# PACTHEMAN123/spMV-test

Hardware: AMD Instinct MI355X
Metric: fp32 CSR SpMV: achieved HBM GB/s (rocprofv3 FETCH_SIZE + WRITE_SIZE bytes of the K steps / wall time) (higher is better)
Workload: dtype f32; 1 GPU; c4: 16777216 x 16777216, nnz 268435456, row lengths 'mixed' mean 16, banded columns (band 8192), seed 20251031; variant=auto, rows_per_gpu=16777216, nnz_per_gpu=268435456, parallelism=single GPU, devices=1 ranks on 1 device(s), launch=one process, algorithmic_bytes_per_gpu=2348810244, hbm_bytes_per_gpu=1840380781

## Files before the change

include/spmv_hip.h:

```cpp
#ifndef SPMV_HIP_H
#define SPMV_HIP_H

#include <stdint.h>

#if defined(__GNUC__)
#define SPMV_API __attribute__((visibility("default")))
#else
#define SPMV_API
#endif

#ifdef __cplusplus
extern "C" {
#endif

typedef struct spmv_csr spmv_csr_t;

enum spmv_status {
    SPMV_OK = 0,
    SPMV_ERR_NO_DEVICE = -1,
    SPMV_ERR_INVALID = -2,
    SPMV_ERR_HIP = -3,
    SPMV_ERR_VARIANT = -4,
    SPMV_ERR_NOT_PLANNED = -5,
    SPMV_ERR_STALE_PLAN = -6
};

enum spmv_variant {
    SPMV_SCALAR = 0,
    SPMV_WAVE = 1,
    SPMV_WAVE_PIPE = 2,
    SPMV_VECTOR = 3,
    SPMV_ADAPTIVE = 4,
    SPMV_TILED = 5,
    SPMV_PANEL = 6,
    SPMV_AUTO = 7,
    SPMV_XSKIP = 8,
    SPMV_VARIANT_COUNT = 9
};

SPMV_API int spmv_device_count(void);
SPMV_API const char *spmv_last_error(void);
SPMV_API const char *spmv_variant_name(int variant);
SPMV_API float spmv_last_first_launch_ms(void);


SPMV_API int spmv_csr_create_host(int64_t rows, int64_t cols, int64_t nnz, const int32_t *row_ptr,
                         const int32_t *col_idx, const float *vals, spmv_csr_t **out);

SPMV_API int spmv_csr_create_device(int64_t rows, int64_t cols, int64_t nnz, const int32_t *d_row_ptr,
                           const int32_t *d_col_idx, const float *d_vals, spmv_csr_t **out);

SPMV_API int spmv_csr_from_dense_host(int M, int N, const float *A_host, void *stream, spmv_csr_t **out);

SPMV_API int spmv_csr_from_dense_device(int M, int N, const float *d_A, void *stream, spmv_csr_t **out);

SPMV_API int spmv_csr_download(const spmv_csr_t *h, int32_t *row_ptr, int32_t *col_idx, float *vals);

SPMV_API int spmv_csr_validate(const spmv_csr_t *h, void *stream);

SPMV_API int spmv_csr_dims(const spmv_csr_t *h, int64_t *rows, int64_t *cols, int64_t *nnz);

SPMV_API int spmv_csr_column_range(const spmv_csr_t *h, int64_t *col_min, int64_t *col_max, void *stream);
SPMV_API int spmv_csr_destroy(spmv_csr_t *h);

SPMV_API int spmv_csr_transpose(const spmv_csr_t *a, int keep_map, void *stream, spmv_csr_t **out);
SPMV_API int spmv_csr_transpose_values(spmv_csr_t *t, const spmv_csr_t *a, void *stream);
SPMV_API int64_t spmv_csr_transpose_map_bytes(const spmv_csr_t *t);

SPMV_API int spmv_csr_plan(spmv_csr_t *h, int variant, void *stream);
SPMV_API int spmv_csr_run(spmv_csr_t *h, int variant, const float *d_x, float *d_y, void *stream);

SPMV_API int spmv_csr_values_changed(spmv_csr_t *h);

SPMV_API int spmv_csr_plan_get(const spmv_csr_t *h, int variant, int32_t params[8]);
SPMV_API int spmv_csr_plan_set(spmv_csr_t *h, int variant, const int32_t params[8], void *stream);
SPMV_API int spmv_csr_plan_like(spmv_csr_t *dst, const spmv_csr_t *src, int variant, void *stream);

SPMV_API int64_t spmv_csr_plan_bytes(const spmv_csr_t *h, int variant);

SPMV_API int spmv_csr_plan_describe(const spmv_csr_t *h, int variant, char *buf, int n);

SPMV_API int spmv_csr_time(spmv_csr_t *h, int variant, const float *d_x, float *d_y, int iters,
                  void *stream, float *ms_per_launch);

SPMV_API int spmv_csr_run_host(spmv_csr_t *h, int variant, const float *x_host, float *y_host,
                               float *kernel_ms);

SPMV_API int spmv_csr_spmm_plan(spmv_csr_t *h, void *stream);
SPMV_API int spmv_csr_spmm(spmv_csr_t *h, int k, const float *d_X, int64_t ldx, float *d_Y, int64_t ldy, void *stream);
SPMV_API int64_t spmv_csr_spmm_plan_bytes(const spmv_csr_t *h);
SPMV_API int spmv_csr_spmm_describe(const spmv_csr_t *h, char *buf, int n);

SPMV_API int spmv_dense_gemv(int M, int N, const float *d_A, const float *d_x, float *d_y, int mode,
                    void *stream);

SPMV_API int64_t spmv_dense_gemv_workspace_bytes(int N, int mode);
SPMV_API int spmv_dense_gemv_ws(int M, int N, const float *d_A, const float *d_x, float *d_y, int mode,
                                void *d_workspace, int64_t workspace_bytes, void *stream);

SPMV_API int spmv_dense_gemv_host(int M, int N, const float *A_host, const float *x_host, float *y_host,
                                  int mode, float *kernel_ms);

SPMV_API int spmv_asp_retile(int M, int N, const float *d_A, float *d_asp, void *stream);
SPMV_API int spmv_asp_gemv_ws(int M, int N, const float *d_asp, const float *d_x, float *d_y, void *d_workspace,
                              int64_t workspace_bytes, void *stream);

typedef struct spmv_tcsr spmv_tcsr_t;
SPMV_API int spmv_tcsr_from_dense_host(int M, int N, const float *A_host, void *stream, spmv_tcsr_t **out);
SPMV_API int spmv_tcsr_from_dense_device(int M, int N, const float *d_A, void *stream, spmv_tcsr_t **out);
SPMV_API int spmv_tcsr_sizes(const spmv_tcsr_t *h, int64_t *n_blk_idx, int64_t *n_bitmaps, int64_t *n_vals);
SPMV_API int spmv_tcsr_download(const spmv_tcsr_t *h, int32_t *blk_idx, uint32_t *bitmaps, float *vals);
SPMV_API int spmv_tcsr_run(const spmv_tcsr_t *h, const float *d_x, float *d_y, void *stream);
SPMV_API int spmv_tcsr_run_host(const spmv_tcsr_t *h, const float *x_host, float *y_host, float *kernel_ms);
SPMV_API int spmv_tcsr_destroy(spmv_tcsr_t *h);

enum spmv_bitmap_format { SPMV_FMT_WSP = 0, SPMV_FMT_AWSP = 1, SPMV_FMT_AWSP_REF = 2, SPMV_FMT_COUNT = 3 };
typedef struct spmv_bitmap spmv_bitmap_t;
SPMV_API int spmv_bitmap_from_dense_host(int format, int M, int N, const float *A_host, void *stream, spmv_bitmap_t **out);
SPMV_API int spmv_bitmap_from_dense_device(int format, int M, int N, const float *d_A, void *stream, spmv_bitmap_t **out);
SPMV_API int spmv_bitmap_sizes(const spmv_bitmap_t *h, int64_t *n_bitmaps, int64_t *n_vals, int32_t stats[4]);
SPMV_API int spmv_bitmap_download(const spmv_bitmap_t *h, uint32_t *bitmaps, float *vals);
SPMV_API int spmv_bitmap_run(const spmv_bitmap_t *h, const float *d_x, float *d_y, void *stream);
SPMV_API int spmv_bitmap_run_host(const spmv_bitmap_t *h, const float *x_host, float *y_host, float *kernel_ms);
SPMV_API int spmv_bitmap_destroy(spmv_bitmap_t *h);

SPMV_API int spmv_synth_fill(uint64_t seed, int64_t row0, int64_t n_local, int64_t rows, int64_t cols,
                    int64_t band, const int32_t *d_row_ptr, int32_t *d_col_idx, float *d_vals,
                    void *stream);
SPMV_API int spmv_synth_x(uint64_t seed, int64_t j0, int64_t n, float *d_x, void *stream);

SPMV_API int spmv_calib_stream(const void *d_src, int64_t bytes, float *d_sink, void *stream);
SPMV_API int spmv_calib_gather(const float *d_table, int64_t table_lines, int64_t n_lines, int touch, float *d_sink,
                               void *stream);
SPMV_API int spmv_calib_store(float *d_dst, int64_t bytes, int width, void *stream);
SPMV_API int spmv_calib_marker(int id, void *stream);

SPMV_API int spmv_debug_bounds(int64_t *records, int n);

#ifdef __cplusplus
}
#endif
#endif
```

spmv-test_amd/capi.py:

```python
from __future__ import annotations

import ctypes as C
import os
from pathlib import Path

PKG_DIR = Path(__file__).resolve().parent
LIB_PATH = PKG_DIR / "lib" / "libspmv_hip.so"
LAUNCHERS_PATH = PKG_DIR / "lib" / "libspmv_launchers.so"
TESTER_PATH = PKG_DIR / "bin" / "sparse_sgemv"
DIST_LIB_PATH = PKG_DIR / "lib" / "libspmv_dist.so"
DIST_SELFTEST_PATH = PKG_DIR / "bin" / "spmv_dist_selftest"

SCALAR, WAVE, WAVE_PIPE, VECTOR, ADAPTIVE, TILED, PANEL, AUTO, XSKIP = range(9)
VARIANTS = {"scalar": SCALAR, "wave": WAVE, "wave_pipe": WAVE_PIPE, "vector": VECTOR,
            "adaptive": ADAPTIVE, "tiled": TILED, "panel": PANEL, "auto": AUTO}
ALL_VARIANTS = dict(VARIANTS, xskip=XSKIP)

OK, ERR_NO_DEVICE, ERR_INVALID, ERR_HIP, ERR_VARIANT, ERR_NOT_PLANNED, ERR_STALE_PLAN = 0, -1, -2, -3, -4, -5, -6

_i32p, _f32p, _vp = C.c_void_p, C.c_void_p, C.c_void_p
_H = C.c_void_p
_HP = C.POINTER(C.c_void_p)
SIGNATURES = {
    "spmv_device_count": (C.c_int, []),
    "spmv_last_error": (C.c_char_p, []),
    "spmv_variant_name": (C.c_char_p, [C.c_int]),
    "spmv_last_first_launch_ms": (C.c_float, []),
    "spmv_csr_create_host": (C.c_int, [C.c_int64, C.c_int64, C.c_int64, _i32p, _i32p, _f32p, _HP]),
    "spmv_csr_create_device": (C.c_int, [C.c_int64, C.c_int64, C.c_int64, _i32p, _i32p, _f32p, _HP]),
    "spmv_csr_from_dense_host": (C.c_int, [C.c_int, C.c_int, _f32p, _vp, _HP]),
    "spmv_csr_from_dense_device": (C.c_int, [C.c_int, C.c_int, _f32p, _vp, _HP]),
    "spmv_csr_download": (C.c_int, [_H, _i32p, _i32p, _f32p]),
    "spmv_csr_validate": (C.c_int, [_H, C.c_void_p]),
    "spmv_csr_dims": (C.c_int, [_H, C.POINTER(C.c_int64), C.POINTER(C.c_int64), C.POINTER(C.c_int64)]),
    "spmv_csr_column_range": (C.c_int, [_H, C.POINTER(C.c_int64), C.POINTER(C.c_int64), _vp]),
    "spmv_csr_destroy": (C.c_int, [_H]),
    "spmv_csr_transpose": (C.c_int, [_H, C.c_int, _vp, _HP]),
    "spmv_csr_transpose_values": (C.c_int, [_H, _H, _vp]),
    "spmv_csr_transpose_map_bytes": (C.c_int64, [_H]),
    "spmv_csr_plan": (C.c_int, [_H, C.c_int, _vp]),
    "spmv_csr_run": (C.c_int, [_H, C.c_int, _f32p, _f32p, _vp]),
    "spmv_csr_values_changed": (C.c_int, [_H]),
    "spmv_csr_spmm_plan": (C.c_int, [_H, _vp]),
    "spmv_csr_spmm": (C.c_int, [_H, C.c_int, _f32p, C.c_int64, _f32p, C.c_int64, _vp]),
    "spmv_csr_spmm_plan_bytes": (C.c_int64, [_H]),
    "spmv_csr_spmm_describe": (C.c_int, [_H, C.c_char_p, C.c_int]),
    "spmv_csr_plan_get": (C.c_int, [_H, C.c_int, C.POINTER(C.c_int32)]),
    "spmv_csr_plan_set": (C.c_int, [_H, C.c_int, C.POINTER(C.c_int32), _vp]),
    "spmv_csr_plan_like": (C.c_int, [_H, _H, C.c_int, _vp]),
    "spmv_csr_plan_bytes": (C.c_int64, [_H, C.c_int]),
    "spmv_csr_plan_describe": (C.c_int, [_H, C.c_int, C.c_char_p, C.c_int]),
    "spmv_csr_time": (C.c_int, [_H, C.c_int, _f32p, _f32p, C.c_int, _vp, C.POINTER(C.c_float)]),
    "spmv_csr_run_host": (C.c_int, [_H, C.c_int, _f32p, _f32p, C.POINTER(C.c_float)]),
    "spmv_dense_gemv": (C.c_int, [C.c_int, C.c_int, _f32p, _f32p, _f32p, C.c_int, _vp]),
    "spmv_dense_gemv_workspace_bytes": (C.c_int64, [C.c_int, C.c_int]),
    "spmv_dense_gemv_ws": (C.c_int, [C.c_int, C.c_int, _f32p, _f32p, _f32p, C.c_int, _vp, C.c_int64, _vp]),
    "spmv_asp_retile": (C.c_int, [C.c_int, C.c_int, _f32p, _f32p, _vp]),
    "spmv_asp_gemv_ws": (C.c_int, [C.c_int, C.c_int, _f32p, _f32p, _f32p, _vp, C.c_int64, _vp]),
    "spmv_dense_gemv_host": (C.c_int, [C.c_int, C.c_int, _f32p, _f32p, _f32p, C.c_int, C.POINTER(C.c_float)]),
    "spmv_tcsr_from_dense_host": (C.c_int, [C.c_int, C.c_int, _f32p, _vp, _HP]),
    "spmv_tcsr_from_dense_device": (C.c_int, [C.c_int, C.c_int, _f32p, _vp, _HP]),
    "spmv_tcsr_sizes": (C.c_int, [_H, C.POINTER(C.c_int64), C.POINTER(C.c_int64), C.POINTER(C.c_int64)]),
    "spmv_tcsr_download": (C.c_int, [_H, _i32p, _i32p, _f32p]),
    "spmv_tcsr_run": (C.c_int, [_H, _f32p, _f32p, _vp]),
    "spmv_tcsr_run_host": (C.c_int, [_H, _f32p, _f32p, C.POINTER(C.c_float)]),
    "spmv_tcsr_destroy": (C.c_int, [_H]),
    "spmv_bitmap_from_dense_host": (C.c_int, [C.c_int, C.c_int, C.c_int, _f32p, _vp, _HP]),
    "spmv_bitmap_from_dense_device": (C.c_int, [C.c_int, C.c_int, C.c_int, _f32p, _vp, _HP]),
    "spmv_bitmap_sizes": (C.c_int, [_H, C.POINTER(C.c_int64), C.POINTER(C.c_int64), C.POINTER(C.c_int32)]),
    "spmv_bitmap_download": (C.c_int, [_H, _i32p, _f32p]),
    "spmv_bitmap_run": (C.c_int, [_H, _f32p, _f32p, _vp]),
    "spmv_bitmap_run_host": (C.c_int, [_H, _f32p, _f32p, C.POINTER(C.c_float)]),
    "spmv_bitmap_destroy": (C.c_int, [_H]),
    "spmv_synth_fill": (C.c_int, [C.c_uint64, C.c_int64, C.c_int64, C.c_int64, C.c_int64, C.c_int64,
                                  _i32p, _i32p, _f32p, _vp]),
    "spmv_synth_x": (C.c_int, [C.c_uint64, C.c_int64, C.c_int64, _f32p, _vp]),
    "spmv_calib_stream": (C.c_int, [_vp, C.c_int64, _f32p, _vp]),
    "spmv_calib_gather": (C.c_int, [_f32p, C.c_int64, C.c_int64, C.c_int, _f32p, _vp]),
    "spmv_calib_store": (C.c_int, [_f32p, C.c_int64, C.c_int, _vp]),
    "spmv_calib_marker": (C.c_int, [C.c_int, _vp]),
    "spmv_debug_bounds": (C.c_int, [_vp, C.c_int]),
}
CHECKED_LIB_PATH = PKG_DIR / "lib" / "libspmv_hip_checked.so"
BOUNDS_SITES = ("k_bs_sums prod", "k_bs_sums acc", "k_bin_sums prod", "k_bin_sums r16", "k_bs_products c16",
                "k_bs_products pvals", "k_bs_products prod store", "k_bs_group store", "k_bs_place load",
                "k_bs_place acc store", "k_bs_place c16/pvals store", "k_bs_fill acc store", "k_bs_fill c16/pvals store",
                "k_panel packed", "k_panel pvals")


class SpmvError(RuntimeError):
    def __init__(self, status: int, message: str):
        super().__init__(f"libspmv_hip status {status}: {message}")
        self.status = status


_lib = None


def use_library(path) -> None:
    global _lib, LIB_PATH
    LIB_PATH = Path(path).resolve()
    _lib = None


def lib() -> C.CDLL:
    global _lib
    if _lib is None:
        if not LIB_PATH.exists():
            raise FileNotFoundError(
                f"{LIB_PATH} is missing: run `python -c 'import __graft_entry__ as g; g.build()'` "
                "(or `make -C spmv-test_amd`); there is no fallback implementation")
        import torch
        l = C.CDLL(os.fspath(LIB_PATH), mode=C.RTLD_LOCAL)
        for name, (res, args) in SIGNATURES.items():
            fn = getattr(l, name)
            fn.restype, fn.argtypes = res, args
        _lib = l
    return _lib


def check(status: int) -> None:
    if status != OK:
        raise SpmvError(status, lib().spmv_last_error().decode(errors="replace"))


def device_count() -> int:
    return lib().spmv_device_count()


def _ptr(t) -> int:
    if t is None:
        return 0
    if hasattr(t, "data_ptr"):
        return t.data_ptr()
    return t.ctypes.data


def _stream_handle(stream=None) -> int:
    import torch
    s = stream if stream is not None else torch.cuda.current_stream()
    return s.cuda_stream


class CsrMatrix:

    def __init__(self, handle: int, keepalive=()):
        self._h = C.c_void_p(handle)
        self._keep = tuple(keepalive)
        r, c, z = C.c_int64(), C.c_int64(), C.c_int64()
        check(lib().spmv_csr_dims(self._h, C.byref(r), C.byref(c), C.byref(z)))
        self.rows, self.cols, self.nnz = r.value, c.value, z.value

    @classmethod
    def from_host(cls, rows, cols, row_ptr, col_idx, vals):
        import numpy as np
        row_ptr = np.ascontiguousarray(row_ptr, dtype=np.int32)
        col_idx = np.ascontiguousarray(col_idx, dtype=np.int32)
        vals = np.ascontiguousarray(vals, dtype=np.float32)
        h = C.c_void_p()
        check(lib().spmv_csr_create_host(rows, cols, int(col_idx.size), _ptr(row_ptr), _ptr(col_idx),
                                         _ptr(vals), C.byref(h)))
        return cls(h.value)

    @classmethod
    def from_device(cls, rows, cols, row_ptr, col_idx, vals):
        h = C.c_void_p()
        check(lib().spmv_csr_create_device(rows, cols, int(col_idx.numel()), _ptr(row_ptr), _ptr(col_idx),
                                           _ptr(vals), C.byref(h)))
        return cls(h.value, keepalive=(row_ptr, col_idx, vals))

    @classmethod
    def from_dense_host(cls, A):
        import numpy as np
        A = np.ascontiguousarray(A, dtype=np.float32)
        M, N = A.shape
        h = C.c_void_p()
        check(lib().spmv_csr_from_dense_host(M, N, _ptr(A), 0, C.byref(h)))
        return cls(h.value)

    @classmethod
    def from_dense_device(cls, A):
        M, N = A.shape
        h = C.c_void_p()
        check(lib().spmv_csr_from_dense_device(M, N, _ptr(A), _stream_handle(), C.byref(h)))
        return cls(h.value)

    def plan(self, variant: int, stream=None) -> None:
        check(lib().spmv_csr_plan(self._h, variant, _stream_handle(stream)))

    def run(self, variant: int, x, y, stream=None) -> None:
        assert x.numel() >= self.cols and y.numel() >= self.rows
        check(lib().spmv_csr_run(self._h, variant, _ptr(x), _ptr(y), _stream_handle(stream)))

    def column_range(self, stream=None):
        lo, hi = C.c_int64(), C.c_int64()
        check(lib().spmv_csr_column_range(self._h, C.byref(lo), C.byref(hi), _stream_handle(stream)))
        return lo.value, hi.value

    def transpose(self, keep_map: bool = False, stream=None) -> "CsrMatrix":
        h = C.c_void_p()
        check(lib().spmv_csr_transpose(self._h, 1 if keep_map else 0, _stream_handle(stream), C.byref(h)))
        return CsrMatrix(h.value)

    def transpose_values(self, a: "CsrMatrix", stream=None) -> None:
        check(lib().spmv_csr_transpose_values(self._h, a._h, _stream_handle(stream)))

    def transpose_map_bytes(self) -> int:
        n = lib().spmv_csr_transpose_map_bytes(self._h)
        if n < 0:
            check(n)
        return n

    def spmm_plan(self, stream=None) -> None:
        check(lib().spmv_csr_spmm_plan(self._h, _stream_handle(stream)))

    def spmm(self, X, Y, stream=None) -> None:
        import torch
        for name, t in (("X", X), ("Y", Y)):
            if not isinstance(t, torch.Tensor) or t.dim() != 2 or t.dtype != torch.float32 or t.stride(1) != 1:
                raise ValueError(f"spmm: {name} must be a 2-D float32 tensor with stride(1) == 1")
        k = X.shape[1]
        if X.shape[0] != self.cols or Y.shape[0] != self.rows or Y.shape[1] < k:
            raise ValueError(f"spmm: X {tuple(X.shape)} and Y {tuple(Y.shape)} do not fit a {self.rows} x {self.cols} matrix")
        check(lib().spmv_csr_spmm(self._h, k, _ptr(X), X.stride(0), _ptr(Y), Y.stride(0), _stream_handle(stream)))

    def spmm_describe(self) -> str:
        buf = C.create_string_buffer(256)
        check(lib().spmv_csr_spmm_describe(self._h, buf, 256))
        return buf.value.decode()

    def spmm_plan_bytes(self) -> int:
        n = lib().spmv_csr_spmm_plan_bytes(self._h)
        if n < 0:
            check(n)
        return n

    def values_changed(self) -> None:
        check(lib().spmv_csr_values_changed(self._h))

    def time(self, variant: int, x, y, iters: int, stream=None) -> float:
        ms = C.c_float()
        check(lib().spmv_csr_time(self._h, variant, _ptr(x), _ptr(y), iters, _stream_handle(stream),
                                  C.byref(ms)))
        return ms.value

    def run_host(self, variant: int, x, y) -> float:
        import numpy as np
        assert x.dtype == np.float32 and y.dtype == np.float32
        ms = C.c_float()
        check(lib().spmv_csr_run_host(self._h, variant, _ptr(x), _ptr(y), C.byref(ms)))
        return ms.value

    def plan_params(self, variant: int):
        a = (C.c_int32 * 8)()
        check(lib().spmv_csr_plan_get(self._h, variant, a))
        return list(a)

    def plan_set(self, variant: int, params, stream=None) -> None:
        a = (C.c_int32 * 8)(*params)
        check(lib().spmv_csr_plan_set(self._h, variant, a, _stream_handle(stream)))

    def plan_like(self, other: "CsrMatrix", variant: int, stream=None) -> None:
        check(lib().spmv_csr_plan_like(self._h, other._h, variant, _stream_handle(stream)))

    def plan_describe(self, variant: int) -> str:
        buf = C.create_string_buffer(256)
        check(lib().spmv_csr_plan_describe(self._h, variant, buf, 256))
        return buf.value.decode()

    def plan_bytes(self, variant: int) -> int:
        return lib().spmv_csr_plan_bytes(self._h, variant)

    def download(self):
        import numpy as np
        rp = np.empty(self.rows + 1, np.int32)
        ci = np.empty(self.nnz, np.int32)
        va = np.empty(self.nnz, np.float32)
        check(lib().spmv_csr_download(self._h, _ptr(rp), _ptr(ci), _ptr(va)))
        return rp, ci, va

    def close(self) -> None:
        if self._h:
            check(lib().spmv_csr_destroy(self._h))
            self._h = C.c_void_p()
            self._keep = ()

    def __del__(self):
        try:
            self.close()
        except Exception:
            pass


class TcsrMatrix:

    def __init__(self, handle: int, M: int, N: int):
        self._h = C.c_void_p(handle)
        self.M, self.N = M, N
        a, b, c = C.c_int64(), C.c_int64(), C.c_int64()
        check(lib().spmv_tcsr_sizes(self._h, C.byref(a), C.byref(b), C.byref(c)))
        self.n_blk_idx, self.n_bitmaps, self.nnz = a.value, b.value, c.value

    @classmethod
    def from_dense_host(cls, A):
        import numpy as np
        A = np.ascontiguousarray(A, dtype=np.float32)
        M, N = A.shape
        h = C.c_void_p()
        check(lib().spmv_tcsr_from_dense_host(M, N, _ptr(A), 0, C.byref(h)))
        return cls(h.value, M, N)

    @classmethod
    def from_dense_device(cls, A):
        M, N = A.shape
        h = C.c_void_p()
        check(lib().spmv_tcsr_from_dense_device(M, N, _ptr(A), _stream_handle(), C.byref(h)))
        return cls(h.value, M, N)

    def download(self):
        import numpy as np
        bi = np.empty(self.n_blk_idx, np.int32)
        bm = np.empty(self.n_bitmaps, np.uint32)
        va = np.empty(self.nnz, np.float32)
        check(lib().spmv_tcsr_download(self._h, _ptr(bi), _ptr(bm), _ptr(va)))
        return bi, bm, va

    def run(self, x, y, stream=None) -> None:
        assert x.numel() >= self.M and y.numel() >= self.N
        check(lib().spmv_tcsr_run(self._h, _ptr(x), _ptr(y), _stream_handle(stream)))

    def run_host(self, x, y) -> float:
        ms = C.c_float()
        check(lib().spmv_tcsr_run_host(self._h, _ptr(x), _ptr(y), C.byref(ms)))
        return ms.value

    def close(self) -> None:
        if self._h:
            check(lib().spmv_tcsr_destroy(self._h))
            self._h = C.c_void_p()

    def __del__(self):
        try:
            self.close()
        except Exception:
            pass


BITMAP_FORMATS = {"wsp": 0, "awsp": 1, "awsp_ref": 2}


class BitmapMatrix:

    def __init__(self, handle: int, fmt: str, M: int, N: int):
        self._h = C.c_void_p(handle)
        self.fmt, self.M, self.N = fmt, M, N
        a, b = C.c_int64(), C.c_int64()
        st = (C.c_int32 * 4)()
        check(lib().spmv_bitmap_sizes(self._h, C.byref(a), C.byref(b), st))
        self.n_bitmaps, self.n_vals, self.stats = a.value, b.value, list(st)

    @classmethod
    def from_dense_host(cls, fmt: str, A):
        import numpy as np
        A = np.ascontiguousarray(A, dtype=np.float32)
        M, N = A.shape
        h = C.c_void_p()
        check(lib().spmv_bitmap_from_dense_host(BITMAP_FORMATS[fmt], M, N, _ptr(A), 0, C.byref(h)))
        return cls(h.value, fmt, M, N)

    @classmethod
    def from_dense_device(cls, fmt: str, A):
        M, N = A.shape
        h = C.c_void_p()
        check(lib().spmv_bitmap_from_dense_device(BITMAP_FORMATS[fmt], M, N, _ptr(A), _stream_handle(), C.byref(h)))
        return cls(h.value, fmt, M, N)

    def download(self):
        import numpy as np
        bm = np.empty(self.n_bitmaps, np.uint32)
        va = np.empty(self.n_vals, np.float32)
        check(lib().spmv_bitmap_download(self._h, _ptr(bm), _ptr(va)))
        return bm, va

    def run(self, x, y, stream=None) -> None:
        assert x.numel() >= self.M and y.numel() >= self.N
        check(lib().spmv_bitmap_run(self._h, _ptr(x), _ptr(y), _stream_handle(stream)))

    def run_host(self, x, y) -> float:
        ms = C.c_float()
        check(lib().spmv_bitmap_run_host(self._h, _ptr(x), _ptr(y), C.byref(ms)))
        return ms.value

    def close(self) -> None:
        if self._h:
            check(lib().spmv_bitmap_destroy(self._h))
            self._h = C.c_void_p()

    def __del__(self):
        try:
            self.close()
        except Exception:
            pass


def dense_gemv(A, x, y, mode: int, stream=None, workspace=None) -> None:
    M, N = A.shape
    if workspace is None:
        check(lib().spmv_dense_gemv(M, N, _ptr(A), _ptr(x), _ptr(y), mode, _stream_handle(stream)))
    else:
        check(lib().spmv_dense_gemv_ws(M, N, _ptr(A), _ptr(x), _ptr(y), mode, _ptr(workspace),
                                       workspace.numel() * workspace.element_size(), _stream_handle(stream)))


def dense_gemv_workspace_bytes(N: int, mode: int) -> int:
    return lib().spmv_dense_gemv_workspace_bytes(N, mode)


def asp_retile(A, out, stream=None) -> None:
    M, N = A.shape
    check(lib().spmv_asp_retile(M, N, _ptr(A), _ptr(out), _stream_handle(stream)))


def asp_gemv(M: int, N: int, asp, x, y, workspace, stream=None) -> None:
    check(lib().spmv_asp_gemv_ws(M, N, _ptr(asp), _ptr(x), _ptr(y), _ptr(workspace),
                                 workspace.numel() * workspace.element_size(), _stream_handle(stream)))


def synth_fill(seed, row0, n_local, rows, cols, band, row_ptr, col_idx, vals, stream=None) -> None:
    check(lib().spmv_synth_fill(seed, row0, n_local, rows, cols, band, _ptr(row_ptr), _ptr(col_idx),
                                _ptr(vals), _stream_handle(stream)))


def synth_x(seed, j0, n, x, stream=None) -> None:
    check(lib().spmv_synth_x(seed, j0, n, _ptr(x), _stream_handle(stream)))


def calib_stream(src, nbytes: int, sink, stream=None) -> None:
    check(lib().spmv_calib_stream(_ptr(src), nbytes, _ptr(sink), _stream_handle(stream)))


def calib_gather(table, table_lines: int, n_lines: int, touch: int, sink, stream=None) -> None:
    check(lib().spmv_calib_gather(_ptr(table), table_lines, n_lines, touch, _ptr(sink), _stream_handle(stream)))


def calib_store(dst, nbytes: int, width: int, stream=None) -> None:
    check(lib().spmv_calib_store(_ptr(dst), nbytes, width, _stream_handle(stream)))


def calib_marker(ident: int, stream=None) -> None:
    check(lib().spmv_calib_marker(ident, _stream_handle(stream)))


def debug_bounds(max_records: int = 64) -> list:
    import numpy as np
    rec = np.zeros(3 * max_records, np.int64)
    n = lib().spmv_debug_bounds(rec.ctypes.data, max_records)
    if n < 0:
        check(n)
    return [(BOUNDS_SITES[int(rec[3 * i])], int(rec[3 * i + 1]), int(rec[3 * i + 2])) for i in range(min(n, max_records))]
```

spmv-test_amd/csrc/capi.hip:

```cpp
#include <cstdarg>
#include <cstdint>
#include <cstdlib>
#include <cstring>
#include <new>
#include "spmv_internal.hpp"

namespace spmv {

static thread_local char g_err[512] = "";
static thread_local float g_first_launch_ms = 0.0f;

void set_error(const char *fmt, ...)
{
    va_list ap;
    va_start(ap, fmt);
    vsnprintf(g_err, sizeof g_err, fmt, ap);
    va_end(ap);
}

int hip_fail(hipError_t e, const char *what, const char *file, int line)
{
    set_error("HIP error %s:%d: %s (%s)", file, line, hipGetErrorString(e), what);
    return SPMV_ERR_HIP;
}

static int require_device()
{
    int n = 0;
    hipError_t e = hipGetDeviceCount(&n);
    if (e != hipSuccess || n <= 0) {
        (void)hipGetLastError();
        set_error("no HIP device visible (hipGetDeviceCount: %s); libspmv_hip has no CPU path",
                  e == hipSuccess ? "0 devices" : hipGetErrorString(e));
        return SPMV_ERR_NO_DEVICE;
    }
    return SPMV_OK;
}

int LdsOptIn::ensure(const void *fn, int device, int bytes)
{
    const uint64_t bit = (device >= 0 && device < 64) ? (1ull << device) : 0ull;
    if (bit && (done.load(std::memory_order_acquire) & bit)) return SPMV_OK;
    SPMV_HIP_TRY(hipFuncSetAttribute(fn, hipFuncAttributeMaxDynamicSharedMemorySize, bytes));
    if (bit) done.fetch_or(bit, std::memory_order_release);
    return SPMV_OK;
}

int device_cus(int device)
{
    static std::atomic<int> cache[64];
    const bool cached = device >= 0 && device < 64;
    if (cached) {
        const int c = cache[device].load(std::memory_order_relaxed);
        if (c > 0) return c;
    }
    int cus = 0;
    if (hipDeviceGetAttribute(&cus, hipDeviceAttributeMultiprocessorCount, device) != hipSuccess || cus <= 0) {
        (void)hipGetLastError();
        cus = 256;
    }
    if (cached) cache[device].store(cus, std::memory_order_relaxed);
    return cus;
}

int require_current(int device, const char *what)
{
    int cur = -1;
    if (hipGetDevice(&cur) != hipSuccess) {
        (void)hipGetLastError();
        set_error("%s: hipGetDevice failed", what);
        return SPMV_ERR_HIP;
    }
    if (cur != device) {
        set_error("%s: the handle lives on device %d but the current device is %d (hipSetDevice first)", what, device, cur);
        return SPMV_ERR_INVALID;
    }
    return SPMV_OK;
}

static bool aligned16(const void *p) { return (reinterpret_cast<uintptr_t>(p) & 15u) == 0; }

template <typename Launch>
static int time_cold_then_warm(const Launch &launch, float *kernel_ms)
{
    hipEvent_t ev[2] = {nullptr, nullptr};
    const int rc = [&]() -> int {
        SPMV_HIP_TRY(hipEventCreate(&ev[0]));
        SPMV_HIP_TRY(hipEventCreate(&ev[1]));
        float ms = 0.0f;
        for (int i = 0; i < 2; ++i) {
            SPMV_HIP_TRY(hipEventRecord(ev[0], nullptr));
            const int r = launch();
            SPMV_HIP_TRY(hipEventRecord(ev[1], nullptr));
            SPMV_HIP_TRY(hipEventSynchronize(ev[1]));
            if (r) return r;
            SPMV_HIP_TRY(hipEventElapsedTime(i == 0 ? &g_first_launch_ms : &ms, ev[0], ev[1]));
            SPMV_HIP_TRY(hipDeviceSynchronize());
        }
        if (kernel_ms) *kernel_ms = ms;
        return SPMV_OK;
    }();
    for (hipEvent_t e : ev)
        if (e) (void)hipEventDestroy(e);
    return rc;
}

}

using namespace spmv;

extern "C" {

int spmv_device_count(void)
{
    int n = 0;
    if (hipGetDeviceCount(&n) != hipSuccess) {
        (void)hipGetLastError();
        return 0;
    }
    return n;
}

const char *spmv_last_error(void) { return g_err; }

float spmv_last_first_launch_ms(void) { return g_first_launch_ms; }

int spmv_debug_bounds(int64_t *records, int n)
{
#if defined(SPMV_CHECK_BOUNDS)
    if (n < 0 || (n > 0 && !records)) {
        spmv::set_error("spmv_debug_bounds: n = %d records at %p", n, (void *)records);
        return SPMV_ERR_INVALID;
    }
    unsigned long long t[spmv::kBoundsSites][2] = {};
    if (int rc = spmv::bounds_collect_binned(t)) return rc;
    if (int rc = spmv::bounds_collect_panel(t)) return rc;
    int hit = 0;
    for (int i = 0; i < spmv::kBoundsSites; ++i) {
        if (t[i][0] == 0) continue;
        if (hit < n) {
            records[3 * hit] = i;
            records[3 * hit + 1] = (int64_t)t[i][0];
            records[3 * hit + 2] = (int64_t)t[i][1];
        }
        ++hit;
    }
    return hit;
#else
    (void)records;
    (void)n;
    spmv::set_error("spmv_debug_bounds: not instrumented (this is the normal build; lib/libspmv_hip_checked.so is the checked one)");
    return SPMV_ERR_INVALID;
#endif
}

const char *spmv_variant_name(int variant)
{
    switch (variant) {
        case SPMV_SCALAR: return "scalar";
        case SPMV_WAVE: return "wave";
        case SPMV_WAVE_PIPE: return "wave_pipe";
        case SPMV_VECTOR: return "vector";
        case SPMV_ADAPTIVE: return "adaptive";
        case SPMV_TILED: return "tiled";
        case SPMV_PANEL: return "panel";
        case SPMV_AUTO: return "auto";
        case SPMV_XSKIP: return "xskip";
        default: return "unknown";
    }
}

static int check_dims(int64_t rows, int64_t cols, int64_t nnz)
{
    if (rows < 0 || cols < 0 || nnz < 0 || rows >= (1LL << 31) || cols >= (1LL << 31) || nnz >= (1LL << 31)) {
        set_error("bad dimensions rows=%lld cols=%lld nnz=%lld (each must be in [0, 2^31))", (long long)rows,
                  (long long)cols, (long long)nnz);
        return SPMV_ERR_INVALID;
    }
    return SPMV_OK;
}

int spmv_csr_validate(const spmv_csr_t *h, void *stream)
{
    if (!h) { set_error("spmv_csr_validate: null handle"); return SPMV_ERR_INVALID; }
    hipStream_t st = (hipStream_t)stream;
    const int32_t init[4] = {INT32_MAX, INT32_MAX, 0, (int32_t)h->nnz};
    int32_t bad[4];
    DevPtr<int32_t> d_bad;
    SPMV_HIP_TRY(d_bad.alloc(4));
    SPMV_HIP_TRY(hipMemcpyAsync(d_bad.get(), init, sizeof init, hipMemcpyHostToDevice, st));
    int rc = launch_validate(h, d_bad.get(), st);
    if (rc) return rc;
    SPMV_HIP_TRY(hipMemcpyAsync(bad, d_bad.get(), sizeof bad, hipMemcpyDeviceToHost, st));
    SPMV_HIP_TRY(hipStreamSynchronize(st));
    if (bad[2] != 0 || (int64_t)bad[3] != h->nnz) {
        set_error("malformed CSR: row_ptr[0]=%d row_ptr[rows]=%d, expected 0 and nnz=%lld", bad[2], bad[3],
                  (long long)h->nnz);
        return SPMV_ERR_INVALID;
    }
    if (bad[0] != INT32_MAX) {
        set_error("malformed CSR: row_ptr decreases or leaves [0, nnz] at row %d", bad[0]);
        return SPMV_ERR_INVALID;
    }
    if (bad[1] != INT32_MAX) {
        set_error("malformed CSR: column index of element %d is outside [0, %lld)", bad[1], (long long)h->cols);
        return SPMV_ERR_INVALID;
    }
    return SPMV_OK;
}

int spmv_csr_create_host(int64_t rows, int64_t cols, int64_t nnz, const int32_t *row_ptr,
                         const int32_t *col_idx, const float *vals, spmv_csr_t **out)
{
    if (!out || !row_ptr || (nnz > 0 && (!col_idx || !vals))) {
        set_error("spmv_csr_create_host: null argument");
        return SPMV_ERR_INVALID;
    }
    int rc = check_dims(rows, cols, nnz);
    if (rc) return rc;
    if ((rc = require_device())) return rc;
    if (row_ptr[0] != 0 || row_ptr[rows] != nnz) {
        set_error("spmv_csr_create_host: row_ptr[0]=%d row_ptr[rows]=%d, expected 0 and nnz=%lld", row_ptr[0],
                  row_ptr[rows], (long long)nnz);
        return SPMV_ERR_INVALID;
    }
    DevPtr<int32_t> rp, ci;
    DevPtr<float> va;
    SPMV_HIP_TRY(rp.alloc((size_t)rows + 1));
    SPMV_HIP_TRY(ci.alloc((size_t)nnz));
    SPMV_HIP_TRY(va.alloc((size_t)nnz));
    SPMV_HIP_TRY(hipMemcpy(rp.get(), row_ptr, sizeof(int32_t) * ((size_t)rows + 1), hipMemcpyHostToDevice));
    if (nnz > 0) {
        SPMV_HIP_TRY(hipMemcpy(ci.get(), col_idx, sizeof(int32_t) * (size_t)nnz, hipMemcpyHostToDevice));
        SPMV_HIP_TRY(hipMemcpy(va.get(), vals, sizeof(float) * (size_t)nnz, hipMemcpyHostToDevice));
    }
    spmv_csr *h = new (std::nothrow) spmv_csr();
    if (!h) { set_error("out of host memory"); return SPMV_ERR_INVALID; }
    h->rows = rows; h->cols = cols; h->nnz = nnz;
    if (hipGetDevice(&h->device) != hipSuccess) h->device = 0;
    h->d_row_ptr = rp; h->d_col_idx = ci; h->d_vals = va;
    h->own_row_ptr = std::move(rp); h->own_col_idx = std::move(ci); h->own_vals = std::move(va);
    if ((rc = spmv_csr_validate(h, nullptr))) {
        spmv_csr_destroy(h);
        return rc;
    }
    *out = h;
    return SPMV_OK;
}

int spmv_csr_create_device(int64_t rows, int64_t cols, int64_t nnz, const int32_t *d_row_ptr,
                           const int32_t *d_col_idx, const float *d_vals, spmv_csr_t **out)
{
    if (!out || !d_row_ptr || (nnz > 0 && (!d_col_idx || !d_vals))) {
        set_error("spmv_csr_create_device: null argument");
        return SPMV_ERR_INVALID;
    }
    int rc = check_dims(rows, cols, nnz);
    if (rc) return rc;
    if ((rc = require_device())) return rc;
    if (!aligned16(d_col_idx) || !aligned16(d_vals)) {
        set_error("spmv_csr_create_device: col_idx and vals must be 16-byte aligned");
        return SPMV_ERR_INVALID;
    }
    spmv_csr *h = new (std::nothrow) spmv_csr();
    if (!h) { set_error("out of host memory"); return SPMV_ERR_INVALID; }
    h->rows = rows; h->cols = cols; h->nnz = nnz;
    h->d_row_ptr = d_row_ptr; h->d_col_idx = d_col_idx; h->d_vals = d_vals;
    if (hipGetDevice(&h->device) != hipSuccess) h->device = 0;
    if ((rc = spmv_csr_validate(h, nullptr))) {
        delete h;
        return rc;
    }
    *out = h;
    return SPMV_OK;
}

int spmv_csr_from_dense_device(int M, int N, const float *d_A, void *stream, spmv_csr_t **out)
{
    if (!out || M < 0 || N < 0 || (!d_A && (int64_t)M * N > 0)) {
        set_error("spmv_csr_from_dense_device: bad argument");
        return SPMV_ERR_INVALID;
    }
    int rc = require_device();
    if (rc) return rc;
    return dense_to_csr(M, N, d_A, (hipStream_t)stream, out);
}

int spmv_csr_from_dense_host(int M, int N, const float *A_host, void *stream, spmv_csr_t **out)
{
    if (!out || M < 0 || N < 0 || (!A_host && (int64_t)M * N > 0)) {
        set_error("spmv_csr_from_dense_host: bad argument");
        return SPMV_ERR_INVALID;
    }
    int rc = require_device();
    if (rc) return rc;
    const size_t bytes = sizeof(float) * (size_t)M * (size_t)N;
    DevPtr<float> dA;
    SPMV_HIP_TRY(dA.alloc((size_t)M * (size_t)N));
    SPMV_HIP_TRY(hipMemcpyAsync(dA.get(), A_host, bytes, hipMemcpyHostToDevice, (hipStream_t)stream));
    rc = dense_to_csr(M, N, dA.get(), (hipStream_t)stream, out);
    (void)hipStreamSynchronize((hipStream_t)stream);
    return rc;
}

int spmv_csr_download(const spmv_csr_t *h, int32_t *row_ptr, int32_t *col_idx, float *vals)
{
    if (!h) { set_error("spmv_csr_download: null handle"); return SPMV_ERR_INVALID; }
    if (row_ptr)
        SPMV_HIP_TRY(hipMemcpy(row_ptr, h->d_row_ptr, sizeof(int32_t) * ((size_t)h->rows + 1), hipMemcpyDeviceToHost));
    if (col_idx && h->nnz)
        SPMV_HIP_TRY(hipMemcpy(col_idx, h->d_col_idx, sizeof(int32_t) * (size_t)h->nnz, hipMemcpyDeviceToHost));
    if (vals && h->nnz)
        SPMV_HIP_TRY(hipMemcpy(vals, h->d_vals, sizeof(float) * (size_t)h->nnz, hipMemcpyDeviceToHost));
    return SPMV_OK;
}

int spmv_csr_dims(const spmv_csr_t *h, int64_t *rows, int64_t *cols, int64_t *nnz)
{
    if (!h) { set_error("spmv_csr_dims: null handle"); return SPMV_ERR_INVALID; }
    if (rows) *rows = h->rows;
    if (cols) *cols = h->cols;
    if (nnz) *nnz = h->nnz;
    return SPMV_OK;
}

int spmv_csr_column_range(const spmv_csr_t *h, int64_t *col_min, int64_t *col_max, void *stream)
{
    if (!h || !col_min || !col_max) { set_error("spmv_csr_column_range: null argument"); return SPMV_ERR_INVALID; }
    hipStream_t st = (hipStream_t)stream;
    DevPtr<int32_t> d;
    SPMV_HIP_TRY(d.alloc(2));
    int rc = launch_column_range(*h, d.get(), st);
    if (rc) return rc;
    int32_t out[2] = {0, 0};
    SPMV_HIP_TRY(hipMemcpyAsync(out, d.get(), sizeof out, hipMemcpyDeviceToHost, st));
    SPMV_HIP_TRY(hipStreamSynchronize(st));
    *col_min = out[1] < 0 ? h->cols : (int64_t)out[0];
    *col_max = (int64_t)out[1];
    return SPMV_OK;
}

int spmv_csr_destroy(spmv_csr_t *h)
{
    if (!h) return SPMV_OK;
    int rc = SPMV_OK;
    for (hipError_t e : {h->own_row_ptr.reset(), h->own_col_idx.reset(), h->own_vals.reset()})
        if (e != hipSuccess) rc = SPMV_ERR_HIP;
    delete h;
    if (rc) set_error("hipFree failed in spmv_csr_destroy");
    return rc;
}

int spmv_csr_transpose(const spmv_csr_t *a, int keep_map, void *stream, spmv_csr_t **out)
{
    if (!a || !out) { set_error("spmv_csr_transpose: null argument"); return SPMV_ERR_INVALID; }
    if (keep_map != 0 && keep_map != 1) {
        set_error("spmv_csr_transpose: keep_map = %d (0 or 1)", keep_map);
        return SPMV_ERR_INVALID;
    }
    if (int rc = require_device()) return rc;
    if (int rc = require_current(a->device, "spmv_csr_transpose")) return rc;
    return transpose(*a, keep_map == 1, (hipStream_t)stream, out);
}

int spmv_csr_transpose_values(spmv_csr_t *t, const spmv_csr_t *a, void *stream)
{
    if (!t || !a) { set_error("spmv_csr_transpose_values: null argument"); return SPMV_ERR_INVALID; }
    if (!t->transpose_map) {
        set_error("spmv_csr_transpose_values: the handle has no map (it was not made by spmv_csr_transpose with keep_map = 1)");
        return SPMV_ERR_INVALID;
    }
    if (a->rows != t->cols || a->cols != t->rows || a->nnz != t->nnz) {
        set_error("spmv_csr_transpose_values: a is %lld x %lld with %lld nonzeros, the transpose of t would be %lld x %lld with %lld",
                  (long long)a->rows, (long long)a->cols, (long long)a->nnz, (long long)t->cols, (long long)t->rows,
                  (long long)t->nnz);
        return SPMV_ERR_INVALID;
    }
    if (int rc = require_current(t->device, "spmv_csr_transpose_values")) return rc;
    if (a->device != t->device) {
        set_error("spmv_csr_transpose_values: a lives on device %d, t on device %d", a->device, t->device);
        return SPMV_ERR_INVALID;
    }
    if (int rc = transpose_values(*t, *a, (hipStream_t)stream)) return rc;
    ++t->values_gen;
    return SPMV_OK;
}

int64_t spmv_csr_transpose_map_bytes(const spmv_csr_t *t)
{
    if (!t) { set_error("spmv_csr_transpose_map_bytes: null handle"); return SPMV_ERR_INVALID; }
    return t->transpose_map ? 4 * t->nnz : 0;
}

static int plan_auto(spmv_csr &h, hipStream_t s)
{
    if (h.auto_variant == SPMV_PANEL) return refresh_panel(h, h.plan_auto_panel, s);
    if (h.auto_variant >= 0) return SPMV_OK;
    h.auto_made_tiled = h.plan_tiled.block == 0;
    int rc = plan_adaptive(h, true, s);
    if (rc) return rc;
    auto release_tiled = [&]() { if (h.auto_made_tiled) h.plan_tiled = ChunkPlan{}; h.auto_made_tiled = false; };
    const ChunkPlan &p = h.plan_tiled;
    const double cost_tiled = p.model_cost;
    const bool little_staged = p.nchunks > 0 && 2 * ((int64_t)p.staged_full + p.nsorted) < p.nchunks &&
                               2 * (int64_t)p.nblk_chunks < p.nchunks;
    const bool x_beyond_l2 = h.cols * (int64_t)sizeof(float) >= (4ll << 20);
    bool try_sorted = p.nchunks > 0 && cost_tiled > 1.20 && 2 * (int64_t)p.nblk_chunks < p.nchunks &&
                      h.rows >= 4096ll * (3 * device_cus(h.device) / 4);
    if (const char *e = getenv("SPMV_AUTO_SORTED_BLOCKS")) try_sorted = try_sorted && atoi(e) != 0;
    if (try_sorted) {
        double long_frac = 0.0, wide_frac = 0.0, lines_est = 0.0;
        if ((rc = colsort_probe(h, s, &long_frac, &wide_frac, &lines_est))) return rc;
        if (long_frac <= 0.10 && wide_frac <= 0.10 && 0.95 * colsort_cost(4096, lines_est, long_frac) < cost_tiled) {
            const bool big = lines_est > 0.30 && h.rows >= 4096ll * 16 * device_cus(h.device);
            rc = build_panel(h, h.plan_auto_panel, big ? 8192 : 0, big ? 4 : 0, 3, s);
            if (rc == SPMV_OK) {
                const PanelPlan &pp = h.plan_auto_panel;
                const bool fits = (double)pp.tail <= 0.10 * (double)h.nnz && 10 * pp.wide_blocks <= pp.nblocks;
                if (fits && colsort_model_cost(pp, h.nnz) < 0.98 * cost_tiled) {
                    h.auto_variant = SPMV_PANEL;
                    release_tiled();
                    return SPMV_OK;
                }
                h.plan_auto_panel = PanelPlan{};
            } else if (rc != SPMV_ERR_INVALID) {
                return rc;
            }
        }
    }
    if (little_staged && x_beyond_l2) {
        const bool big_x = h.cols * (int64_t)sizeof(float) >= (8ll << 20);
        const double tile = binned_tile_nonzeros(h, 4096);
        int try_binned = big_x && tile >= 4.0 ? 5 : 0;
        if (const char *e = getenv("SPMV_AUTO_BINNED")) try_binned = atoi(e) != 0 ? try_binned : 0;
        if (try_binned) {
            rc = build_panel(h, h.plan_auto_panel, 0, 0, try_binned, s);
            if (rc == SPMV_OK && try_binned == 5 && 32 * (int64_t)h.plan_auto_panel.flagged_tiles > h.plan_auto_panel.nblocks)
                rc = build_panel(h, h.plan_auto_panel, 0, 0, 4, s);
            if (rc == SPMV_OK) {
                h.auto_variant = SPMV_PANEL;
                release_tiled();
                return SPMV_OK;
            }
            if (rc != SPMV_ERR_INVALID) return rc;
        }
        rc = build_panel(h, h.plan_auto_panel, 0, 0, 1, s);
        if (rc == SPMV_OK) {
            h.auto_variant = SPMV_PANEL;
            release_tiled();
            return SPMV_OK;
        }
        if (rc != SPMV_ERR_INVALID) return rc;
    }
    h.auto_variant = SPMV_TILED;
    return SPMV_OK;
}

int spmv_csr_plan(spmv_csr_t *h, int variant, void *stream)
{
    if (!h) { set_error("spmv_csr_plan: null handle"); return SPMV_ERR_INVALID; }
    if (int rc = require_current(h->device, "spmv_csr_plan")) return rc;
    hipStream_t s = (hipStream_t)stream;
    switch (variant) {
        case SPMV_AUTO: return plan_auto(*h, s);
        case SPMV_WAVE: return h->nnz <= 32 * h->rows ? plan_wave(*h, s) : SPMV_OK;
        case SPMV_SCALAR:
        case SPMV_WAVE_PIPE: return plan_wave(*h, s);
        case SPMV_VECTOR: return plan_vector(*h, s);
        case SPMV_ADAPTIVE: return plan_adaptive(*h, false, s);
        case SPMV_TILED: return plan_adaptive(*h, true, s);
        case SPMV_PANEL: return plan_panel(*h, s);
        case SPMV_XSKIP: return plan_xskip(*h, s);
        default:
            set_error("spmv_csr_plan: unknown variant %d", variant);
            return SPMV_ERR_VARIANT;
    }
}

int spmv_csr_run(spmv_csr_t *h, int variant, const float *d_x, float *d_y, void *stream)
{
    if (!h || (!d_x && h->cols > 0) || (!d_y && h->rows > 0)) {
        set_error("spmv_csr_run: null argument");
        return SPMV_ERR_INVALID;
    }
    if (!aligned16(d_x)) {
        set_error("spmv_csr_run: x must be 16-byte aligned");
        return SPMV_ERR_INVALID;
    }
    if (int rc = require_current(h->device, "spmv_csr_run")) return rc;
    hipStream_t s = (hipStream_t)stream;
    if (variant == SPMV_AUTO) {
        if (h->auto_variant < 0) { set_error("SPMV_AUTO used before spmv_csr_plan"); return SPMV_ERR_NOT_PLANNED; }
        if (h->auto_variant == SPMV_PANEL) return launch_panel_plan(*h, h->plan_auto_panel, d_x, d_y, s);
        variant = h->auto_variant;
    }
    switch (variant) {
        case SPMV_SCALAR: return launch_scalar(*h, d_x, d_y, s);
        case SPMV_WAVE: return launch_wave(*h, d_x, d_y, false, s);
        case SPMV_WAVE_PIPE: return launch_wave(*h, d_x, d_y, true, s);
        case SPMV_VECTOR: return launch_vector(*h, d_x, d_y, s);
        case SPMV_ADAPTIVE: return launch_adaptive(*h, d_x, d_y, false, s);
        case SPMV_TILED: return launch_adaptive(*h, d_x, d_y, true, s);
        case SPMV_PANEL: return launch_panel(*h, d_x, d_y, s);
        case SPMV_XSKIP: return launch_xskip(*h, d_x, d_y, s);
        default:
            set_error("spmv_csr_run: unknown variant %d", variant);
            return SPMV_ERR_VARIANT;
    }
}

int spmv_csr_spmm_plan(spmv_csr_t *h, void *stream)
{
    if (!h) { set_error("spmv_csr_spmm_plan: null handle"); return SPMV_ERR_INVALID; }
    if (int rc = require_current(h->device, "spmv_csr_spmm_plan")) return rc;
    return plan_spmm(*h, (hipStream_t)stream);
}

int spmv_csr_spmm(spmv_csr_t *h, int k, const float *d_X, int64_t ldx, float *d_Y, int64_t ldy, void *stream)
{
    if (!h) { set_error("spmv_csr_spmm: null handle"); return SPMV_ERR_INVALID; }
    if (k < 1 || k > 64 || ldx < k || ldy < k) {
        set_error("spmv_csr_spmm: k = %d, ldx = %lld, ldy = %lld (need 1 <= k <= 64, ldx >= k, ldy >= k)", k, (long long)ldx,
                  (long long)ldy);
        return SPMV_ERR_INVALID;
    }
    if ((!d_X && h->cols > 0) || (!d_Y && h->rows > 0)) { set_error("spmv_csr_spmm: null X or Y"); return SPMV_ERR_INVALID; }
    if (!aligned16(d_X) || !aligned16(d_Y)) { set_error("spmv_csr_spmm: X and Y must be 16-byte aligned"); return SPMV_ERR_INVALID; }
    if (ldx > INT64_MAX / 4 / (h->cols > 0 ? h->cols : 1) || ldy > INT64_MAX / 4 / (h->rows > 0 ? h->rows : 1)) {
        set_error("spmv_csr_spmm: ldx = %lld or ldy = %lld overflows 64-bit byte offsets", (long long)ldx, (long long)ldy);
        return SPMV_ERR_INVALID;
    }
    if (int rc = require_current(h->device, "spmv_csr_spmm")) return rc;
    if (!h->plan_spmm.ready) { set_error("spmv_csr_spmm used before spmv_csr_spmm_plan"); return SPMV_ERR_NOT_PLANNED; }
    return launch_spmm(*h, k, d_X, ldx, d_Y, ldy, (hipStream_t)stream);
}

int64_t spmv_csr_spmm_plan_bytes(const spmv_csr_t *h)
{
    if (!h) { set_error("spmv_csr_spmm_plan_bytes: null handle"); return SPMV_ERR_INVALID; }
    return spmm_plan_bytes(*h);
}

int spmv_csr_spmm_describe(const spmv_csr_t *h, char *buf, int n)
{
    if (!h || !buf || n <= 0) { set_error("spmv_csr_spmm_describe: bad argument"); return SPMV_ERR_INVALID; }
    const SpmmPlan &p = h->plan_spmm;
    if (!p.ready) snprintf(buf, (size_t)n, "not planned");
    else snprintf(buf, (size_t)n, "row_cap=%d piece_len=%d long_rows=%d pieces=%d", p.row_cap, p.piece_len, p.n_long, p.pieces);
    return SPMV_OK;
}

int spmv_csr_values_changed(spmv_csr_t *h)
{
    if (!h) { set_error("spmv_csr_values_changed: null handle"); return SPMV_ERR_INVALID; }
    ++h->values_gen;
    return SPMV_OK;
}

int spmv_csr_plan_get(const spmv_csr_t *h, int variant, int32_t params[8])
{
    if (!h || !params) { set_error("spmv_csr_plan_get: null argument"); return SPMV_ERR_INVALID; }
    for (int i = 0; i < 8; ++i) params[i] = 0;
    const bool is_auto = variant == SPMV_AUTO;
    if (variant == SPMV_AUTO) {
        if (h->auto_variant < 0) { set_error("spmv_csr_plan_get: SPMV_AUTO is not planned"); return SPMV_ERR_NOT_PLANNED; }
        variant = h->auto_variant;
    }
    const PanelPlan &panel = is_auto ? h->plan_auto_panel : h->plan_panel;
    params[0] = variant;
    switch (variant) {
        case SPMV_SCALAR: case SPMV_WAVE: case SPMV_WAVE_PIPE: return SPMV_OK;
        case SPMV_VECTOR: params[1] = h->vector_width; return SPMV_OK;
        case SPMV_ADAPTIVE:
        case SPMV_TILED: {
            const ChunkPlan &p = variant == SPMV_TILED ? h->plan_tiled : h->plan_adaptive;
            if (!p.block) { set_error("spmv_csr_plan_get: variant %d is not planned", variant); return SPMV_ERR_NOT_PLANNED; }
            params[1] = p.block; params[2] = p.maxpass; params[3] = p.col16_wanted ? 1 : 0;
            return SPMV_OK;
        }
        case SPMV_XSKIP:
            if (!h->plan_xskip.ready) { set_error("spmv_csr_plan_get: xskip is not planned"); return SPMV_ERR_NOT_PLANNED; }
            params[1] = h->plan_xskip.slabs;
            return SPMV_OK;
        case SPMV_PANEL:
            if (!panel.ready) { set_error("spmv_csr_plan_get: panel is not planned"); return SPMV_ERR_NOT_PLANNED; }
            params[4] = panel.pw_bits; params[5] = panel.waves_per_launch;
            params[6] = panel.binned_mode ? (panel.scatter_mode ? 5 : 4) : panel.sorted_mode ? 3 : (panel.lds_mode ? 2 : 1);
            if (panel.sorted_mode) { params[4] = panel.sb_rows; params[5] = panel.sb_waves; }
            if (panel.binned_mode) { params[4] = panel.bin_rows; params[5] = 0; }
            return SPMV_OK;
        default: set_error("spmv_csr_plan_get: unknown variant %d", variant); return SPMV_ERR_VARIANT;
    }
}

int spmv_csr_plan_set(spmv_csr_t *h, int variant, const int32_t params[8], void *stream)
{
    if (!h || !params) { set_error("spmv_csr_plan_set: null argument"); return SPMV_ERR_INVALID; }
    if (int rc = require_current(h->device, "spmv_csr_plan_set")) return rc;
    hipStream_t s = (hipStream_t)stream;
    int target = variant;
    if (variant == SPMV_AUTO) {
        target = params[0];
        if (target != SPMV_TILED && target != SPMV_PANEL) {
            set_error("spmv_csr_plan_set: SPMV_AUTO resolves to tiled or panel, not %d", target);
            return SPMV_ERR_INVALID;
        }
    } else if (params[0] != variant) {
        set_error("spmv_csr_plan_set: params describe variant %d, not %d", params[0], variant);
        return SPMV_ERR_INVALID;
    }
    int rc;
    switch (target) {
        case SPMV_SCALAR: case SPMV_WAVE: case SPMV_WAVE_PIPE: rc = SPMV_OK; break;
        case SPMV_VECTOR: {
            const int w = params[1];
            if (w != 2 && w != 4 && w != 8 && w != 16 && w != 32) { set_error("spmv_csr_plan_set: lanes per row %d", w); return SPMV_ERR_INVALID; }
            h->vector_width = w;
            rc = SPMV_OK;
            break;
        }
        case SPMV_ADAPTIVE: rc = plan_adaptive_with(*h, params[1], s); break;
        case SPMV_TILED: rc = plan_tiled_with(*h, params[1], params[2], params[3] != 0, s); break;
        case SPMV_PANEL: rc = build_panel(*h, variant == SPMV_AUTO ? h->plan_auto_panel : h->plan_panel, params[4], params[5], params[6], s); break;
        case SPMV_XSKIP: h->plan_xskip = XskipPlan{}; rc = plan_xskip(*h, s); break;
        default: set_error("spmv_csr_plan_set: unknown variant %d", target); return SPMV_ERR_VARIANT;
    }
    if (rc == SPMV_OK && variant == SPMV_AUTO) h->auto_variant = target;
    return rc;
}

int spmv_csr_plan_like(spmv_csr_t *dst, const spmv_csr_t *src, int variant, void *stream)
{
    int32_t params[8];
    int rc = spmv_csr_plan_get(src, variant, params);
    return rc ? rc : spmv_csr_plan_set(dst, variant, params, stream);
}

int64_t spmv_csr_plan_bytes(const spmv_csr_t *h, int variant)
{
    if (!h) return 0;
    const PanelPlan &panel = variant == SPMV_AUTO ? h->plan_auto_panel : h->plan_panel;
    if (variant == SPMV_AUTO) variant = h->auto_variant;
    switch (variant) {
        case SPMV_ADAPTIVE:
            return (int64_t)(h->plan_adaptive.nchunks + 1) * 4 + (int64_t)h->plan_adaptive.nchunks * 8;
        case SPMV_TILED:
            return (int64_t)(h->plan_tiled.nchunks + 1) * 4 + (int64_t)h->plan_tiled.nchunks * 16 +
                   ((h->plan_tiled.n16 || h->plan_tiled.nsorted) ? (int64_t)h->plan_tiled.nchunks * 4 : 0) +
                   (int64_t)h->plan_tiled.n16 * 2 * h->plan_tiled.block * kNnzPerThread +
                   (int64_t)h->plan_tiled.nsorted * 4 * h->plan_tiled.block * kNnzPerThread +
                   (int64_t)h->plan_tiled.nblk_chunks * 256 * 4;
        case SPMV_XSKIP:
            return (int64_t)h->plan_xskip.nseg * 8 + ((int64_t)h->plan_xskip.nblocks + 1) * 4 +
                   (h->plan_xskip.slabs > 1 ? (int64_t)h->plan_xskip.nblocks * h->plan_xskip.slabs * 1024 * 8 : 0);
        case SPMV_PANEL:
            if (panel.binned_mode && panel.scatter_mode)
                return panel.padded * (2 + 4) + panel.padded / 512 * 4 + panel.runs * 4 + panel.bm_entries * (4 + 2) +
                       (int64_t)panel.nblocks * (1024 * 4 + 16) + ((int64_t)panel.npanels + 1) * 4;
            if (panel.binned_mode)
                return (int64_t)panel.nblocks * (2 * (int64_t)panel.npanels + 2) * 4 + panel.padded * (2 + 4 + 4) + h->nnz * 2;
            if (panel.sorted_mode)
                return panel.units * 4 + (int64_t)panel.nblocks * 20 + panel.tail_units * 512;
            return (int64_t)panel.nblocks * (panel.npanels + 1) * 4 + ((int64_t)panel.nblocks + 1) * 4;
        case SPMV_WAVE:
            if (h->nnz > 32 * h->rows) return 0;
            return (int64_t)h->plan_wave.n_long * 8 + (int64_t)h->plan_wave.pieces * 16;
        case SPMV_SCALAR:
        case SPMV_WAVE_PIPE:
            return (int64_t)h->plan_wave.n_long * 8 + (int64_t)h->plan_wave.pieces * 16 + h->plan_wave.blocks * 8;
        default: return 0;
    }
}

int spmv_csr_plan_describe(const spmv_csr_t *h, int variant, char *buf, int n)
{
    if (!h || !buf || n <= 0) { set_error("spmv_csr_plan_describe: bad argument"); return SPMV_ERR_INVALID; }
    const PanelPlan *panel = &h->plan_panel;
    if (variant == SPMV_AUTO) {
        if (h->auto_variant < 0) { snprintf(buf, (size_t)n, "not planned"); return SPMV_OK; }
        const int w = snprintf(buf, (size_t)n, "auto -> %s: ", spmv_variant_name(h->auto_variant));
        if (w < 0 || w >= n) return SPMV_OK;
        if (h->auto_variant != SPMV_PANEL) return spmv_csr_plan_describe(h, h->auto_variant, buf + w, n - w);
        panel = &h->plan_auto_panel;
        variant = SPMV_PANEL;
        buf += w;
        n -= w;
    }
    const ChunkPlan *p = variant == SPMV_ADAPTIVE ? &h->plan_adaptive : (variant == SPMV_TILED ? &h->plan_tiled : nullptr);
    if (variant == SPMV_VECTOR) snprintf(buf, (size_t)n, "lanes_per_row=%d", h->vector_width);
    else if (variant == SPMV_WAVE && h->nnz > 32 * h->rows) snprintf(buf, (size_t)n, "no plan (a wavefront per row)");
    else if (variant == SPMV_WAVE_PIPE || variant == SPMV_SCALAR || variant == SPMV_WAVE) {
        if (!h->plan_wave.ready) snprintf(buf, (size_t)n, "not planned (the first run plans)");
        else snprintf(buf, (size_t)n, "long_rows=%d pieces=%d block_rows=%d blocks=%lld blocks_with_x_window=%lld col16=%d", h->plan_wave.n_long,
                      h->plan_wave.pieces, h->plan_wave.block_rows, (long long)h->plan_wave.blocks, (long long)h->plan_wave.win_blocks,
                      h->plan_wave.d_col16 ? 1 : 0);
    }
    else if (variant == SPMV_PANEL && panel->ready && panel->binned_mode && panel->scatter_mode)
        snprintf(buf, (size_t)n, "binned scattered_products bins=%d rows_per_bin=%d panels=%d panel_columns=%d nonzeros_per_tile=%.1f rows_with_spare_sums=%d flagged_bins=%d product_workgroups_per_panel=%d padded=%lld bin_entries=%lld",
                 panel->nblocks, panel->bin_rows, panel->npanels, 1 << panel->pw_bits,
                 panel->nblocks ? (double)h->nnz / ((double)panel->nblocks * panel->npanels) : 0.0, panel->long_rows, panel->flagged_tiles,
                 panel->splits, (long long)panel->padded, (long long)panel->bm_entries);
    else if (variant == SPMV_PANEL && panel->ready && panel->binned_mode)
        snprintf(buf, (size_t)n, "binned bins=%d rows_per_bin=%d panels=%d panel_columns=%d nonzeros_per_tile=%.1f products_per_lane=%d long_rows=%d flagged_tiles=%d product_workgroups_per_panel=%d padded=%lld",
                 panel->nblocks, panel->bin_rows, panel->npanels, 1 << panel->pw_bits,
                 panel->nblocks ? (double)h->nnz / ((double)panel->nblocks * panel->npanels) : 0.0, panel->wide_pieces ? 4 : 2, panel->long_rows, panel->flagged_tiles, panel->splits,
                 (long long)panel->padded);
    else if (variant == SPMV_PANEL && panel->ready && panel->sorted_mode)
        snprintf(buf, (size_t)n, "sorted_blocks=%d rows_per_block=%d wavefronts=%d lines_per_nonzero=%.3f tail_nonzeros=%lld wide_blocks=%lld model_cost=%.3f",
                 panel->nblocks, panel->sb_rows, panel->sb_waves,
                 h->nnz ? (double)panel->lines / (double)h->nnz : 0.0, (long long)panel->tail,
                 (long long)panel->wide_blocks, colsort_model_cost(*panel, h->nnz));
    else if (variant == SPMV_PANEL && panel->ready)
        snprintf(buf, (size_t)n, "panel_columns=%d panels=%d row_blocks=%d waves_per_launch=%d launches=%d x_panels_in=%s nonzeros_per_step=%d",
                 1 << panel->pw_bits, panel->npanels, panel->nblocks,
                 panel->waves_per_launch, panel_launches(*panel), panel->lds_mode ? "LDS" : "L2", panel->lds_mode ? 64 : 256 * panel->step_vecs);
    else if (variant == SPMV_XSKIP && h->plan_xskip.ready)
        snprintf(buf, (size_t)n, "output_blocks=%d segments=%d slabs_per_block=%d", h->plan_xskip.nblocks, h->plan_xskip.nseg,
                 h->plan_xskip.slabs);
    else if (!p) snprintf(buf, (size_t)n, "no plan");
    else if (!p->block) snprintf(buf, (size_t)n, "not planned");
    else
        snprintf(buf, (size_t)n, "block=%d region=%d maxpass=%d chunks=%d staged_single=%d staged_full=%d col16_chunks=%d sorted_chunks=%d block_list_chunks=%d spanning_rows=%d persist=%d model_cost=%.3f",
                 p->block, p->region, p->maxpass, p->nchunks, p->staged_single, p->staged_full, p->n16, p->nsorted,
                 p->nblk_chunks, p->spanning_rows, p->persist ? 1 : 0, p->model_cost);
    return SPMV_OK;
}

int spmv_csr_time(spmv_csr_t *h, int variant, const float *d_x, float *d_y, int iters, void *stream,
                  float *ms_per_launch)
{
    if (iters <= 0 || !ms_per_launch) { set_error("spmv_csr_time: bad argument"); return SPMV_ERR_INVALID; }
    hipStream_t s = (hipStream_t)stream;
    hipEvent_t t0, t1;
    SPMV_HIP_TRY(hipEventCreate(&t0));
    SPMV_HIP_TRY(hipEventCreate(&t1));
    int rc = SPMV_OK;
    SPMV_HIP_TRY(hipEventRecord(t0, s));
    for (int i = 0; i < iters && rc == SPMV_OK; ++i) rc = spmv_csr_run(h, variant, d_x, d_y, s);
    SPMV_HIP_TRY(hipEventRecord(t1, s));
    SPMV_HIP_TRY(hipEventSynchronize(t1));
    float ms = 0.0f;
    SPMV_HIP_TRY(hipEventElapsedTime(&ms, t0, t1));
    (void)hipEventDestroy(t0);
    (void)hipEventDestroy(t1);
    *ms_per_launch = ms / (float)iters;
    return rc;
}

int spmv_csr_run_host(spmv_csr_t *h, int variant, const float *x_host, float *y_host, float *kernel_ms)
{
    if (!h || (!x_host && h->cols > 0) || (!y_host && h->rows > 0)) {
        set_error("spmv_csr_run_host: null argument");
        return SPMV_ERR_INVALID;
    }
    int rc = spmv_csr_plan(h, variant, nullptr);
    if (rc) return rc;
    DevPtr<float> dx, dy;
    SPMV_HIP_TRY(dx.alloc((size_t)h->cols));
    SPMV_HIP_TRY(dy.alloc((size_t)h->rows));
    SPMV_HIP_TRY(hipMemcpy(dx.get(), x_host, sizeof(float) * (size_t)h->cols, hipMemcpyHostToDevice));
    if ((rc = time_cold_then_warm([&] { return spmv_csr_run(h, variant, dx.get(), dy.get(), nullptr); }, kernel_ms)))
        return rc;
    SPMV_HIP_TRY(hipMemcpy(y_host, dy.get(), sizeof(float) * (size_t)h->rows, hipMemcpyDeviceToHost));
    return SPMV_OK;
}

int spmv_dense_gemv_host(int M, int N, const float *A_host, const float *x_host, float *y_host, int mode,
                         float *kernel_ms)
{
    if (M < 0 || N < 0 || ((int64_t)M * N > 0 && (!A_host || !x_host)) || (N > 0 && !y_host)) {
        set_error("spmv_dense_gemv_host: bad argument");
        return SPMV_ERR_INVALID;
    }
    int rc = require_device();
    if (rc) return rc;
    DevPtr<float> dA, dx, dy;
    SPMV_HIP_TRY(dA.alloc((size_t)M * (size_t)N));
    SPMV_HIP_TRY(dx.alloc((size_t)M));
    SPMV_HIP_TRY(dy.alloc((size_t)N));
    SPMV_HIP_TRY(hipMemcpy(dA.get(), A_host, sizeof(float) * (size_t)M * (size_t)N, hipMemcpyHostToDevice));
    SPMV_HIP_TRY(hipMemcpy(dx.get(), x_host, sizeof(float) * (size_t)M, hipMemcpyHostToDevice));
    if ((rc = time_cold_then_warm([&] { return dense_gemv(M, N, dA.get(), dx.get(), dy.get(), mode, nullptr); }, kernel_ms)))
        return rc;
    SPMV_HIP_TRY(hipMemcpy(y_host, dy.get(), sizeof(float) * (size_t)N, hipMemcpyDeviceToHost));
    return SPMV_OK;
}

static int tcsr_check_dims(int M, int N, const void *A, const void *out)
{
    if (!out || M < 0 || N < 0 || (M % 32) || (N % 32) || (!A && (int64_t)M * N > 0) || (int64_t)M * N >= (1LL << 36)) {
        set_error("spmv_tcsr_from_dense: M and N must be non-negative multiples of 32 (got %d x %d)", M, N);
        return SPMV_ERR_INVALID;
    }
    return require_device();
}

int spmv_tcsr_from_dense_device(int M, int N, const float *d_A, void *stream, spmv_tcsr_t **out)
{
    int rc = tcsr_check_dims(M, N, d_A, out);
    if (rc) return rc;
    return tcsr_from_dense(M, N, d_A, (hipStream_t)stream, out);
}

int spmv_tcsr_from_dense_host(int M, int N, const float *A_host, void *stream, spmv_tcsr_t **out)
{
    int rc = tcsr_check_dims(M, N, A_host, out);
    if (rc) return rc;
    DevPtr<float> dA;
    const size_t bytes = sizeof(float) * (size_t)M * (size_t)N;
    SPMV_HIP_TRY(dA.alloc((size_t)M * (size_t)N));
    SPMV_HIP_TRY(hipMemcpyAsync(dA.get(), A_host, bytes, hipMemcpyHostToDevice, (hipStream_t)stream));
    rc = tcsr_from_dense(M, N, dA.get(), (hipStream_t)stream, out);
    (void)hipStreamSynchronize((hipStream_t)stream);
    return rc;
}

int spmv_tcsr_sizes(const spmv_tcsr_t *h, int64_t *n_blk_idx, int64_t *n_bitmaps, int64_t *n_vals)
{
    if (!h) { set_error("spmv_tcsr_sizes: null handle"); return SPMV_ERR_INVALID; }
    return tcsr_sizes(*h, n_blk_idx, n_bitmaps, n_vals);
}

int spmv_tcsr_download(const spmv_tcsr_t *h, int32_t *blk_idx, uint32_t *bitmaps, float *vals)
{
    if (!h) { set_error("spmv_tcsr_download: null handle"); return SPMV_ERR_INVALID; }
    return tcsr_download(*h, blk_idx, bitmaps, vals);
}

int spmv_tcsr_run(const spmv_tcsr_t *h, const float *d_x, float *d_y, void *stream)
{
    if (!h || !d_x || !d_y) { set_error("spmv_tcsr_run: null argument"); return SPMV_ERR_INVALID; }
    return tcsr_run(*h, d_x, d_y, (hipStream_t)stream);
}

int spmv_tcsr_run_host(const spmv_tcsr_t *h, const float *x_host, float *y_host, float *kernel_ms)
{
    if (!h || !x_host || !y_host) { set_error("spmv_tcsr_run_host: null argument"); return SPMV_ERR_INVALID; }
    int64_t nb = 0, nw = 0, nv = 0;
    tcsr_sizes(*h, &nb, &nw, &nv);
    int M = 0, N = 0;
    tcsr_dims(*h, &M, &N);
    DevPtr<float> dx, dy;
    SPMV_HIP_TRY(dx.alloc((size_t)M));
    SPMV_HIP_TRY(dy.alloc((size_t)N));
    SPMV_HIP_TRY(hipMemcpy(dx.get(), x_host, sizeof(float) * (size_t)M, hipMemcpyHostToDevice));
    if (int rc = time_cold_then_warm([&] { return tcsr_run(*h, dx.get(), dy.get(), nullptr); }, kernel_ms)) return rc;
    SPMV_HIP_TRY(hipMemcpy(y_host, dy.get(), sizeof(float) * (size_t)N, hipMemcpyDeviceToHost));
    return SPMV_OK;
}

int spmv_tcsr_destroy(spmv_tcsr_t *h)
{
    delete h;
    return SPMV_OK;
}

static int bitmap_check_dims(int format, int M, int N, const void *A, const void *out)
{
    if (format < 0 || format >= SPMV_FMT_COUNT) { set_error("spmv_bitmap_from_dense: unknown format %d", format); return SPMV_ERR_VARIANT; }
    if (!out || M < 0 || N < 0 || (M % 32) || (N % 32) || (!A && (int64_t)M * N > 0) || (int64_t)M * N >= (1LL << 36)) {
        set_error("spmv_bitmap_from_dense: M and N must be non-negative multiples of 32 (got %d x %d)", M, N);
        return SPMV_ERR_INVALID;
    }
    return require_device();
}

int spmv_bitmap_from_dense_device(int format, int M, int N, const float *d_A, void *stream, spmv_bitmap_t **out)
{
    int rc = bitmap_check_dims(format, M, N, d_A, out);
    if (rc) return rc;
    return bitmap_from_dense(format, M, N, d_A, (hipStream_t)stream, out);
}

int spmv_bitmap_from_dense_host(int format, int M, int N, const float *A_host, void *stream, spmv_bitmap_t **out)
{
    int rc = bitmap_check_dims(format, M, N, A_host, out);
    if (rc) return rc;
    DevPtr<float> dA;
    const size_t bytes = sizeof(float) * (size_t)M * (size_t)N;
    SPMV_HIP_TRY(dA.alloc((size_t)M * (size_t)N));
    SPMV_HIP_TRY(hipMemcpyAsync(dA.get(), A_host, bytes, hipMemcpyHostToDevice, (hipStream_t)stream));
    rc = bitmap_from_dense(format, M, N, dA.get(), (hipStream_t)stream, out);
    (void)hipStreamSynchronize((hipStream_t)stream);
    return rc;
}

int spmv_bitmap_sizes(const spmv_bitmap_t *h, int64_t *n_bitmaps, int64_t *n_vals, int32_t stats[4])
{
    if (!h) { set_error("spmv_bitmap_sizes: null handle"); return SPMV_ERR_INVALID; }
    bitmap_info(*h, nullptr, nullptr, nullptr, n_bitmaps, n_vals, stats);
    return SPMV_OK;
}

int spmv_bitmap_download(const spmv_bitmap_t *h, uint32_t *bitmaps, float *vals)
{
    if (!h) { set_error("spmv_bitmap_download: null handle"); return SPMV_ERR_INVALID; }
    return bitmap_download(*h, bitmaps, vals);
}

int spmv_bitmap_run(const spmv_bitmap_t *h, const float *d_x, float *d_y, void *stream)
{
    if (!h || !d_x || !d_y) { set_error("spmv_bitmap_run: null argument"); return SPMV_ERR_INVALID; }
    if (int rc = require_current(bitmap_device(*h), "spmv_bitmap_run")) return rc;
    return bitmap_run(*h, d_x, d_y, (hipStream_t)stream);
}

int spmv_bitmap_run_host(const spmv_bitmap_t *h, const float *x_host, float *y_host, float *kernel_ms)
{
    if (!h || !x_host || !y_host) { set_error("spmv_bitmap_run_host: null argument"); return SPMV_ERR_INVALID; }
    int M = 0, N = 0;
    bitmap_info(*h, nullptr, &M, &N, nullptr, nullptr, nullptr);
    DevPtr<float> dx, dy;
    SPMV_HIP_TRY(dx.alloc((size_t)M));
    SPMV_HIP_TRY(dy.alloc((size_t)N));
    SPMV_HIP_TRY(hipMemcpy(dx.get(), x_host, sizeof(float) * (size_t)M, hipMemcpyHostToDevice));
    if (int rc = time_cold_then_warm([&] { return bitmap_run(*h, dx.get(), dy.get(), nullptr); }, kernel_ms)) return rc;
    SPMV_HIP_TRY(hipMemcpy(y_host, dy.get(), sizeof(float) * (size_t)N, hipMemcpyDeviceToHost));
    return SPMV_OK;
}

int spmv_bitmap_destroy(spmv_bitmap_t *h)
{
    delete h;
    return SPMV_OK;
}

int spmv_dense_gemv(int M, int N, const float *d_A, const float *d_x, float *d_y, int mode, void *stream)
{
    if (M < 0 || N < 0 || ((int64_t)M * N > 0 && (!d_A || !d_x)) || (N > 0 && !d_y)) {
        set_error("spmv_dense_gemv: bad argument");
        return SPMV_ERR_INVALID;
    }
    int rc = require_device();
    if (rc) return rc;
    return dense_gemv(M, N, d_A, d_x, d_y, mode, (hipStream_t)stream);
}

int64_t spmv_dense_gemv_workspace_bytes(int N, int mode) { return (int64_t)dense_gemv_workspace_bytes(N, mode); }

int spmv_dense_gemv_ws(int M, int N, const float *d_A, const float *d_x, float *d_y, int mode, void *d_workspace,
                       int64_t workspace_bytes, void *stream)
{
    if (M < 0 || N < 0 || ((int64_t)M * N > 0 && (!d_A || !d_x)) || (N > 0 && !d_y) || workspace_bytes < 0) {
        set_error("spmv_dense_gemv_ws: bad argument");
        return SPMV_ERR_INVALID;
    }
    int rc = require_device();
    if (rc) return rc;
    return dense_gemv_ws(M, N, d_A, d_x, d_y, mode, d_workspace, (size_t)workspace_bytes, (hipStream_t)stream);
}

int spmv_asp_retile(int M, int N, const float *d_A, float *d_asp, void *stream)
{
    if (M < 0 || N < 0 || (M % 32) || (N % 32) || ((int64_t)M * N > 0 && (!d_A || !d_asp))) {
        set_error("spmv_asp_retile: bad argument (M and N are multiples of 32, like the reference's tester asserts)");
        return SPMV_ERR_INVALID;
    }
    int rc = require_device();
    if (rc) return rc;
    return asp_retile(M, N, d_A, d_asp, (hipStream_t)stream);
}

int spmv_asp_gemv_ws(int M, int N, const float *d_asp, const float *d_x, float *d_y, void *d_workspace, int64_t workspace_bytes,
                     void *stream)
{
    if (M < 0 || N < 0 || (M % 32) || (N % 32) || ((int64_t)M * N > 0 && (!d_asp || !d_x)) || (N > 0 && !d_y) ||
        workspace_bytes < 0) {
        set_error("spmv_asp_gemv_ws: bad argument");
        return SPMV_ERR_INVALID;
    }
    int rc = require_device();
    if (rc) return rc;
    return asp_gemv_ws(M, N, d_asp, d_x, d_y, d_workspace, (size_t)workspace_bytes, (hipStream_t)stream);
}

int spmv_synth_fill(uint64_t seed, int64_t row0, int64_t n_local, int64_t rows, int64_t cols, int64_t band,
                    const int32_t *d_row_ptr, int32_t *d_col_idx, float *d_vals, void *stream)
{
    if (n_local < 0 || row0 < 0 || row0 + n_local > rows || cols <= 0 || cols >= (1LL << 31) ||
        rows >= (1LL << 31) || !d_row_ptr) {
        set_error("spmv_synth_fill: bad argument");
        return SPMV_ERR_INVALID;
    }
    int rc = require_device();
    if (rc) return rc;
    return synth_fill(seed, row0, n_local, rows, cols, band, d_row_ptr, d_col_idx, d_vals, (hipStream_t)stream);
}

int spmv_synth_x(uint64_t seed, int64_t j0, int64_t n, float *d_x, void *stream)
{
    if (n < 0 || j0 < 0 || (n > 0 && !d_x)) { set_error("spmv_synth_x: bad argument"); return SPMV_ERR_INVALID; }
    int rc = require_device();
    if (rc) return rc;
    return synth_x(seed, j0, n, d_x, (hipStream_t)stream);
}

}
```

spmv-test_amd/csrc/kernels_adaptive.hip:

```cpp
#include <atomic>
#include <climits>
#include <cstdlib>
#include <cstring>
#include "spmv_internal.hpp"

namespace spmv {

using i4 = int __attribute__((ext_vector_type(4)));
using f4 = float __attribute__((ext_vector_type(4)));

#ifndef SPMV_T_GROUP
#define SPMV_T_GROUP 16
#endif
constexpr int kGroup = SPMV_T_GROUP;

__host__ __device__ constexpr int chunk_of(int block) { return block * kNnzPerThread; }
__host__ __device__ constexpr int prod_words(int block) { return chunk_of(block) + (chunk_of(block) >> 5); }
__host__ __device__ constexpr int region_words(int block) { return (block / 256) * 4832; }
static_assert(region_words(256) >= prod_words(256), "region must hold the products");
__host__ __device__ constexpr int max_long(int block) { return chunk_of(block) / (kShortSeg + 1) + 2; }
#ifndef SPMV_T_HUGE
#define SPMV_T_HUGE 512
#endif
constexpr int kHugeSeg = SPMV_T_HUGE;
__host__ __device__ constexpr int max_huge(int block) { return chunk_of(block) / (kHugeSeg + 1) + 2; }

#ifdef SPMV_T_NOPAD
__device__ __forceinline__ int pad_idx(int i) { return i; }
#else
__device__ __forceinline__ int pad_idx(int i) { return i + (i >> 5); }
#endif
template <int BLOCK>
__device__ __forceinline__ void zero_pad_words(float *smem, int tid)
{
#ifndef SPMV_T_NOPAD
    for (int h = tid; h < (chunk_of(BLOCK) >> 5); h += BLOCK) smem[h * 33 + 32] = 0.0f;
#endif
}

__device__ __forceinline__ int xcd_chunk(int bid, int n)
{
    const int q = n / kXcds, rem = n % kXcds;
    const int j = bid % kXcds, idx = bid / kXcds;
    return j * q + (j < rem ? j : rem) + idx;
}

__global__ void k_plan_chunks(int64_t rows, int nchunks, int chunk, const int32_t *__restrict__ row_ptr,
                              int32_t *__restrict__ lb)
{
    int c = blockIdx.x * blockDim.x + threadIdx.x;
    if (c > nchunks) return;
    if (c == nchunks) { lb[c] = (int32_t)rows; return; }
    const int64_t key = (int64_t)c * chunk;
    int64_t lo = 0, hi = rows;
    while (lo < hi) {
        int64_t mid = (lo + hi) >> 1;
        if ((int64_t)row_ptr[mid] < key) lo = mid + 1; else hi = mid;
    }
    lb[c] = (int32_t)lo;
}

constexpr int kOutsideBit = 1 << 30;
constexpr int kCol16Bit = 1 << 29;
constexpr int kBlockBit = 1 << 28;
constexpr int kSortedBit = 1 << 27;
constexpr int kLenMask = kSortedBit - 1;
#ifndef SPMV_T_SORTED_FROM
#define SPMV_T_SORTED_FROM (-1)
#endif
constexpr int kSortedFromDefault = SPMV_T_SORTED_FROM;
__host__ __device__ constexpr int sorted_pos_bits(int block) { return block == 1024 ? 14 : (block == 512 ? 13 : 12); }
__host__ __device__ constexpr int sorted_col_bits(int) { return 18; }
static_assert(sorted_pos_bits(1024) + sorted_col_bits(1024) <= 32, "one word per nonzero");
#ifndef SPMV_T_BLKBITS
#define SPMV_T_BLKBITS 8
#endif
constexpr int kBlkBits = SPMV_T_BLKBITS;
constexpr int kBlkCols = 1 << kBlkBits;
constexpr int kBlkMax = 65536 / kBlkCols;

struct PlanCost {
    int c16_base = 788, c16_pass = 110, c32_base = 1075, c32_pass = 123, sorted_base = 1075, sorted_line_512 = 1792,
        sorted_line_1024 = 1485, sorted_few_rows = 205, unstaged = 3072, long_piece = 512;
};

__global__ __launch_bounds__(256) void k_plan_windows(int64_t nnz, int64_t cols, int nchunks, int chunk,
                                                      const int32_t *__restrict__ col_idx,
                                                      int32_t *__restrict__ win, int32_t *__restrict__ stats,
                                                      int region, int maxpass, int sorted_from, int sorted_span,
                                                      PlanCost cost, const int32_t *__restrict__ lb,
                                                      const int32_t *__restrict__ row_ptr)
{
    __shared__ int s_min[4], s_max[4], s_cnt[4];
    __shared__ long long s_sum[4];
    __shared__ int s_w0;
    const int c = blockIdx.x;
    const int wv = threadIdx.x >> 6;
    const bool lane0 = (threadIdx.x & (kWave - 1)) == 0;
    const int64_t base = (int64_t)c * chunk;
    const int n = (int)((nnz - base) < chunk ? (nnz - base) : chunk);
    int mn = 0x7fffffff, mx = -1;
    long long sum = 0;
    for (int i = threadIdx.x; i < n; i += 256) {
        int v = col_idx[base + i];
        mn = v < mn ? v : mn;
        mx = v > mx ? v : mx;
        sum += v;
    }
#pragma unroll
    for (int o = kWave / 2; o > 0; o >>= 1) {
        int a = __shfl_down(mn, o, kWave), b = __shfl_down(mx, o, kWave);
        mn = a < mn ? a : mn;
        mx = b > mx ? b : mx;
        sum += __shfl_down(sum, o, kWave);
    }
    if (lane0) { s_min[wv] = mn; s_max[wv] = mx; s_sum[wv] = sum; }
    __syncthreads();
    for (int w = 0; w < 4; ++w) {
        mn = w == 0 ? s_min[0] : (s_min[w] < mn ? s_min[w] : mn);
        mx = w == 0 ? s_max[0] : (s_max[w] > mx ? s_max[w] : mx);
    }
    {
        const int w0_line = mn & ~31;
        const int64_t span_l = (int64_t)mx + 1 - w0_line;
        const int64_t span4 = (int64_t)mx + 1 - (mn & ~3);
        const int64_t passes = (span4 + region - 1) / region;
        const int lines = (int)((span_l + 31) >> 5);
        const int cost_staged = passes > maxpass ? cost.unstaged
                                : (span4 < 65536 ? cost.c16_base + cost.c16_pass * (int)passes
                                                 : cost.c32_base + cost.c32_pass * (int)passes);
        const int rows_here = lb[c + 1] - lb[c];
        int longest = 0;
        {
            const int64_t lim = base + n;
            for (int t = threadIdx.x; t <= rows_here; t += 256) {
                const int64_t a = t == 0 ? base : (int64_t)row_ptr[lb[c] + t - 1];
                int64_t b = t == 0 ? (int64_t)row_ptr[lb[c]] : (int64_t)row_ptr[lb[c] + t];
                b = b < lim ? b : lim;
                const int len = (int)(b - (a > base ? a : base));
                longest = len > longest ? len : longest;
            }
#pragma unroll
            for (int o = kWave / 2; o > 0; o >>= 1) {
                const int v = __shfl_down(longest, o, kWave);
                longest = v > longest ? v : longest;
            }
            __syncthreads();
            if (lane0) s_cnt[wv] = longest;
            __syncthreads();
            longest = s_cnt[0];
            for (int w = 1; w < 4; ++w) longest = s_cnt[w] > longest ? s_cnt[w] : longest;
        }
        const int cost_sorted = cost.sorted_base + (int)((int64_t)(chunk >= 16384 ? cost.sorted_line_1024 : cost.sorted_line_512) * lines / chunk) -
                                (rows_here <= 16 ? cost.sorted_few_rows : 0);
        const bool eligible = sorted_from != 0 && n == chunk && span_l <= sorted_span;
        const bool long_row_rule = longest > cost.long_piece && passes >= 3;
        const bool sort = eligible && (sorted_from > 0 ? span_l > (int64_t)region * (sorted_from - 1)
                                                       : (cost_sorted < cost_staged || long_row_rule));
        if (threadIdx.x == 0) {
            atomicAdd(reinterpret_cast<unsigned long long *>(stats + 4), (unsigned long long)(sort ? cost_sorted : cost_staged));
            if (long_row_rule) atomicAdd(&stats[3], 1);
        }
        if (sort) {
            if (threadIdx.x == 0) {
                win[2 * c] = w0_line;
                win[2 * c + 1] = kSortedBit;
                atomicAdd(&stats[2], 1);
            }
            return;
        }
    }
    const int w0_full = mn & ~3;
    const int64_t span = (int64_t)mx + 1 - w0_full;
    if (span <= (int64_t)region * maxpass) {
        if (threadIdx.x == 0) {
            win[2 * c] = w0_full;
            win[2 * c + 1] = (int32_t)span;
            if (span <= region) atomicAdd(&stats[0], 1);
            atomicAdd(&stats[1], 1);
        }
        return;
    }
    if (threadIdx.x == 0) {
        const long long tot = s_sum[0] + s_sum[1] + s_sum[2] + s_sum[3];
        long long w0 = tot / (n > 0 ? n : 1) - region / 2;
        if (w0 > cols - region) w0 = cols - region;
        if (w0 < 0) w0 = 0;
        s_w0 = (int)(w0 & ~3ll);
    }
    __syncthreads();
    const int w0 = s_w0;
    int cnt = 0;
    for (int i = threadIdx.x; i < n; i += 256) cnt += ((unsigned)(col_idx[base + i] - w0) < (unsigned)region) ? 1 : 0;
#pragma unroll
    for (int o = kWave / 2; o > 0; o >>= 1) cnt += __shfl_down(cnt, o, kWave);
    if (lane0) s_cnt[wv] = cnt;
    __syncthreads();
    if (threadIdx.x == 0) {
        cnt = s_cnt[0] + s_cnt[1] + s_cnt[2] + s_cnt[3];
        const bool stage = 4 * (int64_t)cnt >= n;
        int64_t wl = region;
        if (w0 + wl > cols) wl = cols - w0;
        win[2 * c] = w0;
        win[2 * c + 1] = stage ? ((int32_t)wl | kOutsideBit) : 0;
    }
}

struct Segment {
    int s, e;
    float *dst;
};

__device__ __forceinline__ Segment make_segment(int t, int lb0, int64_t base, int64_t lim, int32_t rb, int32_t re,
                                                float *__restrict__ y, float *__restrict__ carry, int c)
{
    Segment g;
    if (t == 0) {
        g.s = 0;
        g.e = (int)(((int64_t)rb < lim ? (int64_t)rb : lim) - base);
        g.dst = carry + c;
    } else {
        g.s = (int)((int64_t)rb - base);
        g.e = (int)(((int64_t)re < lim ? (int64_t)re : lim) - base);
        g.dst = y + ((int64_t)lb0 + t - 1);
    }
    return g;
}

template <int BLOCK>
struct ChunkShared {
    int2 long_seg[max_long(BLOCK)];
    int2 huge_seg[max_huge(BLOCK)];
    int long_count, huge_count;
};

template <int BLOCK, bool PREF>
__device__ __forceinline__ void reduce_chunk(const float *smem, ChunkShared<BLOCK> &sh, int tid, int c, int lb0, int m,
                                             int64_t base, int64_t lim, const int32_t *__restrict__ row_ptr,
                                             float *__restrict__ y, float *__restrict__ carry, int32_t rb0, int32_t re0)
{
    for (int t = tid; t <= m; t += BLOCK) {
        int32_t rb, re;
        if (PREF && t == tid) { rb = rb0; re = re0; }
        else { rb = row_ptr[t == 0 ? lb0 : lb0 + t - 1]; re = t == 0 ? 0 : row_ptr[lb0 + t]; }
        const Segment g = make_segment(t, lb0, base, lim, rb, re, y, carry, c);
        const int ps = pad_idx(g.s), pe = pad_idx(g.e);
        if (g.e - g.s <= kShortSeg) {
            float acc = 0.0f;
            const float *w = smem + ps;
            int i = 0;
            const int n = pe - ps;
            for (; i + 3 < n; i += 4) {
                const float a0 = w[i], a1 = w[i + 1], a2 = w[i + 2], a3 = w[i + 3];
                acc = (((acc + a0) + a1) + a2) + a3;
            }
            for (; i < n; ++i) acc += w[i];
            *g.dst = acc;
        } else if (g.e - g.s <= kHugeSeg) {
            const int slot = atomicAdd(&sh.long_count, 1);
            sh.long_seg[slot] = make_int2(t, ps | (pe << 16));
        } else {
            const int slot = atomicAdd(&sh.huge_count, 1);
            sh.huge_seg[slot] = make_int2(t, ps | (pe << 16));
        }
    }
    __syncthreads();

    const int nlong = sh.long_count;
    const int sub = tid & (kGroup - 1);
    for (int i = tid / kGroup; i < nlong; i += BLOCK / kGroup) {
        const int2 q = sh.long_seg[i];
        const int qe = (int)((unsigned)q.y >> 16);
        float acc = 0.0f;
        for (int k = (q.y & 0xffff) + sub; k < qe; k += kGroup) acc += smem[k];
#pragma unroll
        for (int o = kGroup / 2; o > 0; o >>= 1) acc += __shfl_down(acc, o, kGroup);
        if (sub == 0) {
            if (q.x == 0) carry[c] = acc;
            else y[(int64_t)lb0 + q.x - 1] = acc;
        }
    }

    const int nhuge = sh.huge_count;
    const int lane = tid & (kWave - 1);
    for (int i = tid >> 6; i < nhuge; i += BLOCK / kWave) {
        const int2 q = sh.huge_seg[i];
        const int qe = (int)((unsigned)q.y >> 16);
        float a0 = 0.0f, a1 = 0.0f;
        int k = (q.y & 0xffff) + lane;
        for (; k + kWave < qe; k += 2 * kWave) {
            a0 += smem[k];
            a1 += smem[k + kWave];
        }
        if (k < qe) a0 += smem[k];
        float acc = a0 + a1;
#pragma unroll
        for (int o = kWave / 2; o > 0; o >>= 1) acc += __shfl_down(acc, o, kWave);
        if (lane == 0) {
            if (q.x == 0) carry[c] = acc;
            else y[(int64_t)lb0 + q.x - 1] = acc;
        }
    }
}

template <int BLOCK, bool FULL_ONLY>
__device__ __forceinline__ void load_stream(int64_t base, int n, int pad_col, const int32_t *__restrict__ col_idx,
                                            const float *__restrict__ vals, int tid, i4 (&cc)[kNnzPerThread / 4],
                                            f4 (&vv)[kNnzPerThread / 4])
{
    constexpr int kVec = kNnzPerThread / 4;
    if (FULL_ONLY || n == chunk_of(BLOCK)) {
        const i4 *c4 = reinterpret_cast<const i4 *>(col_idx + base);
        const f4 *v4 = reinterpret_cast<const f4 *>(vals + base);
#pragma unroll
        for (int j = 0; j < kVec; ++j) {
            cc[j] = __builtin_nontemporal_load(&c4[j * BLOCK + tid]);
            vv[j] = __builtin_nontemporal_load(&v4[j * BLOCK + tid]);
        }
    } else {
#pragma unroll
        for (int j = 0; j < kVec; ++j) {
            const int i0 = (j * BLOCK + tid) * 4;
#pragma unroll
            for (int q = 0; q < 4; ++q) {
                const bool ok = (i0 + q) < n;
                cc[j][q] = ok ? col_idx[base + i0 + q] : pad_col;
                vv[j][q] = ok ? vals[base + i0 + q] : 0.0f;
            }
        }
    }
}

struct Walk {
    int c, end, stride;
};

__device__ __forceinline__ Walk first_chunk(bool persist, int bid, int grid, int nchunks)
{
    Walk w;
    if (!persist) {
        w.c = xcd_chunk(bid, nchunks);
        w.end = w.c + 1;
        w.stride = 1;
        return w;
    }
    const int j = bid % kXcds, i = bid / kXcds;
    const int q = nchunks / kXcds, rem = nchunks % kXcds;
    const int start = j * q + (j < rem ? j : rem);
    const int cnt = q + (j < rem ? 1 : 0);
    w.stride = grid / kXcds + (j < grid % kXcds ? 1 : 0);
    w.c = start + i;
    w.end = start + cnt;
    return w;
}

__host__ __device__ constexpr int waves_per_simd(int block, bool persist) { return !persist ? 8 : (block == 1024 ? 4 : 6); }

template <int BLOCK, bool DMA>
__device__ __forceinline__ void stage_slice(const float *__restrict__ x, int64_t g0, int len, int64_t cols, float *smem,
                                            int tid)
{
    if (g0 + len + 3 < cols) {
        for (int i = tid * 4; i < len; i += BLOCK * 4) {
            if (DMA) __builtin_amdgcn_global_load_lds(x + g0 + i, smem + i, 16, 0, 0);
            else *reinterpret_cast<f4 *>(smem + i) = *reinterpret_cast<const f4 *>(x + g0 + i);
        }
    } else {
        for (int i = tid * 4; i < len; i += BLOCK * 4) {
#pragma unroll
            for (int q = 0; q < 4; ++q)
                if (g0 + i + q < cols) smem[i + q] = x[g0 + i + q];
        }
    }
}

template <int BLOCK>
__device__ __forceinline__ void stage_blocks(const float *__restrict__ x, const int32_t *__restrict__ ids, int nb,
                                             int64_t cols, float *smem, int tid)
{
    const int lane = tid & (kWave - 1);
    for (int b = __builtin_amdgcn_readfirstlane(tid >> 6); b < nb; b += BLOCK / kWave) {
        const int64_t g = (int64_t)ids[b] * kBlkCols;
        float *dst = smem + b * kBlkCols;
        if (g + kBlkCols + 3 < cols) {
            const float *src = x + g + lane * 4;
#pragma unroll 1
            for (int q = 0; q < kBlkCols / (kWave * 4); ++q)
                __builtin_amdgcn_global_load_lds(src + q * kWave * 4, dst + (q * kWave + lane) * 4, 16, 0, 0);
        } else {
            for (int i = lane; i < kBlkCols; i += kWave)
                if (g + i < cols) dst[i] = x[g + i];
        }
    }
}

template <int BLOCK, bool TILED, bool PERSIST>
__device__ __forceinline__ void adaptive_body(float *smem, ChunkShared<BLOCK> &sh, int bid, int grid, int64_t rows,
                                              int64_t nnz, int64_t cols, int chunk0, int nrun,
                                              const int32_t *__restrict__ row_ptr,
                                              const int32_t *__restrict__ col_idx, const float *__restrict__ vals,
                                              const float *__restrict__ x, float *__restrict__ y,
                                              const int32_t *__restrict__ chunk_lb, float *__restrict__ carry,
                                              const int32_t *__restrict__ win, const int32_t *__restrict__ list,
                                              int kRegion)
{
    constexpr int kChunkT = chunk_of(BLOCK);
    constexpr int kVec = kNnzPerThread / 4;

    const int tid0 = threadIdx.x;
    Walk wk = first_chunk(PERSIST, bid, grid, nrun);
    if (wk.c >= wk.end) return;
    if (!PERSIST && list) {
        wk.c = list[wk.c];
        wk.end = wk.c + 1;
    } else {
        wk.c += chunk0;
        wk.end += chunk0;
    }

    i4 cc[kVec];
    f4 vv[kVec];
    {
        const int64_t b0 = (int64_t)wk.c * kChunkT;
        const int n0 = (int)((nnz - b0) < kChunkT ? (nnz - b0) : kChunkT);
        load_stream<BLOCK, PERSIST>(b0, n0, TILED ? win[2 * wk.c] : 0, col_idx, vals, tid0, cc, vv);
    }

    for (;;) {
        int tid = tid0;
        if (PERSIST) asm volatile("" : "+v"(tid));
        const int c = wk.c;
        const int64_t base = (int64_t)c * kChunkT;
        const int n = (int)((nnz - base) < kChunkT ? (nnz - base) : kChunkT);
        const int64_t lim = base + n;
        if (tid == 0) { sh.long_count = 0; sh.huge_count = 0; }

        const int lb0 = chunk_lb[c], lb1 = chunk_lb[c + 1];
        const int m = lb1 - lb0;
        int w0 = 0, wlen = 0;
        bool outside = false;
        if (TILED) {
            w0 = win[2 * c];
            const int wl = win[2 * c + 1];
            wlen = wl & kLenMask;
            outside = (wl & kOutsideBit) != 0;
        }

        int32_t rb0 = 0, re0 = 0;
        if (!TILED && tid <= m) {
            rb0 = row_ptr[tid == 0 ? lb0 : lb0 + tid - 1];
            re0 = tid == 0 ? 0 : row_ptr[lb0 + tid];
        }

        f4 xv[kVec];
        if (TILED && wlen > 0) {
#pragma unroll
            for (int j = 0; j < kVec; ++j)
#pragma unroll
                for (int q = 0; q < 4; ++q) xv[j][q] = 0.0f;
            if (outside) {
#pragma unroll
                for (int j = 0; j < kVec; ++j)
#pragma unroll
                    for (int q = 0; q < 4; ++q)
                        if ((unsigned)(cc[j][q] - w0) >= (unsigned)wlen) xv[j][q] = x[cc[j][q]];
            }
            for (int off = 0; off < wlen; off += kRegion) {
                const int len = (wlen - off) < kRegion ? (wlen - off) : kRegion;
                const int64_t g0 = (int64_t)w0 + off;
                stage_slice<BLOCK, true>(x, g0, len, cols, smem, tid);
                __syncthreads();
#pragma unroll
                for (int j = 0; j < kVec; ++j)
#pragma unroll
                    for (int q = 0; q < 4; ++q) {
                        const unsigned o = (unsigned)(cc[j][q] - w0 - off);
                        if (o < (unsigned)len) xv[j][q] = smem[o];
                    }
                __syncthreads();
            }
        } else {
#pragma unroll
            for (int j = 0; j < kVec; ++j)
#pragma unroll
                for (int q = 0; q < 4; ++q) xv[j][q] = x[cc[j][q]];
        }

        zero_pad_words<BLOCK>(smem, tid);
#pragma unroll
        for (int j = 0; j < kVec; ++j) {
            const int p0 = pad_idx((j * BLOCK + tid) * 4);
            smem[p0] = vv[j][0] * xv[j][0];
            smem[p0 + 1] = vv[j][1] * xv[j][1];
            smem[p0 + 2] = vv[j][2] * xv[j][2];
            smem[p0 + 3] = vv[j][3] * xv[j][3];
        }

        const int cn = c + wk.stride;
        const bool more = PERSIST && cn < wk.end;
        if (more) {
            const int64_t bn = (int64_t)cn * kChunkT;
            const int nn = (int)((nnz - bn) < kChunkT ? (nnz - bn) : kChunkT);
            load_stream<BLOCK, PERSIST>(bn, nn, TILED ? win[2 * cn] : 0, col_idx, vals, tid, cc, vv);
        }
        __syncthreads();

        reduce_chunk<BLOCK, !TILED>(smem, sh, tid, c, lb0, m, base, lim, row_ptr, y, carry, rb0, re0);

        if (!more) break;
        __syncthreads();
        wk.c = cn;
    }
}

template <int BLOCK, bool TILED, bool PERSIST>
__global__ __launch_bounds__(BLOCK, waves_per_simd(BLOCK, PERSIST))
void k_adaptive(int64_t rows, int64_t nnz, int64_t cols, int chunk0, int nrun, const int32_t *__restrict__ row_ptr,
                const int32_t *__restrict__ col_idx, const float *__restrict__ vals, const float *__restrict__ x,
                float *__restrict__ y, const int32_t *__restrict__ chunk_lb, float *__restrict__ carry,
                const int32_t *__restrict__ win, const int32_t *__restrict__ list, int kRegion)
{
    extern __shared__ __attribute__((aligned(16))) float smem[];
    __shared__ ChunkShared<BLOCK> sh;
    adaptive_body<BLOCK, TILED, PERSIST>(smem, sh, (int)blockIdx.x, (int)gridDim.x, rows, nnz, cols, chunk0, nrun, row_ptr,
                                         col_idx, vals, x, y, chunk_lb, carry, win, list, kRegion);
}

using u4 = unsigned __attribute__((ext_vector_type(4)));

template <int BLOCK, bool BLOCKS>
__device__ __forceinline__ void tiled16_body(float *smem, ChunkShared<BLOCK> &sh, int bid, int64_t rows, int64_t cols,
                                             int nrun, const int32_t *__restrict__ row_ptr,
                                             const uint16_t *__restrict__ col16, const float *__restrict__ vals,
                                             const float *__restrict__ x, float *__restrict__ y,
                                             const int32_t *__restrict__ chunk_lb, float *__restrict__ carry,
                                             const int32_t *__restrict__ win, const int32_t *__restrict__ list,
                                             int kRegionArg, const int32_t *__restrict__ blk)
{
    constexpr int kChunkT = chunk_of(BLOCK);
    constexpr int kVec = kNnzPerThread / 4;
    static_assert(kNnzPerThread == 16, "the col16 lane layout is two 16-byte loads of eight offsets");

    const int tid = threadIdx.x;
    const int ci = xcd_chunk(bid, nrun);
    const int c = list ? list[ci] : ci;
    const int64_t base = (int64_t)c * kChunkT;
    const int64_t lim = base + kChunkT;
    if (tid == 0) { sh.long_count = 0; sh.huge_count = 0; }
    const int lb0 = chunk_lb[c], lb1 = chunk_lb[c + 1];
    const int m = lb1 - lb0;
    const int w0 = win[2 * c];
    const int wl = win[2 * c + 1];
    const int wlen = wl & kLenMask;
    const bool by_blocks = BLOCKS && (wl & kBlockBit);
    const int kRegion = by_blocks ? (kRegionArg / kBlkCols) * kBlkCols : kRegionArg;

    u4 raw[2];
    f4 vv[kVec];
    {
        const u4 *c8 = reinterpret_cast<const u4 *>(col16 + base);
        const f4 *v4 = reinterpret_cast<const f4 *>(vals + base);
        raw[0] = __builtin_nontemporal_load(&c8[tid]);
        raw[1] = __builtin_nontemporal_load(&c8[BLOCK + tid]);
#pragma unroll
        for (int j = 0; j < kVec; ++j) vv[j] = __builtin_nontemporal_load(&v4[j * BLOCK + tid]);
    }

    int32_t rb0 = 0, re0 = 0;
    if (tid <= m) {
        rb0 = row_ptr[tid == 0 ? lb0 : lb0 + tid - 1];
        re0 = tid == 0 ? 0 : row_ptr[lb0 + tid];
    }

    f4 xv[kVec];
#pragma unroll
    for (int j = 0; j < kVec; ++j)
#pragma unroll
        for (int q = 0; q < 4; ++q) xv[j][q] = 0.0f;
#ifndef SPMV_T_NOSTAGE
    if (wlen <= kRegion && wlen > 0) {
        if (by_blocks) stage_blocks<BLOCK>(x, blk + (int64_t)c * kBlkMax, wlen / kBlkCols, cols, smem, tid);
        else stage_slice<BLOCK, true>(x, (int64_t)w0, wlen, cols, smem, tid);
        __syncthreads();
#pragma unroll
        for (int j = 0; j < kVec; ++j)
#pragma unroll
            for (int q = 0; q < 4; ++q) {
                const int e = (j & 1) * 4 + q;
                const unsigned word = raw[j >> 1][e >> 1];
                xv[j][q] = smem[(e & 1) ? (word >> 16) : (word & 0xffffu)];
            }
        __syncthreads();
    } else
#endif
#ifdef SPMV_T_NOSTAGE
    for (int off = 0; off < 0; off += kRegion) {
#else
    for (int off = 0; off < wlen; off += kRegion) {
#endif
        const int len = (wlen - off) < kRegion ? (wlen - off) : kRegion;
        const int64_t g0 = (int64_t)w0 + off;
        if (by_blocks) stage_blocks<BLOCK>(x, blk + (int64_t)c * kBlkMax + off / kBlkCols, len / kBlkCols, cols, smem, tid);
        else stage_slice<BLOCK, true>(x, g0, len, cols, smem, tid);
        __syncthreads();
#pragma unroll
        for (int j = 0; j < kVec; ++j)
#pragma unroll
            for (int q = 0; q < 4; ++q) {
                const int e = (j & 1) * 4 + q;
                const unsigned word = raw[j >> 1][e >> 1];
                const unsigned cl = (e & 1) ? (word >> 16) : (word & 0xffffu);
                const unsigned o = cl - (unsigned)off;
                if (o < (unsigned)len) xv[j][q] = smem[o];
            }
        __syncthreads();
    }

    zero_pad_words<BLOCK>(smem, tid);
#pragma unroll
    for (int j = 0; j < kVec; ++j) {
        const int p0 = pad_idx((j * BLOCK + tid) * 4);
        smem[p0] = vv[j][0] * xv[j][0];
        smem[p0 + 1] = vv[j][1] * xv[j][1];
        smem[p0 + 2] = vv[j][2] * xv[j][2];
        smem[p0 + 3] = vv[j][3] * xv[j][3];
    }
    __syncthreads();
#ifdef SPMV_T_NOREDUCE
    if (tid <= m && rb0 == 0x7fffffff) y[lb0 + tid] = smem[tid] + (float)re0;
#else
    reduce_chunk<BLOCK, true>(smem, sh, tid, c, lb0, m, base, lim, row_ptr, y, carry, rb0, re0);
#endif
}

template <int BLOCK, bool BLOCKS>
__global__ __launch_bounds__(BLOCK, 8) void k_tiled16(int64_t rows, int64_t cols, int nrun,
                                                      const int32_t *__restrict__ row_ptr,
                                                      const uint16_t *__restrict__ col16,
                                                      const float *__restrict__ vals,
                                                      const float *__restrict__ x, float *__restrict__ y,
                                                      const int32_t *__restrict__ chunk_lb,
                                                      float *__restrict__ carry,
                                                      const int32_t *__restrict__ win,
                                                      const int32_t *__restrict__ list, int kRegion,
                                                      const int32_t *__restrict__ blk)
{
    extern __shared__ __attribute__((aligned(16))) float smem[];
    __shared__ ChunkShared<BLOCK> sh;
    tiled16_body<BLOCK, BLOCKS>(smem, sh, (int)blockIdx.x, rows, cols, nrun, row_ptr, col16, vals, x, y, chunk_lb, carry, win,
                                list, kRegion, blk);
}

template <int BLOCK>
__device__ __forceinline__ void sorted_body(float *smem, ChunkShared<BLOCK> &sh, int bid, int64_t rows, int nrun,
                                            const int32_t *__restrict__ row_ptr, const uint32_t *__restrict__ perm,
                                            const float *__restrict__ vals, const float *__restrict__ x,
                                            float *__restrict__ y, const int32_t *__restrict__ chunk_lb,
                                            float *__restrict__ carry, const int32_t *__restrict__ win,
                                            const int32_t *__restrict__ list)
{
    constexpr int kChunkT = chunk_of(BLOCK);
    constexpr int kVec = kNnzPerThread / 4;
    constexpr int kColBits = sorted_col_bits(BLOCK);
    constexpr unsigned kColMask = (1u << kColBits) - 1u;

    const int tid = threadIdx.x;
    const int ci = xcd_chunk(bid, nrun);
    const int c = list[ci];
    const int64_t base = (int64_t)c * kChunkT;
    const int64_t lim = base + kChunkT;
    if (tid == 0) { sh.long_count = 0; sh.huge_count = 0; }
    const int lb0 = chunk_lb[c], lb1 = chunk_lb[c + 1];
    const int m = lb1 - lb0;
    const float *xw = x + win[2 * c];

    u4 pw[kVec];
    f4 vv[kVec];
    {
        const u4 *p4 = reinterpret_cast<const u4 *>(perm + (int64_t)ci * kChunkT);
        const f4 *v4 = reinterpret_cast<const f4 *>(vals + base);
#ifdef SPMV_SORTED_FAKE7
#pragma unroll
        for (int j = 0; j < kVec - 1; ++j) pw[j] = __builtin_nontemporal_load(&p4[j * BLOCK + tid]);
        for (int q = 0; q < 4; ++q) pw[kVec - 1][q] = (pw[kVec - 2][q] ^ (1u << kColBits)) + 37u;
#else
#pragma unroll
        for (int j = 0; j < kVec; ++j) pw[j] = __builtin_nontemporal_load(&p4[j * BLOCK + tid]);
#endif
#pragma unroll
        for (int j = 0; j < kVec; ++j) vv[j] = __builtin_nontemporal_load(&v4[j * BLOCK + tid]);
    }
    int32_t rb0 = 0, re0 = 0;
    if (tid <= m) {
        rb0 = row_ptr[tid == 0 ? lb0 : lb0 + tid - 1];
        re0 = tid == 0 ? 0 : row_ptr[lb0 + tid];
    }

#pragma unroll
    for (int j = 0; j < kVec; ++j) {
        float g[4];
#pragma unroll
        for (int q = 0; q < 4; ++q) g[q] = xw[pw[j][q] & kColMask];
#pragma unroll
        for (int q = 0; q < 4; ++q) smem[pad_idx((int)(pw[j][q] >> kColBits))] = g[q];
    }
    __syncthreads();
    zero_pad_words<BLOCK>(smem, tid);
#pragma unroll
    for (int j = 0; j < kVec; ++j) {
        const int p0 = pad_idx((j * BLOCK + tid) * 4);
        smem[p0] = vv[j][0] * smem[p0];
        smem[p0 + 1] = vv[j][1] * smem[p0 + 1];
        smem[p0 + 2] = vv[j][2] * smem[p0 + 2];
        smem[p0 + 3] = vv[j][3] * smem[p0 + 3];
    }
    __syncthreads();
    reduce_chunk<BLOCK, true>(smem, sh, tid, c, lb0, m, base, lim, row_ptr, y, carry, rb0, re0);
}

template <int BLOCK>
__global__ __launch_bounds__(BLOCK, 8) void k_sorted(int64_t rows, int nrun, const int32_t *__restrict__ row_ptr,
                                                     const uint32_t *__restrict__ perm, const float *__restrict__ vals,
                                                     const float *__restrict__ x, float *__restrict__ y,
                                                     const int32_t *__restrict__ chunk_lb, float *__restrict__ carry,
                                                     const int32_t *__restrict__ win, const int32_t *__restrict__ list)
{
    extern __shared__ __attribute__((aligned(16))) float smem[];
    __shared__ ChunkShared<BLOCK> sh;
    sorted_body<BLOCK>(smem, sh, (int)blockIdx.x, rows, nrun, row_ptr, perm, vals, x, y, chunk_lb, carry, win, list);
}

template <int BLOCK>
__global__ __launch_bounds__(BLOCK) void k_plan_sorted(const int32_t *__restrict__ col_idx,
                                                       const int32_t *__restrict__ win, const int32_t *__restrict__ slot,
                                                       uint32_t *__restrict__ perm)
{
    constexpr int kChunkT = chunk_of(BLOCK);
    constexpr int kColBits = sorted_col_bits(BLOCK);
    constexpr int kLines = 1 << (kColBits - 5);
    constexpr int kPer = kLines / BLOCK;
    static_assert(kLines % BLOCK == 0, "bins per thread");
    __shared__ int hist[kLines];
    __shared__ int part[BLOCK];
    const int c = blockIdx.x, tid = threadIdx.x;
    if (!(win[2 * c + 1] & kSortedBit)) return;
    const int w0 = win[2 * c];
    const int64_t base = (int64_t)c * kChunkT;
    uint32_t *out = perm + (int64_t)slot[c] * kChunkT;
    for (int i = tid; i < kLines; i += BLOCK) hist[i] = 0;
    __syncthreads();
    for (int i = tid; i < kChunkT; i += BLOCK) atomicAdd(&hist[(col_idx[base + i] - w0) >> 5], 1);
    __syncthreads();
    int sum = 0;
#pragma unroll
    for (int k = 0; k < kPer; ++k) sum += hist[tid * kPer + k];
    part[tid] = sum;
    __syncthreads();
    for (int o = 1; o < BLOCK; o <<= 1) {
        const int v = tid >= o ? part[tid - o] : 0;
        __syncthreads();
        part[tid] += v;
        __syncthreads();
    }
    int run = part[tid] - sum;
#pragma unroll
    for (int k = 0; k < kPer; ++k) {
        const int v = hist[tid * kPer + k];
        hist[tid * kPer + k] = run;
        run += v;
    }
    __syncthreads();
    for (int i = tid; i < kChunkT; i += BLOCK) {
        const int off = col_idx[base + i] - w0;
        const int d = atomicAdd(&hist[off >> 5], 1);
        const int t = d % BLOCK, jq = d / BLOCK;
        out[((jq >> 2) * BLOCK + t) * 4 + (jq & 3)] = ((unsigned)i << kColBits) | (unsigned)off;
    }
}

template <int BLOCK, bool BLOCKS>
__global__ __launch_bounds__(BLOCK, 8) void k_tiled_mixed(int64_t rows, int64_t nnz, int64_t cols, int n32, int nsorted,
                                                          int n16, const int32_t *__restrict__ row_ptr,
                                                          const int32_t *__restrict__ col_idx,
                                                          const uint16_t *__restrict__ col16,
                                                          const uint32_t *__restrict__ perm,
                                                          const float *__restrict__ vals,
                                                          const float *__restrict__ x, float *__restrict__ y,
                                                          const int32_t *__restrict__ chunk_lb,
                                                          float *__restrict__ carry,
                                                          const int32_t *__restrict__ win,
                                                          const int32_t *__restrict__ list32,
                                                          const int32_t *__restrict__ list_sorted,
                                                          const int32_t *__restrict__ list16, int kRegion,
                                                          const int32_t *__restrict__ blk)
{
    extern __shared__ __attribute__((aligned(16))) float smem[];
    __shared__ ChunkShared<BLOCK> sh;
    const int b = (int)blockIdx.x;
    if (b < n32)
        adaptive_body<BLOCK, true, false>(smem, sh, b, n32, rows, nnz, cols, 0, n32, row_ptr, col_idx, vals, x,
                                          y, chunk_lb, carry, win, list32, kRegion);
    else if (b < n32 + nsorted)
        sorted_body<BLOCK>(smem, sh, b - n32, rows, nsorted, row_ptr, perm, vals, x, y, chunk_lb, carry, win, list_sorted);
    else
        tiled16_body<BLOCK, BLOCKS>(smem, sh, b - n32 - nsorted, rows, cols, n16, row_ptr, col16, vals, x, y, chunk_lb,
                                    carry, win, list16, kRegion, blk);
}

template <int BLOCK>
__global__ __launch_bounds__(BLOCK) void k_plan_col16(int64_t nnz, const int32_t *__restrict__ col_idx,
                                                      int32_t *__restrict__ win, uint16_t *__restrict__ col16,
                                                      int32_t *__restrict__ flags, int region, int maxpass,
                                                      int32_t *__restrict__ blk, int32_t *__restrict__ blk_chunks,
                                                      int dry)
{
    constexpr int kChunkT = chunk_of(BLOCK);
    __shared__ int s_min, s_max, s_total;
    __shared__ unsigned bits[BLOCK];
    __shared__ int pref[BLOCK];
    const int c = blockIdx.x, tid = threadIdx.x;
    const int64_t base = (int64_t)c * kChunkT;
    const int wl = win[2 * c + 1];
    const int wlen = wl & kLenMask;
    const bool full_chunk = (nnz - base) >= kChunkT;
    const bool contiguous = full_chunk && wlen > 0 && wlen < 65536 && !(wl & kOutsideBit);
    const int w0 = win[2 * c];
    if (tid == 0) { s_min = INT_MAX; s_max = -1; }
    __syncthreads();

    bool by_blocks = false;
    if (full_chunk && blk && !(contiguous && wlen <= region)) {
        int bmin = INT_MAX, bmax = -1;
        for (int i = tid; i < kChunkT; i += BLOCK) {
            const int b = col_idx[base + i] >> kBlkBits;
            bmin = b < bmin ? b : bmin;
            bmax = b > bmax ? b : bmax;
        }
        atomicMin(&s_min, bmin);
        atomicMax(&s_max, bmax);
        bits[tid] = 0u;
        __syncthreads();
        const int lo = s_min;
        if (s_max - lo < 32 * BLOCK) {
            for (int i = tid; i < kChunkT; i += BLOCK) {
                const int d = (col_idx[base + i] >> kBlkBits) - lo;
                atomicOr(&bits[d >> 5], 1u << (d & 31));
            }
            __syncthreads();
            const int mine = __popc(bits[tid]);
            pref[tid] = mine;
            __syncthreads();
            for (int o = 1; o < BLOCK; o <<= 1) {
                const int v = tid >= o ? pref[tid - o] : 0;
                __syncthreads();
                pref[tid] += v;
                __syncthreads();
            }
            if (tid == BLOCK - 1) s_total = pref[tid];
            const int before = pref[tid] - mine;
            __syncthreads();
            pref[tid] = before;
            __syncthreads();
            const int total = s_total;
            const int cap = (region / kBlkCols) * kBlkCols;
            by_blocks = total <= kBlkMax && total * kBlkCols <= cap && (!contiguous || total * kBlkCols < wlen);
            (void)maxpass;
            if (by_blocks && dry) {
                if (tid == 0) atomicAdd(blk_chunks, 1);
                return;
            }
            if (by_blocks) {
                unsigned w = bits[tid];
                int slot = before;
                while (w) {
                    const int j = __ffs(w) - 1;
                    w &= w - 1;
                    blk[(int64_t)c * kBlkMax + slot++] = lo + tid * 32 + j;
                }
                if (tid == 0) {
                    flags[c] = 1;
                    win[2 * c + 1] = (total * kBlkCols) | kCol16Bit | kBlockBit;
                    atomicAdd(blk_chunks, 1);
                }
                u4 *out = reinterpret_cast<u4 *>(col16 + base);
#pragma unroll
                for (int k = 0; k < 2; ++k) {
                    unsigned v[8];
#pragma unroll
                    for (int e = 0; e < 8; ++e) {
                        const int jj = 2 * k + (e >> 2), q = e & 3;
                        const int col = col_idx[base + (jj * BLOCK + tid) * 4 + q];
                        const int d = (col >> kBlkBits) - lo;
                        const int sl = pref[d >> 5] + __popc(bits[d >> 5] & ((1u << (d & 31)) - 1u));
                        v[e] = (unsigned)(sl * kBlkCols + (col & (kBlkCols - 1)));
                    }
                    u4 wv;
#pragma unroll
                    for (int i = 0; i < 4; ++i) wv[i] = v[2 * i] | (v[2 * i + 1] << 16);
                    out[k * BLOCK + tid] = wv;
                }
            }
        }
    }
    if (by_blocks || dry) return;

    if (tid == 0) {
        flags[c] = contiguous ? 1 : 0;
        if (contiguous) win[2 * c + 1] = wl | kCol16Bit;
    }
    if (!contiguous) return;
    u4 *out = reinterpret_cast<u4 *>(col16 + base);
#pragma unroll
    for (int k = 0; k < 2; ++k) {
        unsigned v[8];
#pragma unroll
        for (int e = 0; e < 8; ++e) {
            const int j = 2 * k + (e >> 2), q = e & 3;
            v[e] = (unsigned)(col_idx[base + (j * BLOCK + tid) * 4 + q] - w0);
        }
        u4 w;
#pragma unroll
        for (int i = 0; i < 4; ++i) w[i] = v[2 * i] | (v[2 * i + 1] << 16);
        out[k * BLOCK + tid] = w;
    }
}

__global__ void k_plan_unblock(int nchunks, int32_t *__restrict__ win)
{
    const int c = blockIdx.x * blockDim.x + threadIdx.x;
    if (c >= nchunks) return;
    const int wl = win[2 * c + 1];
    if (wl & kBlockBit) win[2 * c + 1] = 0;
    else if (wl & kCol16Bit) win[2 * c + 1] = wl & ~kCol16Bit;
}

__global__ void k_plan_kinds(int nchunks, const int32_t *__restrict__ win, int32_t *__restrict__ f16,
                             int32_t *__restrict__ fs)
{
    const int c = blockIdx.x * blockDim.x + threadIdx.x;
    if (c >= nchunks) return;
    const int wl = win[2 * c + 1];
    f16[c] = (wl & kCol16Bit) ? 1 : 0;
    fs[c] = (!(wl & kCol16Bit) && (wl & kSortedBit)) ? 1 : 0;
}

__global__ void k_plan_lists(int nchunks, const int32_t *__restrict__ win, const int32_t *__restrict__ p16,
                             const int32_t *__restrict__ ps, int32_t *__restrict__ list16,
                             int32_t *__restrict__ list_sorted, int32_t *__restrict__ list32)
{
    const int c = blockIdx.x * blockDim.x + threadIdx.x;
    if (c >= nchunks) return;
    const int wl = win[2 * c + 1];
    if (wl & kCol16Bit) list16[p16[c]] = c;
    else if (wl & kSortedBit) list_sorted[ps[c]] = c;
    else list32[c - p16[c] - ps[c]] = c;
}

__global__ void k_carry_fixup(int nchunks, int chunk, const int32_t *__restrict__ row_ptr,
                              const int32_t *__restrict__ chunk_lb, const float *__restrict__ carry,
                              float *__restrict__ y)
{
    int c = blockIdx.x * blockDim.x + threadIdx.x;
    if (c >= nchunks - 1) return;
    const int lb0 = chunk_lb[c], lb1 = chunk_lb[c + 1];
    if (lb1 == lb0) return;
    const int64_t r = (int64_t)lb1 - 1;
    const int64_t endp = row_ptr[r + 1];
    if (endp <= (int64_t)(c + 1) * chunk) return;
    float s = y[r];
    for (int64_t c2 = c + 1; c2 * chunk < endp; ++c2) s += carry[c2];
    y[r] = s;
}

__global__ void k_plan_spans(int nchunks, int chunk, const int32_t *__restrict__ row_ptr,
                             const int32_t *__restrict__ chunk_lb, int32_t *__restrict__ count)
{
    int c = blockIdx.x * blockDim.x + threadIdx.x;
    if (c >= nchunks - 1) return;
    const int lb0 = chunk_lb[c], lb1 = chunk_lb[c + 1];
    if (lb1 == lb0) return;
    if ((int64_t)row_ptr[lb1] > (int64_t)(c + 1) * chunk) atomicAdd(count, 1);
}

static int default_passes(int block) { return block == 1024 ? 12 : (block == 512 ? 4 : 2); }


static int build_plan_impl(const spmv_csr &h, int block, int maxpass, hipStream_t s, ChunkPlan &p, int *single, int *full);

static int build_plan(const spmv_csr &h, int block, int maxpass, hipStream_t s, ChunkPlan &p, int *single, int *full)
{
    const int rc = build_plan_impl(h, block, maxpass, s, p, single, full);
    if (rc) p = ChunkPlan{};
    return rc;
}

static int build_plan_impl(const spmv_csr &h, int block, int maxpass, hipStream_t s, ChunkPlan &p, int *single, int *full)
{
    const bool windows = maxpass > 0;
    p = ChunkPlan{};
    p.block = block;
    p.maxpass = maxpass;
    p.region = region_words(block);
    if (const char *e = getenv("SPMV_PERSIST")) p.persist = atoi(e) != 0;
    p.sorted_from = windows && !p.persist ? kSortedFromDefault : 0;
    if (const char *e = getenv("SPMV_SORTED_FROM")) {
        const int v = atoi(e);
        if (windows && !p.persist && v >= -1 && v <= 64) p.sorted_from = v;
    }
    PlanCost cost;
    if (const char *e = getenv("SPMV_PLAN_COST")) {
        int v[10];
        const int got = sscanf(e, "%d,%d,%d,%d,%d,%d,%d,%d,%d,%d", &v[0], &v[1], &v[2], &v[3], &v[4], &v[5], &v[6], &v[7], &v[8], &v[9]);
        if (got >= 9) {
            cost.c16_base = v[0]; cost.c16_pass = v[1]; cost.c32_base = v[2]; cost.c32_pass = v[3];
            cost.sorted_base = v[4]; cost.sorted_line_512 = v[5]; cost.sorted_line_1024 = v[6]; cost.sorted_few_rows = v[7];
            cost.unstaged = v[8];
            if (got == 10) cost.long_piece = v[9];
        }
    }
    const int chunk = chunk_of(block);
    p.nchunks = (int)((h.nnz + chunk - 1) / chunk);
    if (single) *single = 0;
    if (full) *full = 0;
    if (p.nchunks == 0) return SPMV_OK;
    SPMV_HIP_TRY(p.d_lb.alloc((size_t)p.nchunks + 1));
    SPMV_HIP_TRY(p.d_carry.alloc((size_t)p.nchunks));
    hipLaunchKernelGGL(k_plan_chunks, dim3((p.nchunks + 1 + 255) / 256), dim3(256), 0, s, h.rows, p.nchunks, chunk,
                       h.d_row_ptr, p.d_lb);
    int rc = check_launch("k_plan_chunks");
    if (rc) return rc;
    {
        DevPtr<int32_t> cnt;
        SPMV_HIP_TRY(cnt.alloc(1));
        SPMV_HIP_TRY(hipMemsetAsync(cnt.get(), 0, sizeof(int32_t), s));
        if (p.nchunks > 1) {
            hipLaunchKernelGGL(k_plan_spans, dim3((p.nchunks - 1 + 255) / 256), dim3(256), 0, s, p.nchunks, chunk,
                               h.d_row_ptr, p.d_lb, cnt.get());
            if ((rc = check_launch("k_plan_spans"))) return rc;
        }
        int32_t spans = 0;
        SPMV_HIP_TRY(hipMemcpyAsync(&spans, cnt.get(), sizeof(int32_t), hipMemcpyDeviceToHost, s));
        SPMV_HIP_TRY(hipStreamSynchronize(s));
        p.spanning_rows = spans;
    }
    if (windows) {
        SPMV_HIP_TRY(p.d_win.alloc(2 * (size_t)p.nchunks + 6));
        int32_t *d_stats = p.d_win + 2 * (size_t)p.nchunks;
        SPMV_HIP_TRY(hipMemsetAsync(d_stats, 0, 6 * sizeof(int32_t), s));
        hipLaunchKernelGGL(k_plan_windows, dim3(p.nchunks), dim3(256), 0, s, h.nnz, h.cols, p.nchunks, chunk,
                           h.d_col_idx, p.d_win, d_stats, p.region, maxpass, p.sorted_from, 1 << sorted_col_bits(block),
                           cost, p.d_lb, h.d_row_ptr);
        if ((rc = check_launch("k_plan_windows"))) return rc;
        int32_t stats[6] = {0, 0, 0, 0, 0, 0};
        SPMV_HIP_TRY(hipMemcpyAsync(stats, d_stats, sizeof stats, hipMemcpyDeviceToHost, s));
        SPMV_HIP_TRY(hipStreamSynchronize(s));
        p.staged_single = stats[0];
        p.staged_full = stats[1];
        p.nsorted_marked = stats[2];
        p.long_piece_chunks = stats[3];
        uint64_t total_cost;
        memcpy(&total_cost, &stats[4], sizeof total_cost);
        p.model_cost = (double)total_cost * (double)chunk / 1024.0 / (double)(h.nnz > 0 ? h.nnz : 1);
        if (single) *single = stats[0];
        if (full) *full = stats[1];
    }
    return SPMV_OK;
}

template <int BLOCK>
static int launch_plan_col16(const spmv_csr &h, ChunkPlan &p, int32_t *d_flags, int32_t *d_blk_chunks, const int32_t *d_blk_arg,
                             int dry, hipStream_t s)
{
    hipLaunchKernelGGL((k_plan_col16<BLOCK>), dim3(p.nchunks), dim3(BLOCK), 0, s, h.nnz, h.d_col_idx, p.d_win, p.d_col16,
                       d_flags, p.region, p.maxpass, const_cast<int32_t *>(d_blk_arg), d_blk_chunks, dry);
    return check_launch("k_plan_col16");
}

static int build_col16(const spmv_csr &h, ChunkPlan &p, hipStream_t s)
{
    p.col16_wanted = true;
    if (p.nchunks == 0 || !p.d_win || p.persist) return SPMV_OK;
    if (const char *e = getenv("SPMV_COL16")) {
        if (atoi(e) == 0) return SPMV_OK;
    }
    const size_t chunk = (size_t)chunk_of(p.block);
    DevPtr<int32_t> flags, pos, total;
    SPMV_HIP_TRY(flags.alloc((size_t)p.nchunks));
    SPMV_HIP_TRY(pos.alloc((size_t)p.nchunks));
    SPMV_HIP_TRY(total.alloc(1));
    SPMV_HIP_TRY(p.d_col16.alloc(chunk * (size_t)p.nchunks));
    bool want_blocks = true;
    if (const char *e = getenv("SPMV_BLOCKS")) want_blocks = atoi(e) != 0;
    DevPtr<int32_t> nblk;
    SPMV_HIP_TRY(nblk.alloc(1));
    SPMV_HIP_TRY(hipMemsetAsync(nblk.get(), 0, sizeof(int32_t), s));
    if (want_blocks) SPMV_HIP_TRY(p.d_blk.alloc((size_t)kBlkMax * (size_t)p.nchunks));
    int rc;
    auto run = [&](const int32_t *blk_arg, int dry) {
        if (p.block == 256) return launch_plan_col16<256>(h, p, flags.get(), nblk.get(), blk_arg, dry, s);
        if (p.block == 512) return launch_plan_col16<512>(h, p, flags.get(), nblk.get(), blk_arg, dry, s);
        return launch_plan_col16<1024>(h, p, flags.get(), nblk.get(), blk_arg, dry, s);
    };
    if (want_blocks) {
        if ((rc = run(p.d_blk, 1))) return rc;
        int32_t cand = 0;
        SPMV_HIP_TRY(hipMemcpyAsync(&cand, nblk.get(), sizeof(int32_t), hipMemcpyDeviceToHost, s));
        SPMV_HIP_TRY(hipStreamSynchronize(s));
        if (4 * (int64_t)cand < p.nchunks) (void)p.d_blk.reset();
        SPMV_HIP_TRY(hipMemsetAsync(nblk.get(), 0, sizeof(int32_t), s));
    }
    if ((rc = run(p.d_blk, 0))) return rc;
    SPMV_HIP_TRY(hipMemcpyAsync(pos.get(), flags.get(), sizeof(int32_t) * (size_t)p.nchunks, hipMemcpyDeviceToDevice, s));
    if ((rc = exclusive_scan_i32(pos.get(), p.nchunks, total.get(), s))) return rc;
    int32_t n16 = 0, nb = 0;
    SPMV_HIP_TRY(hipMemcpyAsync(&n16, total.get(), sizeof(int32_t), hipMemcpyDeviceToHost, s));
    SPMV_HIP_TRY(hipMemcpyAsync(&nb, nblk.get(), sizeof(int32_t), hipMemcpyDeviceToHost, s));
    SPMV_HIP_TRY(hipStreamSynchronize(s));
    p.nblk_chunks = nb;
    if (nb == 0) (void)p.d_blk.reset();
    if (2 * ((int64_t)n16 + p.nsorted_marked) < p.nchunks) {
        hipLaunchKernelGGL(k_plan_unblock, dim3((p.nchunks + 255) / 256), dim3(256), 0, s, p.nchunks, p.d_win);
        if ((rc = check_launch("k_plan_unblock"))) return rc;
        SPMV_HIP_TRY(hipStreamSynchronize(s));
        p.nblk_chunks = 0;
        (void)p.d_col16.reset();
        (void)p.d_blk.reset();
    }
    return SPMV_OK;
}

static int count_block_list_chunks(const spmv_csr &h, ChunkPlan &p, hipStream_t s, int *out)
{
    *out = 0;
    if (p.nchunks == 0 || !p.d_win) return SPMV_OK;
    DevPtr<int32_t> nblk, some;
    SPMV_HIP_TRY(nblk.alloc(1));
    SPMV_HIP_TRY(some.alloc(1));
    SPMV_HIP_TRY(hipMemsetAsync(nblk.get(), 0, sizeof(int32_t), s));
    int rc;
    if (p.block == 256) rc = launch_plan_col16<256>(h, p, nullptr, nblk.get(), some.get(), 1, s);
    else if (p.block == 512) rc = launch_plan_col16<512>(h, p, nullptr, nblk.get(), some.get(), 1, s);
    else rc = launch_plan_col16<1024>(h, p, nullptr, nblk.get(), some.get(), 1, s);
    if (rc) return rc;
    int32_t cnt = 0;
    SPMV_HIP_TRY(hipMemcpyAsync(&cnt, nblk.get(), sizeof cnt, hipMemcpyDeviceToHost, s));
    SPMV_HIP_TRY(hipStreamSynchronize(s));
    *out = cnt;
    return SPMV_OK;
}

template <int BLOCK>
static int launch_plan_sorted(const spmv_csr &h, ChunkPlan &p, const int32_t *d_slot, hipStream_t s)
{
    hipLaunchKernelGGL((k_plan_sorted<BLOCK>), dim3(p.nchunks), dim3(BLOCK), 0, s, h.d_col_idx, p.d_win, d_slot, p.d_perm);
    return check_launch("k_plan_sorted");
}

static int build_lists(const spmv_csr &h, ChunkPlan &p, hipStream_t s)
{
    (void)p.d_list16.reset();
    (void)p.d_list32.reset();
    (void)p.d_list_sorted.reset();
    (void)p.d_perm.reset();
    p.n16 = p.nsorted = 0;
    if (p.nchunks == 0 || !p.d_win || p.persist) return SPMV_OK;
    int rc;
    DevPtr<int32_t> f16, fs, t16, ts;
    SPMV_HIP_TRY(f16.alloc((size_t)p.nchunks));
    SPMV_HIP_TRY(fs.alloc((size_t)p.nchunks));
    SPMV_HIP_TRY(t16.alloc(1));
    SPMV_HIP_TRY(ts.alloc(1));
    const unsigned g = (unsigned)((p.nchunks + 255) / 256);
    hipLaunchKernelGGL(k_plan_kinds, dim3(g), dim3(256), 0, s, p.nchunks, p.d_win, f16.get(), fs.get());
    if ((rc = check_launch("k_plan_kinds"))) return rc;
    if ((rc = exclusive_scan_i32(f16.get(), p.nchunks, t16.get(), s))) return rc;
    if ((rc = exclusive_scan_i32(fs.get(), p.nchunks, ts.get(), s))) return rc;
    int32_t n16 = 0, ns = 0;
    SPMV_HIP_TRY(hipMemcpyAsync(&n16, t16.get(), sizeof(int32_t), hipMemcpyDeviceToHost, s));
    SPMV_HIP_TRY(hipMemcpyAsync(&ns, ts.get(), sizeof(int32_t), hipMemcpyDeviceToHost, s));
    SPMV_HIP_TRY(hipStreamSynchronize(s));
    p.n16 = n16;
    p.nsorted = ns;
    if (n16 == 0 && ns == 0) return SPMV_OK;
    SPMV_HIP_TRY(p.d_list16.alloc((size_t)n16));
    SPMV_HIP_TRY(p.d_list_sorted.alloc((size_t)ns));
    SPMV_HIP_TRY(p.d_list32.alloc((size_t)(p.nchunks - n16 - ns)));
    hipLaunchKernelGGL(k_plan_lists, dim3(g), dim3(256), 0, s, p.nchunks, p.d_win, f16.get(), fs.get(), p.d_list16, p.d_list_sorted,
                       p.d_list32);
    if ((rc = check_launch("k_plan_lists"))) return rc;
    if (ns > 0) {
        SPMV_HIP_TRY(p.d_perm.alloc((size_t)chunk_of(p.block) * (size_t)ns));
        if (p.block == 256) rc = launch_plan_sorted<256>(h, p, fs.get(), s);
        else if (p.block == 512) rc = launch_plan_sorted<512>(h, p, fs.get(), s);
        else rc = launch_plan_sorted<1024>(h, p, fs.get(), s);
        if (rc) return rc;
    }
    SPMV_HIP_TRY(hipStreamSynchronize(s));
    return SPMV_OK;
}

int launch_adaptive(const spmv_csr &h, const float *x, float *y, bool tiled, hipStream_t s);

static int finish_tiled(spmv_csr &h, bool col16, hipStream_t s)
{
    int rc = col16 ? build_col16(h, h.plan_tiled, s) : SPMV_OK;
    if (rc == SPMV_OK) rc = build_lists(h, h.plan_tiled, s);
    if (rc) h.plan_tiled = ChunkPlan{};
    return rc;
}

int plan_tiled_with(spmv_csr &h, int block, int maxpass, bool col16, hipStream_t s)
{
    if ((block != 256 && block != 512 && block != 1024) || maxpass < 1 || maxpass > 64) {
        set_error("tiled plan: block %d / maxpass %d outside 256|512|1024 / 1..64", block, maxpass);
        return SPMV_ERR_INVALID;
    }
    int rc = build_plan(h, block, maxpass, s, h.plan_tiled, nullptr, nullptr);
    if (rc == SPMV_OK && col16) rc = build_col16(h, h.plan_tiled, s);
    if (rc == SPMV_OK) rc = build_lists(h, h.plan_tiled, s);
    if (rc) h.plan_tiled = ChunkPlan{};
    return rc;
}

int plan_adaptive_with(spmv_csr &h, int block, hipStream_t s)
{
    if (block != 256) {
        set_error("adaptive plan: block %d (only 256)", block);
        return SPMV_ERR_INVALID;
    }
    return build_plan(h, 256, 0, s, h.plan_adaptive, nullptr, nullptr);
}

int plan_adaptive(spmv_csr &h, bool tiled, hipStream_t s)
{
    if (!tiled) {
        if (h.plan_adaptive.block) return SPMV_OK;
        return build_plan(h, 256, 0, s, h.plan_adaptive, nullptr, nullptr);
    }
    if (h.plan_tiled.block) return SPMV_OK;

    int forced = 0, forced_pass = 0;
    if (const char *e = getenv("SPMV_TILED_BLOCK")) forced = atoi(e);
    if (forced != 256 && forced != 512 && forced != 1024) forced = 0;
    if (const char *e = getenv("SPMV_MAXPASS")) forced_pass = atoi(e);
    if (forced_pass < 1 || forced_pass > 64) forced_pass = 0;
    if (forced) {
        int rc = build_plan(h, forced, forced_pass ? forced_pass : default_passes(forced), s, h.plan_tiled, nullptr, nullptr);
        return rc ? rc : finish_tiled(h, true, s);
    }

    bool autotune = false;
    if (const char *e = getenv("SPMV_AUTOTUNE")) autotune = atoi(e) != 0 && h.nnz >= (1 << 20);
    if (!autotune) {
        const int cands[3] = {256, 512, 1024};
        for (int k = 0; k < 3; ++k) {
            int single = 0, full = 0;
            int rc = build_plan(h, cands[k], default_passes(cands[k]), s, h.plan_tiled, &single, &full);
            if (rc) return rc;
            if (h.plan_tiled.nchunks == 0 || single >= 0.9 * h.plan_tiled.nchunks) return finish_tiled(h, true, s);
        }
        {
            bool want_blocks = true;
            if (const char *e = getenv("SPMV_BLOCKS")) want_blocks = atoi(e) != 0;
            for (int k = 0; k < 3 && want_blocks; ++k) {
                int rc = build_plan(h, cands[k], default_passes(cands[k]), s, h.plan_tiled, nullptr, nullptr);
                if (rc) return rc;
                int lists = 0;
                if ((rc = count_block_list_chunks(h, h.plan_tiled, s, &lists))) { h.plan_tiled = ChunkPlan{}; return rc; }
                if (lists >= 0.9 * h.plan_tiled.nchunks) return finish_tiled(h, true, s);
            }
        }
        int rc = build_plan(h, 1024, 12, s, h.plan_tiled, nullptr, nullptr);
        if (rc) return rc;
        const double cost1024 = h.plan_tiled.model_cost * 1.03;
        const ChunkPlan &q = h.plan_tiled;
        const bool long_rows = 2 * (int64_t)q.long_piece_chunks >= (int64_t)q.nchunks - q.staged_single;
        if ((rc = build_plan(h, 512, 8, s, h.plan_tiled, nullptr, nullptr))) return rc;
        if (!long_rows && cost1024 < h.plan_tiled.model_cost && (rc = build_plan(h, 1024, 12, s, h.plan_tiled, nullptr, nullptr)))
            return rc;
        return finish_tiled(h, true, s);
    }

    struct Cand { int block, maxpass; };
    const Cand cands[] = {{256, 2}, {512, 4}, {512, 8}, {1024, 6}, {1024, 12}};
    {
        const Cand widest[] = {{1024, 12}, {512, 8}, {256, 2}};
        bool any = false;
        for (const Cand &c : widest) {
            int single = 0, full = 0;
            int rc0 = build_plan(h, c.block, c.maxpass, s, h.plan_tiled, &single, &full);
            if (rc0) return rc0;
            if (h.plan_tiled.nchunks == 0 || full > 0 || h.plan_tiled.nsorted_marked > 0) { any = true; break; }
        }
        if (!any) {
            int rc0 = build_plan(h, 512, 8, s, h.plan_tiled, nullptr, nullptr);
            if (rc0 == SPMV_OK) rc0 = build_col16(h, h.plan_tiled, s);
            if (rc0) return rc0;
            any = h.plan_tiled.nblk_chunks > 0;
        }
        if (!any) return build_plan(h, 256, 2, s, h.plan_tiled, nullptr, nullptr);
    }
    DevPtr<float> xt, yt;
    SPMV_HIP_TRY(xt.alloc((size_t)h.cols));
    SPMV_HIP_TRY(yt.alloc((size_t)h.rows));
    SPMV_HIP_TRY(hipMemsetAsync(xt.get(), 0, sizeof(float) * (size_t)(h.cols ? h.cols : 1), s));
    hipEvent_t e0, e1;
    SPMV_HIP_TRY(hipEventCreate(&e0));
    SPMV_HIP_TRY(hipEventCreate(&e1));
    struct Pick { int block = 0, maxpass = 0, narrow = 0, single = 0, chunks = 0; float ms = 0.0f; bool set = false; };
    Pick best, second;
    int rc = SPMV_OK;
    auto time_plan = [&](int reps, int launches, float &ms) -> int {
        int r = SPMV_OK;
        for (int i = 0; i < 2 && r == SPMV_OK; ++i) r = launch_adaptive(h, xt.get(), yt.get(), true, s);
        bool timed = true;
        for (int rep = 0; rep < reps && timed && r == SPMV_OK; ++rep) {
            timed = hipEventRecord(e0, s) == hipSuccess;
            for (int i = 0; i < launches && r == SPMV_OK; ++i) r = launch_adaptive(h, xt.get(), yt.get(), true, s);
            timed = timed && hipEventRecord(e1, s) == hipSuccess && hipEventSynchronize(e1) == hipSuccess;
            float t = 0.0f;
            timed = timed && hipEventElapsedTime(&t, e0, e1) == hipSuccess;
            t /= (float)launches;
            if (rep == 0 || t < ms) ms = t;
        }
        return r ? r : (timed ? SPMV_OK : SPMV_ERR_HIP);
    };
    for (const Cand &c : cands) {
        ChunkPlan &p = h.plan_tiled;
        int single = 0, full = 0;
        if ((rc = build_plan(h, c.block, c.maxpass, s, p, &single, &full))) break;
        if (p.nchunks == 0) break;
        for (int narrow = 0; narrow < 2 && rc == SPMV_OK; ++narrow) {
            if (narrow) {
                if ((rc = build_col16(h, p, s))) break;
                if (!p.d_col16) break;
            }
            if ((rc = build_lists(h, p, s))) break;
            float ms = 0.0f;
            if ((rc = time_plan(3, 2, ms))) break;
            Pick cur;
            cur.block = c.block; cur.maxpass = c.maxpass; cur.narrow = narrow; cur.single = single; cur.chunks = p.nchunks;
            cur.ms = ms; cur.set = true;
            if (getenv("SPMV_AUTOTUNE_LOG"))
                fprintf(stderr, "[spmv autotune] block=%d maxpass=%d col16=%d: %.4f ms\n", c.block, c.maxpass, narrow, ms);
            if (!best.set || ms < best.ms) { second = best; best = cur; }
            else if (!second.set || ms < second.ms) second = cur;
        }
        if (rc) break;
        if (best.single == best.chunks && best.block == c.block) break;
    }
    if (rc == SPMV_OK && best.set && second.set && second.ms <= 1.08f * best.ms) {
        Pick *both[2] = {&best, &second};
        for (Pick *q : both) {
            if ((rc = build_plan(h, q->block, q->maxpass, s, h.plan_tiled, nullptr, nullptr))) break;
            if ((rc = finish_tiled(h, q->narrow != 0, s))) break;
            if ((rc = time_plan(4, 4, q->ms))) break;
            if (getenv("SPMV_AUTOTUNE_LOG"))
                fprintf(stderr, "[spmv autotune] rematch block=%d maxpass=%d col16=%d: %.4f ms\n", q->block, q->maxpass,
                        q->narrow, q->ms);
        }
        if (rc == SPMV_OK && second.ms < best.ms) best = second;
    }
    (void)hipEventDestroy(e0);
    (void)hipEventDestroy(e1);
    if (rc) { h.plan_tiled = ChunkPlan{}; return rc; }
    if (!best.set) return SPMV_OK;
    if ((rc = build_plan(h, best.block, best.maxpass, s, h.plan_tiled, nullptr, nullptr))) return rc;
    return finish_tiled(h, best.narrow != 0, s);
}

static int resident_workgroups(int device, int block, int waves_simd)
{
    int per_cu = (waves_simd * 4 * kWave) / block;
    if (per_cu < 1) per_cu = 1;
    return device_cus(device) * per_cu;
}

template <int BLOCK, bool TILED, bool PERSIST>
static int launch_range(const spmv_csr &h, const ChunkPlan &p, int chunk0, int nrun, const float *x, float *y,
                        hipStream_t s, const int32_t *list = nullptr)
{
    if (nrun <= 0) return SPMV_OK;
    const size_t lds = sizeof(float) * (size_t)p.region;
    static LdsOptIn optin;
    if (int rc = optin.ensure(reinterpret_cast<const void *>(&k_adaptive<BLOCK, TILED, PERSIST>), h.device, (int)lds)) return rc;
    int grid = nrun;
    if (PERSIST) {
        const int res = resident_workgroups(h.device, BLOCK, waves_per_simd(BLOCK, true));
        if (grid > res) grid = res;
    }
    hipLaunchKernelGGL((k_adaptive<BLOCK, TILED, PERSIST>), dim3(grid), dim3(BLOCK), lds, s, h.rows, h.nnz, h.cols,
                       chunk0, nrun, h.d_row_ptr, h.d_col_idx, h.d_vals, x, y, p.d_lb, p.d_carry, p.d_win, list, p.region);
    return check_launch("k_adaptive");
}

template <int BLOCK, bool BLOCKS>
static int launch_tiled16_t(const spmv_csr &h, const ChunkPlan &p, const float *x, float *y, hipStream_t s)
{
    const size_t lds = sizeof(float) * (size_t)p.region;
    static LdsOptIn optin;
    if (int rc = optin.ensure(reinterpret_cast<const void *>(&k_tiled16<BLOCK, BLOCKS>), h.device, (int)lds)) return rc;
    hipLaunchKernelGGL((k_tiled16<BLOCK, BLOCKS>), dim3(p.n16), dim3(BLOCK), lds, s, h.rows, h.cols, p.n16, h.d_row_ptr,
                       p.d_col16, h.d_vals, x, y, p.d_lb, p.d_carry, p.d_win,
                       p.n16 == p.nchunks ? (const int32_t *)nullptr : p.d_list16, p.region, p.d_blk);
    return check_launch("k_tiled16");
}

template <int BLOCK>
static int launch_tiled16(const spmv_csr &h, const ChunkPlan &p, const float *x, float *y, hipStream_t s)
{
    if (p.n16 <= 0) return SPMV_OK;
    return p.nblk_chunks > 0 ? launch_tiled16_t<BLOCK, true>(h, p, x, y, s) : launch_tiled16_t<BLOCK, false>(h, p, x, y, s);
}

template <int BLOCK, bool BLOCKS>
static int launch_mixed_t(const spmv_csr &h, const ChunkPlan &p, const float *x, float *y, hipStream_t s)
{
    const size_t lds = sizeof(float) * (size_t)p.region;
    static LdsOptIn optin;
    if (int rc = optin.ensure(reinterpret_cast<const void *>(&k_tiled_mixed<BLOCK, BLOCKS>), h.device, (int)lds)) return rc;
    const int n32 = p.nchunks - p.n16 - p.nsorted;
    hipLaunchKernelGGL((k_tiled_mixed<BLOCK, BLOCKS>), dim3(p.nchunks), dim3(BLOCK), lds, s, h.rows, h.nnz, h.cols, n32,
                       p.nsorted, p.n16, h.d_row_ptr, h.d_col_idx, p.d_col16, p.d_perm, h.d_vals, x, y, p.d_lb, p.d_carry,
                       p.d_win, p.d_list32, p.d_list_sorted, p.d_list16, p.region, p.d_blk);
    return check_launch("k_tiled_mixed");
}

template <int BLOCK>
static int launch_mixed(const spmv_csr &h, const ChunkPlan &p, const float *x, float *y, hipStream_t s)
{
    return p.nblk_chunks > 0 ? launch_mixed_t<BLOCK, true>(h, p, x, y, s) : launch_mixed_t<BLOCK, false>(h, p, x, y, s);
}

template <int BLOCK>
static int launch_sorted(const spmv_csr &h, const ChunkPlan &p, const float *x, float *y, hipStream_t s)
{
    const size_t lds = sizeof(float) * (size_t)p.region;
    static LdsOptIn optin;
    if (int rc = optin.ensure(reinterpret_cast<const void *>(&k_sorted<BLOCK>), h.device, (int)lds)) return rc;
    hipLaunchKernelGGL((k_sorted<BLOCK>), dim3(p.nsorted), dim3(BLOCK), lds, s, h.rows, p.nsorted, h.d_row_ptr, p.d_perm,
                       h.d_vals, x, y, p.d_lb, p.d_carry, p.d_win, p.d_list_sorted);
    return check_launch("k_sorted");
}

template <int BLOCK, bool TILED>
static int launch_either(bool persist, const spmv_csr &h, const ChunkPlan &p, const float *x, float *y, hipStream_t s)
{
    if constexpr (TILED) {
        if (!persist && (p.n16 > 0 || p.nsorted > 0)) {
            if (p.n16 == p.nchunks) return launch_tiled16<BLOCK>(h, p, x, y, s);
            if (p.nsorted == p.nchunks) return launch_sorted<BLOCK>(h, p, x, y, s);
            return launch_mixed<BLOCK>(h, p, x, y, s);
        }
    }
    if (!persist) return launch_range<BLOCK, TILED, false>(h, p, 0, p.nchunks, x, y, s);
    const int nfull = (int)(h.nnz / chunk_of(BLOCK));
    int rc = launch_range<BLOCK, TILED, true>(h, p, 0, nfull, x, y, s);
    if (rc == SPMV_OK && p.nchunks > nfull) rc = launch_range<BLOCK, TILED, false>(h, p, nfull, p.nchunks - nfull, x, y, s);
    return rc;
}

int launch_adaptive(const spmv_csr &h, const float *x, float *y, bool tiled, hipStream_t s)
{
    const ChunkPlan &p = tiled ? h.plan_tiled : h.plan_adaptive;
    if (!p.block) {
        set_error("%s used before spmv_csr_plan", tiled ? "SPMV_TILED" : "SPMV_ADAPTIVE");
        return SPMV_ERR_NOT_PLANNED;
    }
    if (h.rows == 0) return SPMV_OK;
    if (p.nchunks == 0) {
        SPMV_HIP_TRY(hipMemsetAsync(y, 0, sizeof(float) * (size_t)h.rows, s));
        return SPMV_OK;
    }
    const bool persist = p.persist;
    int rc;
    const bool nothing_staged = tiled && p.block == 256 && p.staged_full == 0 && p.n16 == 0 && p.nsorted == 0;
    if (!tiled || nothing_staged) rc = launch_either<256, false>(persist, h, p, x, y, s);
    else if (p.block == 256) rc = launch_either<256, true>(persist, h, p, x, y, s);
    else if (p.block == 512) rc = launch_either<512, true>(persist, h, p, x, y, s);
    else rc = launch_either<1024, true>(persist, h, p, x, y, s);
    if (rc) return rc;
    if (p.nchunks > 1 && p.spanning_rows > 0) {
        hipLaunchKernelGGL(k_carry_fixup, dim3((p.nchunks - 1 + 255) / 256), dim3(256), 0, s, p.nchunks,
                           chunk_of(p.block), h.d_row_ptr, p.d_lb, p.d_carry, y);
        rc = check_launch("k_carry_fixup");
    }
    return rc;
}

}
```

spmv-test_amd/csrc/spmv_internal.hpp:

```cpp
#pragma once
#include <hip/hip_runtime.h>
#include <atomic>
#include <cstdint>
#include <cstdio>
#include <utility>
#include "spmv_hip.h"

namespace spmv {

void set_error(const char *fmt, ...) __attribute__((format(printf, 1, 2)));
int hip_fail(hipError_t e, const char *what, const char *file, int line);

#define SPMV_HIP_TRY(call)                                                   \
    do {                                                                     \
        hipError_t e__ = (call);                                             \
        if (e__ != hipSuccess) return ::spmv::hip_fail(e__, #call, __FILE__, __LINE__); \
    } while (0)

static inline int check_launch(const char *what)
{
    hipError_t e = hipGetLastError();
    if (e != hipSuccess) return hip_fail(e, what, __FILE__, __LINE__);
    return SPMV_OK;
}

template <typename T>
class DevPtr {
    T *p_ = nullptr;
public:
    DevPtr() = default;
    DevPtr(DevPtr &&o) noexcept : p_(o.p_) { o.p_ = nullptr; }
    DevPtr &operator=(DevPtr &&o) noexcept
    {
        T *q = o.p_;
        o.p_ = nullptr;
        (void)reset();
        p_ = q;
        return *this;
    }
    ~DevPtr() { (void)reset(); }
    DevPtr *operator&() = delete;
    hipError_t alloc(size_t count)
    {
        (void)reset();
        return hipMalloc((void **)&p_, sizeof(T) * (count ? count : 1));
    }
    hipError_t reset()
    {
        T *q = p_;
        p_ = nullptr;
        return q ? hipFree(q) : hipSuccess;
    }
    T *get() const { return p_; }
    operator T *() const { return p_; }
};

struct LdsOptIn {
    std::atomic<uint64_t> done{0};
    int ensure(const void *fn, int device, int bytes);
};
int device_cus(int device);
int require_current(int device, const char *what);

constexpr int kWave = 64;
constexpr int kBlock = 256;
constexpr int kXcds = 8;

#ifndef SPMV_T_NPT
#define SPMV_T_NPT 16
#endif
#ifndef SPMV_T_SHORT
#define SPMV_T_SHORT 32
#endif
constexpr int kNnzPerThread = SPMV_T_NPT;
constexpr int kShortSeg = SPMV_T_SHORT;

struct ChunkPlan {
    int block = 0;
    int nchunks = 0;
    DevPtr<int32_t> d_lb;
    DevPtr<float> d_carry;
    DevPtr<int32_t> d_win;
    DevPtr<uint16_t> d_col16;
    DevPtr<int32_t> d_list16;
    DevPtr<int32_t> d_list32;
    int n16 = 0;
    DevPtr<uint32_t> d_perm;
    DevPtr<int32_t> d_list_sorted;
    int nsorted = 0;
    int nsorted_marked = 0;
    int sorted_from = 0;
    int long_piece_chunks = 0;
    double model_cost = 0.0;
    DevPtr<int32_t> d_blk;
    int nblk_chunks = 0;
    int maxpass = 0;
    bool col16_wanted = false;
    int spanning_rows = 0;
    int region = 0;
    bool persist = false;
    int staged_single = 0;
    int staged_full = 0;
};

struct ValuesStamp {
    uint64_t gen = 0;
    uint64_t sum = 0;
    bool have_sum = false;
};

struct PanelPlan {
    bool ready = false;
    bool lds_mode = false;
    int pw_bits = 0;
    int npanels = 0;
    int nblocks = 0;
    int waves_per_launch = 0;
    int step_vecs = 8;
    DevPtr<uint32_t> d_packed;
    DevPtr<float> d_pvals;
    DevPtr<int32_t> d_tile_ptr;
    DevPtr<int32_t> d_brow;
    ValuesStamp stamp;
    bool sorted_mode = false;
    DevPtr<int32_t> d_ubeg;
    DevPtr<int32_t> d_usimple;
    DevPtr<int32_t> d_uend;
    DevPtr<int32_t> d_ubase;
    DevPtr<int32_t> d_tbeg;
    DevPtr<uint16_t> d_trow;
    int64_t tail_units = 0;
    int sb_rows = 0, sb_waves = 0;
    int64_t wide_blocks = 0;
    int64_t units = 0;
    int64_t lines = 0;
    int64_t tail = 0;
    bool binned_mode = false;
    int bin_rows = 0;
    DevPtr<uint16_t> d_c16;
    DevPtr<uint16_t> d_r16;
    DevPtr<int32_t> d_pm;
    DevPtr<int32_t> d_pbase;
    DevPtr<float> d_prod;
    int64_t padded = 0;
    int splits = 1;
    bool wide_pieces = false;
    int flagged_tiles = 0;
    int long_rows = 0;
    DevPtr<int32_t> d_lptr;
    DevPtr<uint32_t> d_lrow;
    DevPtr<int32_t> d_lcnt;
    bool scatter_mode = false;
    DevPtr<int32_t> d_offset;
    DevPtr<int32_t> d_first_run;
    int64_t runs = 0;
    DevPtr<int32_t> d_bbase;
    DevPtr<int32_t> d_bcnt;
    DevPtr<int32_t> d_nlong;
    int64_t bm_entries = 0;
    int64_t bm_alloc = 0;
};

struct XskipPlan {
    bool ready = false;
    int nblocks = 0, nseg = 0, slabs = 0;
    DevPtr<int32_t> d_block_seg;
    DevPtr<int32_t> d_seg_input;
    DevPtr<int32_t> d_seg_ptr;
    DevPtr<uint16_t> d_erow;
    DevPtr<float> d_evals;
    DevPtr<float> d_part;
    ValuesStamp stamp;
};

struct WavePlan {
    bool ready = false;
    int n_long = 0, pieces = 0;
    DevPtr<int32_t> d_long_row;
    DevPtr<int32_t> d_long_first;
    DevPtr<int32_t> d_piece_k0;
    DevPtr<int32_t> d_piece_len;
    DevPtr<float> d_partial;
    int block_rows = 512;
    DevPtr<int32_t> d_blk_lo;
    DevPtr<uint16_t> d_col16;
    DevPtr<int32_t> d_piece_base;
    bool windows = false;
    int64_t blocks = 0, win_blocks = 0;
};

struct SpmmPlan {
    bool ready = false;
    int n_long = 0, pieces = 0;
    int row_cap = 0, piece_len = 0;
    DevPtr<int32_t> d_order;
    DevPtr<int32_t> d_long_row;
    DevPtr<int32_t> d_long_first;
    DevPtr<int32_t> d_piece_k0;
    DevPtr<int32_t> d_piece_len;
    DevPtr<float> d_partial;
};

}


struct spmv_csr {
    int64_t rows = 0, cols = 0, nnz = 0;
    const int32_t *d_row_ptr = nullptr;
    const int32_t *d_col_idx = nullptr;
    const float *d_vals = nullptr;
    spmv::DevPtr<int32_t> own_row_ptr, own_col_idx;
    spmv::DevPtr<float> own_vals;
    spmv::DevPtr<uint32_t> transpose_map;
    int device = 0;

    int vector_width = 0;
    spmv::ChunkPlan plan_adaptive;
    spmv::ChunkPlan plan_tiled;
    spmv::PanelPlan plan_panel;
    spmv::PanelPlan plan_auto_panel;
    bool auto_made_tiled = false;
    spmv::XskipPlan plan_xskip;
    spmv::WavePlan plan_wave;
    spmv::SpmmPlan plan_spmm;
    int auto_variant = -1;
    uint64_t values_gen = 0;
};

struct spmv_tcsr {
    int M = 0, N = 0;
    int64_t nnz = 0, nblocks = 0;
    spmv::DevPtr<int32_t> d_blk_idx;
    spmv::DevPtr<uint32_t> d_bitmaps;
    spmv::DevPtr<float> d_vals;
    int nseg = 0;
    spmv::DevPtr<float> d_partial;
};

struct spmv_bitmap {
    int format = 0;
    int M = 0, N = 0;
    int device = 0;
    int64_t n_bitmaps = 0, n_vals = 0;
    int32_t stats[4] = {0, 0, 0, 0};
    spmv::DevPtr<uint32_t> d_bitmaps;
    spmv::DevPtr<float> d_vals;
    spmv::DevPtr<float> d_partial;
};

namespace spmv {

int launch_scalar(spmv_csr &h, const float *x, float *y, hipStream_t s);
int launch_wave(spmv_csr &h, const float *x, float *y, bool pipelined, hipStream_t s);
int plan_wave(spmv_csr &h, hipStream_t s);
int launch_vector(const spmv_csr &h, const float *x, float *y, hipStream_t s);
int launch_adaptive(const spmv_csr &h, const float *x, float *y, bool tiled, hipStream_t s);
int launch_panel(const spmv_csr &h, const float *x, float *y, hipStream_t s);

int plan_xskip(spmv_csr &h, hipStream_t s);
int launch_xskip(const spmv_csr &h, const float *x, float *y, hipStream_t s);
int plan_panel(spmv_csr &h, hipStream_t s);
int panel_launches(const PanelPlan &p);
int plan_vector(spmv_csr &h, hipStream_t s);
int plan_adaptive(spmv_csr &h, bool tiled, hipStream_t s);
int plan_tiled_with(spmv_csr &h, int block, int maxpass, bool col16, hipStream_t s);
int plan_adaptive_with(spmv_csr &h, int block, hipStream_t s);
int plan_panel_with(spmv_csr &h, int pw_bits, int waves_per_launch, int mode, hipStream_t s);
int build_panel(spmv_csr &h, PanelPlan &dst, int pw_bits, int waves_per_launch, int mode, hipStream_t s);
int refresh_panel(spmv_csr &h, PanelPlan &dst, hipStream_t s);
int launch_panel_plan(const spmv_csr &h, const PanelPlan &p, const float *x, float *y, hipStream_t s);
int panel_row_blocks(const spmv_csr &h, int64_t nb0, int cap, hipStream_t s, DevPtr<int32_t> &brow, int32_t *nblocks);
int panel_rowloc(const spmv_csr &h, const int32_t *d_brow, int nblocks, uint16_t *d_rowloc, hipStream_t s);
int plan_colsort(spmv_csr &h, PanelPlan &p, int want_rows, int want_waves, hipStream_t s);
double colsort_model_cost(const PanelPlan &p, int64_t nnz);
double colsort_cost(int rows_per_block, double lines_per_nnz, double tail_frac);
int colsort_probe(const spmv_csr &h, hipStream_t s, double *long_frac, double *wide_frac, double *lines_per_nnz);
int launch_colsort(const spmv_csr &h, const PanelPlan &p, const float *x, float *y, hipStream_t s);
int panel_tile_ptr(const spmv_csr &h, const int32_t *d_brow, int nblocks, int pw_bits, int np, int32_t *d_tile_ptr, hipStream_t s);
int plan_binned(spmv_csr &h, PanelPlan &p, int want_rows, bool scatter, hipStream_t s);
int launch_binned(const spmv_csr &h, const PanelPlan &p, const float *x, float *y, hipStream_t s);
double binned_tile_nonzeros(const spmv_csr &h, int bin_rows);
int plan_spmm(spmv_csr &h, hipStream_t s);
int launch_spmm(const spmv_csr &h, int k, const float *X, int64_t ldx, float *Y, int64_t ldy, hipStream_t s);
int64_t spmm_plan_bytes(const spmv_csr &h);
int transpose(const spmv_csr &a, bool keep_map, hipStream_t s, spmv_csr_t **out);
int transpose_values(spmv_csr &t, const spmv_csr &a, hipStream_t s);

int dense_to_csr(int M, int N, const float *d_A, hipStream_t s, spmv_csr_t **out);
int dense_gemv(int M, int N, const float *d_A, const float *d_x, float *d_y, int mode, hipStream_t s);
int asp_retile(int M, int N, const float *d_A, float *d_asp, hipStream_t s);
int asp_gemv_ws(int M, int N, const float *d_asp, const float *d_x, float *d_y, void *d_ws, size_t ws_bytes, hipStream_t s);
size_t dense_gemv_workspace_bytes(int N, int mode);
int dense_gemv_ws(int M, int N, const float *d_A, const float *d_x, float *d_y, int mode, void *d_ws, size_t ws_bytes,
                  hipStream_t s);

int launch_validate(const spmv_csr *h, int32_t *d_bad4, hipStream_t stream);
int values_checksum(const spmv_csr &h, hipStream_t s, uint64_t *out);
bool check_values_env();
int stamp_values(const spmv_csr &h, hipStream_t s, ValuesStamp &st);
int require_fresh_values(const spmv_csr &h, const ValuesStamp &st, hipStream_t s, const char *variant);
int launch_column_range(const spmv_csr &h, int32_t *d_out2, hipStream_t s);
int exclusive_scan_i32(int32_t *d_data, int64_t n, int32_t *d_total, hipStream_t s);

int tcsr_from_dense(int M, int N, const float *d_A, hipStream_t s, spmv_tcsr_t **out);
int tcsr_run(const spmv_tcsr &h, const float *d_x, float *d_y, hipStream_t s);
int tcsr_sizes(const spmv_tcsr &h, int64_t *n_blk_idx, int64_t *n_bitmaps, int64_t *n_vals);
int tcsr_download(const spmv_tcsr &h, int32_t *blk_idx, uint32_t *bitmaps, float *vals);
void tcsr_dims(const spmv_tcsr &h, int *M, int *N);

int bitmap_from_dense(int format, int M, int N, const float *d_A, hipStream_t s, spmv_bitmap_t **out);
int bitmap_run(const spmv_bitmap &h, const float *d_x, float *d_y, hipStream_t s);
void bitmap_info(const spmv_bitmap &h, int *format, int *M, int *N, int64_t *n_bitmaps, int64_t *n_vals, int32_t stats[4]);
int bitmap_download(const spmv_bitmap &h, uint32_t *bitmaps, float *vals);
int bitmap_device(const spmv_bitmap &h);

int synth_fill(uint64_t seed, int64_t row0, int64_t n_local, int64_t rows, int64_t cols, int64_t band,
               const int32_t *d_row_ptr, int32_t *d_col_idx, float *d_vals, hipStream_t s);
int synth_x(uint64_t seed, int64_t j0, int64_t n, float *d_x, hipStream_t s);


enum BoundsSite {
    kSiteBsSumsProd = 0, kSiteBsSumsAcc, kSiteBinSumsProd, kSiteBinSumsR16, kSiteBsProductsC16, kSiteBsProductsVals,
    kSiteBsProductsStore, kSiteBsGroupStore, kSiteBsPlaceLoad, kSiteBsPlaceAcc, kSiteBsPlaceC16, kSiteBsFillAcc,
    kSiteBsFillC16, kSitePanelPacked, kSitePanelVals,
    kBoundsSites
};
#if defined(SPMV_CHECK_BOUNDS)
namespace {
__device__ __attribute__((unused)) unsigned long long g_bounds[kBoundsSites][2];
}
#if defined(__HIPCC__)
__device__ __forceinline__ bool bounds_in(int site, int64_t lo, int64_t len, int64_t limit)
{
    if (lo >= 0 && lo + len <= limit) return true;
    atomicAdd(&g_bounds[site][0], 1ull);
    atomicMax(&g_bounds[site][1], (unsigned long long)(lo < 0 ? -lo : lo + len - limit));
    return false;
}
#endif
static inline int bounds_collect_local(unsigned long long out[kBoundsSites][2])
{
    unsigned long long t[kBoundsSites][2] = {};
    SPMV_HIP_TRY(hipDeviceSynchronize());
    SPMV_HIP_TRY(hipMemcpyFromSymbol(t, HIP_SYMBOL(g_bounds), sizeof t));
    const unsigned long long zero[kBoundsSites][2] = {};
    SPMV_HIP_TRY(hipMemcpyToSymbol(HIP_SYMBOL(g_bounds), zero, sizeof zero));
    for (int i = 0; i < kBoundsSites; ++i) {
        out[i][0] += t[i][0];
        if (t[i][1] > out[i][1]) out[i][1] = t[i][1];
    }
    return SPMV_OK;
}
#define SPMV_BOUNDS_LOAD(ok, site, var, lo, len, limit) \
    const bool ok = ::spmv::bounds_in((site), (int64_t)(lo), (int64_t)(len), (int64_t)(limit)); \
    if (!ok) var = 0
#define SPMV_BOUNDS_VALUE(ok, v) ((ok) ? (v) : decltype(v){})
#define SPMV_BOUNDS_BUF(ok, site, voff, soff, len, limit) \
    const bool ok = ::spmv::bounds_in((site), (int64_t)(uint32_t)(voff) + (int64_t)(uint32_t)(soff), (int64_t)(len), (int64_t)(limit)); \
    voff = ok ? voff + soff : 0; \
    soff = 0
#define SPMV_BOUNDS_STORE(site, lo, len, limit) if (::spmv::bounds_in((site), (int64_t)(lo), (int64_t)(len), (int64_t)(limit)))
#else
#define SPMV_BOUNDS_LOAD(ok, site, var, lo, len, limit)
#define SPMV_BOUNDS_VALUE(ok, v) (v)
#define SPMV_BOUNDS_BUF(ok, site, voff, soff, len, limit)
#define SPMV_BOUNDS_STORE(site, lo, len, limit)
#endif
int bounds_collect_binned(unsigned long long out[kBoundsSites][2]);
int bounds_collect_panel(unsigned long long out[kBoundsSites][2]);

#if defined(__HIPCC__)
__device__ __forceinline__ bool lone_in_step(volatile int *tags, bool valid, int key, int lane)
{
    const int slot = key & 255;
    if (valid) tags[slot] = lane;
    __builtin_amdgcn_wave_barrier();
    const int first = valid ? tags[slot] : lane;
    __builtin_amdgcn_wave_barrier();
    if (valid && first != lane) tags[slot] = kWave;
    __builtin_amdgcn_wave_barrier();
    const int second = valid ? tags[slot] : kWave;
    __builtin_amdgcn_wave_barrier();
    return valid && second == lane;
}
#endif

}
```

Measured before the change: 5831 GB/s.

## Fuse carry fixup into chunk kernels via atomic handoff slots, make LDS padding optional

Rows that span chunk boundaries now resolve in-kernel. Each side atomically exchanges its partial sum into a per-boundary 64-bit slot, and whichever arrives second writes y, which removes the separate k_carry_fixup launch and the carry round trip. LDS bank-conflict padding becomes a template parameter chosen at plan time from the row-length histogram. The unpadded path stores products as float4 and uses index arithmetic in the long and huge reductions. Costs include agent-scope atomics per spanning row, slot memory that must be zeroed, and more kernel instantiations.

```diff
diff --git a/include/spmv_hip.h b/include/spmv_hip.h
--- a/include/spmv_hip.h
+++ b/include/spmv_hip.h
@@ -80,6 +80,8 @@
 
 SPMV_API int spmv_csr_plan_describe(const spmv_csr_t *h, int variant, char *buf, int n);
 
+SPMV_API int spmv_csr_plan_modes(const spmv_csr_t *h, int variant, int32_t modes[4]);
+
 SPMV_API int spmv_csr_time(spmv_csr_t *h, int variant, const float *d_x, float *d_y, int iters,
                   void *stream, float *ms_per_launch);
 
diff --git a/spmv-test_amd/capi.py b/spmv-test_amd/capi.py
--- a/spmv-test_amd/capi.py
+++ b/spmv-test_amd/capi.py
@@ -50,6 +50,7 @@
     "spmv_csr_plan_like": (C.c_int, [_H, _H, C.c_int, _vp]),
     "spmv_csr_plan_bytes": (C.c_int64, [_H, C.c_int]),
     "spmv_csr_plan_describe": (C.c_int, [_H, C.c_int, C.c_char_p, C.c_int]),
+    "spmv_csr_plan_modes": (C.c_int, [_H, C.c_int, C.POINTER(C.c_int32)]),
     "spmv_csr_time": (C.c_int, [_H, C.c_int, _f32p, _f32p, C.c_int, _vp, C.POINTER(C.c_float)]),
     "spmv_csr_run_host": (C.c_int, [_H, C.c_int, _f32p, _f32p, C.POINTER(C.c_float)]),
     "spmv_dense_gemv": (C.c_int, [C.c_int, C.c_int, _f32p, _f32p, _f32p, C.c_int, _vp]),
@@ -271,6 +272,11 @@
     def plan_bytes(self, variant: int) -> int:
         return lib().spmv_csr_plan_bytes(self._h, variant)
 
+    def plan_modes(self, variant: int) -> dict:
+        m = (C.c_int32 * 4)()
+        check(lib().spmv_csr_plan_modes(self._h, variant, m))
+        return {"launches": m[0], "fused": bool(m[1]), "padded": bool(m[2]), "long_spans": m[3]}
+
     def download(self):
         import numpy as np
         rp = np.empty(self.rows + 1, np.int32)
diff --git a/spmv-test_amd/csrc/capi.hip b/spmv-test_amd/csrc/capi.hip
--- a/spmv-test_amd/csrc/capi.hip
+++ b/spmv-test_amd/csrc/capi.hip
@@ -726,6 +726,26 @@
     return SPMV_OK;
 }
 
+int spmv_csr_plan_modes(const spmv_csr_t *h, int variant, int32_t modes[4])
+{
+    if (!h || !modes) { set_error("spmv_csr_plan_modes: bad argument"); return SPMV_ERR_INVALID; }
+    if (variant == SPMV_AUTO) variant = h->auto_variant;
+    if (variant != SPMV_ADAPTIVE && variant != SPMV_TILED) {
+        set_error("spmv_csr_plan_modes: variant %d has no chunk plan", variant);
+        return SPMV_ERR_INVALID;
+    }
+    const ChunkPlan &p = variant == SPMV_ADAPTIVE ? h->plan_adaptive : h->plan_tiled;
+    if (!p.block) { set_error("spmv_csr_plan_modes: not planned"); return SPMV_ERR_NOT_PLANNED; }
+    const int64_t chunk = (int64_t)p.block * kNnzPerThread;
+    const bool fixup = !p.fused && p.nchunks > 1 && p.spanning_rows > 0;
+    const bool two_main = p.persist && h->nnz >= chunk && h->nnz % chunk != 0;
+    modes[0] = h->rows == 0 ? 0 : (p.nchunks == 0 ? 1 : 1 + (two_main ? 1 : 0) + (fixup ? 1 : 0));
+    modes[1] = p.fused ? 1 : 0;
+    modes[2] = (p.pad || p.persist || p.nblk_chunks > 0) ? 1 : 0;
+    modes[3] = p.long_spans;
+    return SPMV_OK;
+}
+
 int spmv_csr_time(spmv_csr_t *h, int variant, const float *d_x, float *d_y, int iters, void *stream,
                   float *ms_per_launch)
 {
diff --git a/spmv-test_amd/csrc/kernels_adaptive.hip b/spmv-test_amd/csrc/kernels_adaptive.hip
--- a/spmv-test_amd/csrc/kernels_adaptive.hip
+++ b/spmv-test_amd/csrc/kernels_adaptive.hip
@@ -25,17 +25,27 @@
 constexpr int kHugeSeg = SPMV_T_HUGE;
 __host__ __device__ constexpr int max_huge(int block) { return chunk_of(block) / (kHugeSeg + 1) + 2; }
 
-#ifdef SPMV_T_NOPAD
-__device__ __forceinline__ int pad_idx(int i) { return i; }
-#else
-__device__ __forceinline__ int pad_idx(int i) { return i + (i >> 5); }
-#endif
-template <int BLOCK>
+template <bool PAD>
+__device__ __forceinline__ int pad_idx(int i) { return PAD ? i + (i >> 5) : i; }
+template <int BLOCK, bool PAD>
 __device__ __forceinline__ void zero_pad_words(float *smem, int tid)
 {
-#ifndef SPMV_T_NOPAD
-    for (int h = tid; h < (chunk_of(BLOCK) >> 5); h += BLOCK) smem[h * 33 + 32] = 0.0f;
-#endif
+    if constexpr (PAD)
+        for (int h = tid; h < (chunk_of(BLOCK) >> 5); h += BLOCK) smem[h * 33 + 32] = 0.0f;
+}
+
+template <int BLOCK, bool PAD>
+__device__ __forceinline__ void store_products(float *smem, int tid, int j, f4 prod)
+{
+    const int p0 = pad_idx<PAD>((j * BLOCK + tid) * 4);
+    if constexpr (PAD) {
+        smem[p0] = prod[0];
+        smem[p0 + 1] = prod[1];
+        smem[p0 + 2] = prod[2];
+        smem[p0 + 3] = prod[3];
+    } else {
+        *reinterpret_cast<f4 *>(smem + p0) = prod;
+    }
 }
 
 __device__ __forceinline__ int xcd_chunk(int bid, int n)
@@ -208,21 +218,20 @@
 
 struct Segment {
     int s, e;
-    float *dst;
+    bool spans;
 };
 
-__device__ __forceinline__ Segment make_segment(int t, int lb0, int64_t base, int64_t lim, int32_t rb, int32_t re,
-                                                float *__restrict__ y, float *__restrict__ carry, int c)
+__device__ __forceinline__ Segment make_segment(int t, int64_t base, int64_t lim, int32_t rb, int32_t re)
 {
     Segment g;
     if (t == 0) {
         g.s = 0;
         g.e = (int)(((int64_t)rb < lim ? (int64_t)rb : lim) - base);
-        g.dst = carry + c;
+        g.spans = false;
     } else {
         g.s = (int)((int64_t)rb - base);
         g.e = (int)(((int64_t)re < lim ? (int64_t)re : lim) - base);
-        g.dst = y + ((int64_t)lb0 + t - 1);
+        g.spans = (int64_t)re > lim;
     }
     return g;
 }
@@ -233,18 +242,80 @@
     int2 huge_seg[max_huge(BLOCK)];
     int long_count, huge_count;
 };
-
-template <int BLOCK, bool PREF>
+constexpr int kSpansBit = 1 << 30;
+
+struct Handoff {
+    uint64_t old = 0;
+    float mine = 0.0f;
+    int row = -1;
+};
+
+__device__ __forceinline__ void handoff_issue(Handoff &h, int c, int lb0, uint64_t *__restrict__ slots)
+{
+    if (h.row >= 0)
+        h.old = __hip_atomic_exchange(slots + (h.row >= lb0 ? c + 1 : c), ((uint64_t)1 << 32) | (uint64_t)__float_as_uint(h.mine),
+                                      __ATOMIC_RELAXED, __HIP_MEMORY_SCOPE_AGENT);
+}
+
+__device__ __forceinline__ void handoff_finish(const Handoff &h, int c, int lb0, float *__restrict__ y,
+                                               uint64_t *__restrict__ slots)
+{
+    if (h.row >= 0 && (unsigned)(h.old >> 32) != 0u) {
+        const float other = __uint_as_float((unsigned)h.old);
+        const bool owner = h.row >= lb0;
+        y[h.row] = owner ? h.mine + other : other + h.mine;
+        __hip_atomic_store(slots + (owner ? c + 1 : c), (uint64_t)0, __ATOMIC_RELAXED, __HIP_MEMORY_SCOPE_AGENT);
+    }
+}
+
+__device__ __forceinline__ void handoff_note(Handoff &h, float v, int row, int c, int lb0, float *__restrict__ y,
+                                             uint64_t *__restrict__ slots)
+{
+    if (h.row < 0) {
+        h.mine = v;
+        h.row = row;
+    } else {
+        Handoff t;
+        t.mine = v;
+        t.row = row;
+        handoff_issue(t, c, lb0, slots);
+        handoff_finish(t, c, lb0, y, slots);
+    }
+}
+
+__device__ __forceinline__ void store_sum(Handoff &h, float acc, int t, bool spans, bool empty, int c, int lb0,
+                                          float *__restrict__ y, float *__restrict__ carry,
+                                          uint64_t *__restrict__ slots)
+{
+    if (t == 0) {
+        if (!slots) carry[c] = acc;
+        else if (!empty) handoff_note(h, acc, lb0 - 1, c, lb0, y, slots);
+    } else if (slots && spans) {
+        handoff_note(h, acc, lb0 + t - 1, c, lb0, y, slots);
+    } else {
+        y[(int64_t)lb0 + t - 1] = acc;
+    }
+}
+
+__device__ __forceinline__ float read_as_padded(const float *smem, int k)
+{
+    const int q = (k * 1986) >> 16;
+    return (k - 33 * q == 32) ? 0.0f : smem[k - q];
+}
+
+template <int BLOCK, bool PREF, bool PAD>
 __device__ __forceinline__ void reduce_chunk(const float *smem, ChunkShared<BLOCK> &sh, int tid, int c, int lb0, int m,
                                              int64_t base, int64_t lim, const int32_t *__restrict__ row_ptr,
-                                             float *__restrict__ y, float *__restrict__ carry, int32_t rb0, int32_t re0)
-{
+                                             float *__restrict__ y, float *__restrict__ carry,
+                                             uint64_t *__restrict__ slots, int32_t rb0, int32_t re0)
+{
+    Handoff hs, hl, hh;
     for (int t = tid; t <= m; t += BLOCK) {
         int32_t rb, re;
         if (PREF && t == tid) { rb = rb0; re = re0; }
         else { rb = row_ptr[t == 0 ? lb0 : lb0 + t - 1]; re = t == 0 ? 0 : row_ptr[lb0 + t]; }
-        const Segment g = make_segment(t, lb0, base, lim, rb, re, y, carry, c);
-        const int ps = pad_idx(g.s), pe = pad_idx(g.e);
+        const Segment g = make_segment(t, base, lim, rb, re);
+        const int ps = pad_idx<PAD>(g.s), pe = pad_idx<PAD>(g.e);
         if (g.e - g.s <= kShortSeg) {
             float acc = 0.0f;
             const float *w = smem + ps;
@@ -255,51 +326,79 @@
                 acc = (((acc + a0) + a1) + a2) + a3;
             }
             for (; i < n; ++i) acc += w[i];
-            *g.dst = acc;
+            store_sum(hs, acc, t, g.spans, g.e == g.s, c, lb0, y, carry, slots);
         } else if (g.e - g.s <= kHugeSeg) {
             const int slot = atomicAdd(&sh.long_count, 1);
-            sh.long_seg[slot] = make_int2(t, ps | (pe << 16));
+            sh.long_seg[slot] = make_int2(t | (slots && g.spans ? kSpansBit : 0), ps | (pe << 16));
         } else {
             const int slot = atomicAdd(&sh.huge_count, 1);
-            sh.huge_seg[slot] = make_int2(t, ps | (pe << 16));
-        }
-    }
+            sh.huge_seg[slot] = make_int2(t | (slots && g.spans ? kSpansBit : 0), ps | (pe << 16));
+        }
+    }
+    if (slots) handoff_issue(hs, c, lb0, slots);
     __syncthreads();
 
     const int nlong = sh.long_count;
     const int sub = tid & (kGroup - 1);
     for (int i = tid / kGroup; i < nlong; i += BLOCK / kGroup) {
         const int2 q = sh.long_seg[i];
-        const int qe = (int)((unsigned)q.y >> 16);
+        const int qs = q.y & 0xffff, qe = (int)((unsigned)q.y >> 16);
         float acc = 0.0f;
-        for (int k = (q.y & 0xffff) + sub; k < qe; k += kGroup) acc += smem[k];
+        if constexpr (PAD) {
+            for (int k = qs + sub; k < qe; k += kGroup) acc += smem[k];
+        } else {
+            static_assert(kGroup == 16 && kShortSeg >= 32, "the block walk of the unpadded group sums");
+            const int k0 = qs + (qs >> 5) + sub;
+            int b = qs >> 5;
+            const int b1 = (qe - 1) >> 5;
+            {
+                const int i0 = (b << 5) | ((k0 - b) & 15);
+                const float v0 = smem[i0], v1 = smem[i0 + 16];
+                acc += i0 >= qs ? v0 : 0.0f;
+                acc += i0 + 16 >= qs ? v1 : 0.0f;
+            }
+            for (++b; b < b1; ++b) {
+                const int i0 = (b << 5) | ((k0 - b) & 15);
+                const float v0 = smem[i0], v1 = smem[i0 + 16];
+                acc += v0;
+                acc += v1;
+            }
+            {
+                const int i0 = (b1 << 5) | ((k0 - b1) & 15);
+                const float v0 = smem[i0], v1 = smem[i0 + 16];
+                acc += i0 < qe ? v0 : 0.0f;
+                acc += i0 + 16 < qe ? v1 : 0.0f;
+            }
+        }
 #pragma unroll
         for (int o = kGroup / 2; o > 0; o >>= 1) acc += __shfl_down(acc, o, kGroup);
-        if (sub == 0) {
-            if (q.x == 0) carry[c] = acc;
-            else y[(int64_t)lb0 + q.x - 1] = acc;
-        }
-    }
+        if (sub == 0) store_sum(hl, acc, q.x & ~kSpansBit, (q.x & kSpansBit) != 0, false, c, lb0, y, carry, slots);
+    }
+    if (slots) handoff_issue(hl, c, lb0, slots);
 
     const int nhuge = sh.huge_count;
     const int lane = tid & (kWave - 1);
     for (int i = tid >> 6; i < nhuge; i += BLOCK / kWave) {
         const int2 q = sh.huge_seg[i];
-        const int qe = (int)((unsigned)q.y >> 16);
+        int qs = q.y & 0xffff, qe = (int)((unsigned)q.y >> 16);
+        if constexpr (!PAD) { qs += qs >> 5; qe += qe >> 5; }
         float a0 = 0.0f, a1 = 0.0f;
-        int k = (q.y & 0xffff) + lane;
+        int k = qs + lane;
         for (; k + kWave < qe; k += 2 * kWave) {
-            a0 += smem[k];
-            a1 += smem[k + kWave];
-        }
-        if (k < qe) a0 += smem[k];
+            a0 += PAD ? smem[k] : read_as_padded(smem, k);
+            a1 += PAD ? smem[k + kWave] : read_as_padded(smem, k + kWave);
+        }
+        if (k < qe) a0 += PAD ? smem[k] : read_as_padded(smem, k);
         float acc = a0 + a1;
 #pragma unroll
         for (int o = kWave / 2; o > 0; o >>= 1) acc += __shfl_down(acc, o, kWave);
-        if (lane == 0) {
-            if (q.x == 0) carry[c] = acc;
-            else y[(int64_t)lb0 + q.x - 1] = acc;
-        }
+        if (lane == 0) store_sum(hh, acc, q.x & ~kSpansBit, (q.x & kSpansBit) != 0, false, c, lb0, y, carry, slots);
+    }
+    if (slots) {
+        handoff_issue(hh, c, lb0, slots);
+        handoff_finish(hs, c, lb0, y, slots);
+        handoff_finish(hl, c, lb0, y, slots);
+        handoff_finish(hh, c, lb0, y, slots);
     }
 }
 
@@ -394,13 +493,14 @@
     }
 }
 
-template <int BLOCK, bool TILED, bool PERSIST>
+template <int BLOCK, bool TILED, bool PERSIST, bool PAD>
 __device__ __forceinline__ void adaptive_body(float *smem, ChunkShared<BLOCK> &sh, int bid, int grid, int64_t rows,
                                               int64_t nnz, int64_t cols, int chunk0, int nrun,
                                               const int32_t *__restrict__ row_ptr,
                                               const int32_t *__restrict__ col_idx, const float *__restrict__ vals,
                                               const float *__restrict__ x, float *__restrict__ y,
                                               const int32_t *__restrict__ chunk_lb, float *__restrict__ carry,
+                                              uint64_t *__restrict__ slots,
                                               const int32_t *__restrict__ win, const int32_t *__restrict__ list,
                                               int kRegion)
 {
@@ -486,15 +586,9 @@
                 for (int q = 0; q < 4; ++q) xv[j][q] = x[cc[j][q]];
         }
 
-        zero_pad_words<BLOCK>(smem, tid);
-#pragma unroll
-        for (int j = 0; j < kVec; ++j) {
-            const int p0 = pad_idx((j * BLOCK + tid) * 4);
-            smem[p0] = vv[j][0] * xv[j][0];
-            smem[p0 + 1] = vv[j][1] * xv[j][1];
-            smem[p0 + 2] = vv[j][2] * xv[j][2];
-            smem[p0 + 3] = vv[j][3] * xv[j][3];
-        }
+        zero_pad_words<BLOCK, PAD>(smem, tid);
+#pragma unroll
+        for (int j = 0; j < kVec; ++j) store_products<BLOCK, PAD>(smem, tid, j, vv[j] * xv[j]);
 
         const int cn = c + wk.stride;
         const bool more = PERSIST && cn < wk.end;
@@ -505,7 +599,8 @@
         }
         __syncthreads();
 
-        reduce_chunk<BLOCK, !TILED>(smem, sh, tid, c, lb0, m, base, lim, row_ptr, y, carry, rb0, re0);
+        reduce_chunk<BLOCK, !TILED, PAD>(smem, sh, tid, c, lb0, m, base, lim, row_ptr, y, carry, PERSIST ? nullptr : slots, rb0,
+                                         re0);
 
         if (!more) break;
         __syncthreads();
@@ -513,27 +608,29 @@
     }
 }
 
-template <int BLOCK, bool TILED, bool PERSIST>
+template <int BLOCK, bool TILED, bool PERSIST, bool PAD>
 __global__ __launch_bounds__(BLOCK, waves_per_simd(BLOCK, PERSIST))
 void k_adaptive(int64_t rows, int64_t nnz, int64_t cols, int chunk0, int nrun, const int32_t *__restrict__ row_ptr,
                 const int32_t *__restrict__ col_idx, const float *__restrict__ vals, const float *__restrict__ x,
                 float *__restrict__ y, const int32_t *__restrict__ chunk_lb, float *__restrict__ carry,
-                const int32_t *__restrict__ win, const int32_t *__restrict__ list, int kRegion)
+                uint64_t *__restrict__ slots, const int32_t *__restrict__ win, const int32_t *__restrict__ list,
+                int kRegion)
 {
     extern __shared__ __attribute__((aligned(16))) float smem[];
     __shared__ ChunkShared<BLOCK> sh;
-    adaptive_body<BLOCK, TILED, PERSIST>(smem, sh, (int)blockIdx.x, (int)gridDim.x, rows, nnz, cols, chunk0, nrun, row_ptr,
-                                         col_idx, vals, x, y, chunk_lb, carry, win, list, kRegion);
+    adaptive_body<BLOCK, TILED, PERSIST, PAD>(smem, sh, (int)blockIdx.x, (int)gridDim.x, rows, nnz, cols, chunk0, nrun,
+                                              row_ptr, col_idx, vals, x, y, chunk_lb, carry, slots, win, list, kRegion);
 }
 
 using u4 = unsigned __attribute__((ext_vector_type(4)));
 
-template <int BLOCK, bool BLOCKS>
+template <int BLOCK, bool BLOCKS, bool PAD>
 __device__ __forceinline__ void tiled16_body(float *smem, ChunkShared<BLOCK> &sh, int bid, int64_t rows, int64_t cols,
                                              int nrun, const int32_t *__restrict__ row_ptr,
                                              const uint16_t *__restrict__ col16, const float *__restrict__ vals,
                                              const float *__restrict__ x, float *__restrict__ y,
                                              const int32_t *__restrict__ chunk_lb, float *__restrict__ carry,
+                                             uint64_t *__restrict__ slots,
                                              const int32_t *__restrict__ win, const int32_t *__restrict__ list,
                                              int kRegionArg, const int32_t *__restrict__ blk)
 {
@@ -616,24 +713,18 @@
         __syncthreads();
     }
 
-    zero_pad_words<BLOCK>(smem, tid);
-#pragma unroll
-    for (int j = 0; j < kVec; ++j) {
-        const int p0 = pad_idx((j * BLOCK + tid) * 4);
-        smem[p0] = vv[j][0] * xv[j][0];
-        smem[p0 + 1] = vv[j][1] * xv[j][1];
-        smem[p0 + 2] = vv[j][2] * xv[j][2];
-        smem[p0 + 3] = vv[j][3] * xv[j][3];
-    }
+    zero_pad_words<BLOCK, PAD>(smem, tid);
+#pragma unroll
+    for (int j = 0; j < kVec; ++j) store_products<BLOCK, PAD>(smem, tid, j, vv[j] * xv[j]);
     __syncthreads();
 #ifdef SPMV_T_NOREDUCE
     if (tid <= m && rb0 == 0x7fffffff) y[lb0 + tid] = smem[tid] + (float)re0;
 #else
-    reduce_chunk<BLOCK, true>(smem, sh, tid, c, lb0, m, base, lim, row_ptr, y, carry, rb0, re0);
+    reduce_chunk<BLOCK, true, PAD>(smem, sh, tid, c, lb0, m, base, lim, row_ptr, y, carry, slots, rb0, re0);
 #endif
 }
 
-template <int BLOCK, bool BLOCKS>
+template <int BLOCK, bool BLOCKS, bool PAD>
 __global__ __launch_bounds__(BLOCK, 8) void k_tiled16(int64_t rows, int64_t cols, int nrun,
                                                       const int32_t *__restrict__ row_ptr,
                                                       const uint16_t *__restrict__ col16,
@@ -641,23 +732,24 @@
                                                       const float *__restrict__ x, float *__restrict__ y,
                                                       const int32_t *__restrict__ chunk_lb,
                                                       float *__restrict__ carry,
+                                                      uint64_t *__restrict__ slots,
                                                       const int32_t *__restrict__ win,
                                                       const int32_t *__restrict__ list, int kRegion,
                                                       const int32_t *__restrict__ blk)
 {
     extern __shared__ __attribute__((aligned(16))) float smem[];
     __shared__ ChunkShared<BLOCK> sh;
-    tiled16_body<BLOCK, BLOCKS>(smem, sh, (int)blockIdx.x, rows, cols, nrun, row_ptr, col16, vals, x, y, chunk_lb, carry, win,
-                                list, kRegion, blk);
-}
-
-template <int BLOCK>
+    tiled16_body<BLOCK, BLOCKS, PAD>(smem, sh, (int)blockIdx.x, rows, cols, nrun, row_ptr, col16, vals, x, y, chunk_lb, carry,
+                                     slots, win, list, kRegion, blk);
+}
+
+template <int BLOCK, bool PAD>
 __device__ __forceinline__ void sorted_body(float *smem, ChunkShared<BLOCK> &sh, int bid, int64_t rows, int nrun,
                                             const int32_t *__restrict__ row_ptr, const uint32_t *__restrict__ perm,
                                             const float *__restrict__ vals, const float *__restrict__ x,
                                             float *__restrict__ y, const int32_t *__restrict__ chunk_lb,
-                                            float *__restrict__ carry, const int32_t *__restrict__ win,
-                                            const int32_t *__restrict__ list)
+                                            float *__restrict__ carry, uint64_t *__restrict__ slots,
+                                            const int32_t *__restrict__ win, const int32_t *__restrict__ list)
 {
     constexpr int kChunkT = chunk_of(BLOCK);
     constexpr int kVec = kNnzPerThread / 4;
@@ -702,32 +794,37 @@
 #pragma unroll
         for (int q = 0; q < 4; ++q) g[q] = xw[pw[j][q] & kColMask];
 #pragma unroll
-        for (int q = 0; q < 4; ++q) smem[pad_idx((int)(pw[j][q] >> kColBits))] = g[q];
+        for (int q = 0; q < 4; ++q) smem[pad_idx<PAD>((int)(pw[j][q] >> kColBits))] = g[q];
     }
     __syncthreads();
-    zero_pad_words<BLOCK>(smem, tid);
+    zero_pad_words<BLOCK, PAD>(smem, tid);
 #pragma unroll
     for (int j = 0; j < kVec; ++j) {
-        const int p0 = pad_idx((j * BLOCK + tid) * 4);
-        smem[p0] = vv[j][0] * smem[p0];
-        smem[p0 + 1] = vv[j][1] * smem[p0 + 1];
-        smem[p0 + 2] = vv[j][2] * smem[p0 + 2];
-        smem[p0 + 3] = vv[j][3] * smem[p0 + 3];
+        const int p0 = pad_idx<PAD>((j * BLOCK + tid) * 4);
+        f4 xs;
+        if constexpr (PAD) {
+#pragma unroll
+            for (int q = 0; q < 4; ++q) xs[q] = smem[p0 + q];
+        } else {
+            xs = *reinterpret_cast<const f4 *>(smem + p0);
+        }
+        store_products<BLOCK, PAD>(smem, tid, j, vv[j] * xs);
     }
     __syncthreads();
-    reduce_chunk<BLOCK, true>(smem, sh, tid, c, lb0, m, base, lim, row_ptr, y, carry, rb0, re0);
-}
-
-template <int BLOCK>
+    reduce_chunk<BLOCK, true, PAD>(smem, sh, tid, c, lb0, m, base, lim, row_ptr, y, carry, slots, rb0, re0);
+}
+
+template <int BLOCK, bool PAD>
 __global__ __launch_bounds__(BLOCK, 8) void k_sorted(int64_t rows, int nrun, const int32_t *__restrict__ row_ptr,
                                                      const uint32_t *__restrict__ perm, const float *__restrict__ vals,
                                                      const float *__restrict__ x, float *__restrict__ y,
                                                      const int32_t *__restrict__ chunk_lb, float *__restrict__ carry,
-                                                     const int32_t *__restrict__ win, const int32_t *__restrict__ list)
+                                                     uint64_t *__restrict__ slots, const int32_t *__restrict__ win,
+                                                     const int32_t *__restrict__ list)
 {
     extern __shared__ __attribute__((aligned(16))) float smem[];
     __shared__ ChunkShared<BLOCK> sh;
-    sorted_body<BLOCK>(smem, sh, (int)blockIdx.x, rows, nrun, row_ptr, perm, vals, x, y, chunk_lb, carry, win, list);
+    sorted_body<BLOCK, PAD>(smem, sh, (int)blockIdx.x, rows, nrun, row_ptr, perm, vals, x, y, chunk_lb, carry, slots, win, list);
 }
 
 template <int BLOCK>
@@ -778,7 +875,7 @@
     }
 }
 
-template <int BLOCK, bool BLOCKS>
+template <int BLOCK, bool BLOCKS, bool PAD>
 __global__ __launch_bounds__(BLOCK, 8) void k_tiled_mixed(int64_t rows, int64_t nnz, int64_t cols, int n32, int nsorted,
                                                           int n16, const int32_t *__restrict__ row_ptr,
                                                           const int32_t *__restrict__ col_idx,
@@ -788,6 +885,7 @@
                                                           const float *__restrict__ x, float *__restrict__ y,
                                                           const int32_t *__restrict__ chunk_lb,
                                                           float *__restrict__ carry,
+                                                          uint64_t *__restrict__ slots,
                                                           const int32_t *__restrict__ win,
                                                           const int32_t *__restrict__ list32,
                                                           const int32_t *__restrict__ list_sorted,
@@ -798,13 +896,14 @@
     __shared__ ChunkShared<BLOCK> sh;
     const int b = (int)blockIdx.x;
     if (b < n32)
-        adaptive_body<BLOCK, true, false>(smem, sh, b, n32, rows, nnz, cols, 0, n32, row_ptr, col_idx, vals, x,
-                                          y, chunk_lb, carry, win, list32, kRegion);
+        adaptive_body<BLOCK, true, false, PAD>(smem, sh, b, n32, rows, nnz, cols, 0, n32, row_ptr, col_idx, vals, x,
+                                               y, chunk_lb, carry, slots, win, list32, kRegion);
     else if (b < n32 + nsorted)
-        sorted_body<BLOCK>(smem, sh, b - n32, rows, nsorted, row_ptr, perm, vals, x, y, chunk_lb, carry, win, list_sorted);
+        sorted_body<BLOCK, PAD>(smem, sh, b - n32, rows, nsorted, row_ptr, perm, vals, x, y, chunk_lb, carry, slots, win,
+                                list_sorted);
     else
-        tiled16_body<BLOCK, BLOCKS>(smem, sh, b - n32 - nsorted, rows, cols, n16, row_ptr, col16, vals, x, y, chunk_lb,
-                                    carry, win, list16, kRegion, blk);
+        tiled16_body<BLOCK, BLOCKS, PAD>(smem, sh, b - n32 - nsorted, rows, cols, n16, row_ptr, col16, vals, x, y, chunk_lb,
+                                         carry, slots, win, list16, kRegion, blk);
 }
 
 template <int BLOCK>
@@ -979,7 +1078,28 @@
     if (c >= nchunks - 1) return;
     const int lb0 = chunk_lb[c], lb1 = chunk_lb[c + 1];
     if (lb1 == lb0) return;
-    if ((int64_t)row_ptr[lb1] > (int64_t)(c + 1) * chunk) atomicAdd(count, 1);
+    const int64_t endp = row_ptr[lb1];
+    if (endp > (int64_t)(c + 1) * chunk) atomicAdd(count, 1);
+    if (endp > (int64_t)(c + 2) * chunk) atomicAdd(count + 1, 1);
+}
+
+constexpr int kPadBins = kShortSeg / 4 + 1;
+__global__ __launch_bounds__(256) void k_plan_row_stats(int64_t rows, const int32_t *__restrict__ row_ptr,
+                                                        unsigned long long *__restrict__ stats)
+{
+    __shared__ unsigned hist[kPadBins];
+    __shared__ unsigned long long huge;
+    if (threadIdx.x < kPadBins) hist[threadIdx.x] = 0u;
+    if (threadIdx.x == 0) huge = 0ull;
+    __syncthreads();
+    for (int64_t r = (int64_t)blockIdx.x * 256 + threadIdx.x; r < rows; r += (int64_t)gridDim.x * 256) {
+        const int len = row_ptr[r + 1] - row_ptr[r];
+        if (len > 0 && len <= kShortSeg && (len & 3) == 0) atomicAdd(&hist[len >> 2], 1u);
+        else if (len > kHugeSeg) atomicAdd(&huge, (unsigned long long)len);
+    }
+    __syncthreads();
+    if (threadIdx.x < kPadBins && hist[threadIdx.x]) atomicAdd(&stats[threadIdx.x], (unsigned long long)hist[threadIdx.x]);
+    if (threadIdx.x == 0 && huge) atomicAdd(&stats[kPadBins], huge);
 }
 
 static int default_passes(int block) { return block == 1024 ? 12 : (block == 512 ? 4 : 2); }
@@ -1025,23 +1145,45 @@
     if (p.nchunks == 0) return SPMV_OK;
     SPMV_HIP_TRY(p.d_lb.alloc((size_t)p.nchunks + 1));
     SPMV_HIP_TRY(p.d_carry.alloc((size_t)p.nchunks));
+    SPMV_HIP_TRY(p.d_slots.alloc((size_t)p.nchunks));
+    SPMV_HIP_TRY(hipMemsetAsync(p.d_slots.get(), 0, sizeof(uint64_t) * (size_t)p.nchunks, s));
     hipLaunchKernelGGL(k_plan_chunks, dim3((p.nchunks + 1 + 255) / 256), dim3(256), 0, s, h.rows, p.nchunks, chunk,
                        h.d_row_ptr, p.d_lb);
     int rc = check_launch("k_plan_chunks");
     if (rc) return rc;
     {
         DevPtr<int32_t> cnt;
-        SPMV_HIP_TRY(cnt.alloc(1));
-        SPMV_HIP_TRY(hipMemsetAsync(cnt.get(), 0, sizeof(int32_t), s));
+        DevPtr<unsigned long long> rstat;
+        SPMV_HIP_TRY(cnt.alloc(2));
+        SPMV_HIP_TRY(rstat.alloc(kPadBins + 1));
+        SPMV_HIP_TRY(hipMemsetAsync(cnt.get(), 0, 2 * sizeof(int32_t), s));
+        SPMV_HIP_TRY(hipMemsetAsync(rstat.get(), 0, (kPadBins + 1) * sizeof(unsigned long long), s));
         if (p.nchunks > 1) {
             hipLaunchKernelGGL(k_plan_spans, dim3((p.nchunks - 1 + 255) / 256), dim3(256), 0, s, p.nchunks, chunk,
                                h.d_row_ptr, p.d_lb, cnt.get());
             if ((rc = check_launch("k_plan_spans"))) return rc;
         }
-        int32_t spans = 0;
-        SPMV_HIP_TRY(hipMemcpyAsync(&spans, cnt.get(), sizeof(int32_t), hipMemcpyDeviceToHost, s));
+        {
+            const int64_t want = (h.rows + 255) / 256;
+            hipLaunchKernelGGL(k_plan_row_stats, dim3((unsigned)(want < 4096 ? (want > 0 ? want : 1) : 4096)), dim3(256), 0, s,
+                               h.rows, h.d_row_ptr, rstat.get());
+            if ((rc = check_launch("k_plan_row_stats"))) return rc;
+        }
+        int32_t spans[2] = {0, 0};
+        unsigned long long rs[kPadBins + 1];
+        SPMV_HIP_TRY(hipMemcpyAsync(spans, cnt.get(), sizeof spans, hipMemcpyDeviceToHost, s));
+        SPMV_HIP_TRY(hipMemcpyAsync(rs, rstat.get(), sizeof rs, hipMemcpyDeviceToHost, s));
         SPMV_HIP_TRY(hipStreamSynchronize(s));
-        p.spanning_rows = spans;
+        p.spanning_rows = spans[0];
+        p.long_spans = spans[1];
+        p.fused = p.long_spans == 0 && !p.persist;
+        if (const char *e = getenv("SPMV_CARRY")) {
+            if (!strcmp(e, "fixup")) p.fused = false;
+        }
+        unsigned long long mode = 0;
+        for (int k = 1; k < kPadBins; ++k) mode = rs[k] > mode ? rs[k] : mode;
+        p.pad = 2 * mode >= (unsigned long long)h.rows || 8 * rs[kPadBins] >= (unsigned long long)h.nnz;
+        if (const char *e = getenv("SPMV_PAD")) p.pad = atoi(e) != 0;
     }
     if (windows) {
         SPMV_HIP_TRY(p.d_win.alloc(2 * (size_t)p.nchunks + 6));
@@ -1376,32 +1518,36 @@
     return device_cus(device) * per_cu;
 }
 
-template <int BLOCK, bool TILED, bool PERSIST>
+static uint64_t *slots_of(const ChunkPlan &p) { return p.fused ? p.d_slots.get() : nullptr; }
+static bool padded(const ChunkPlan &p) { return p.pad || p.persist || p.nblk_chunks > 0; }
+
+template <int BLOCK, bool TILED, bool PERSIST, bool PAD>
 static int launch_range(const spmv_csr &h, const ChunkPlan &p, int chunk0, int nrun, const float *x, float *y,
                         hipStream_t s, const int32_t *list = nullptr)
 {
     if (nrun <= 0) return SPMV_OK;
     const size_t lds = sizeof(float) * (size_t)p.region;
     static LdsOptIn optin;
-    if (int rc = optin.ensure(reinterpret_cast<const void *>(&k_adaptive<BLOCK, TILED, PERSIST>), h.device, (int)lds)) return rc;
+    if (int rc = optin.ensure(reinterpret_cast<const void *>(&k_adaptive<BLOCK, TILED, PERSIST, PAD>), h.device, (int)lds)) return rc;
     int grid = nrun;
     if (PERSIST) {
         const int res = resident_workgroups(h.device, BLOCK, waves_per_simd(BLOCK, true));
         if (grid > res) grid = res;
     }
-    hipLaunchKernelGGL((k_adaptive<BLOCK, TILED, PERSIST>), dim3(grid), dim3(BLOCK), lds, s, h.rows, h.nnz, h.cols,
-                       chunk0, nrun, h.d_row_ptr, h.d_col_idx, h.d_vals, x, y, p.d_lb, p.d_carry, p.d_win, list, p.region);
+    hipLaunchKernelGGL((k_adaptive<BLOCK, TILED, PERSIST, PAD>), dim3(grid), dim3(BLOCK), lds, s, h.rows, h.nnz, h.cols,
+                       chunk0, nrun, h.d_row_ptr, h.d_col_idx, h.d_vals, x, y, p.d_lb, p.d_carry, slots_of(p), p.d_win, list,
+                       p.region);
     return check_launch("k_adaptive");
 }
 
-template <int BLOCK, bool BLOCKS>
+template <int BLOCK, bool BLOCKS, bool PAD>
 static int launch_tiled16_t(const spmv_csr &h, const ChunkPlan &p, const float *x, float *y, hipStream_t s)
 {
     const size_t lds = sizeof(float) * (size_t)p.region;
     static LdsOptIn optin;
-    if (int rc = optin.ensure(reinterpret_cast<const void *>(&k_tiled16<BLOCK, BLOCKS>), h.device, (int)lds)) return rc;
-    hipLaunchKernelGGL((k_tiled16<BLOCK, BLOCKS>), dim3(p.n16), dim3(BLOCK), lds, s, h.rows, h.cols, p.n16, h.d_row_ptr,
-                       p.d_col16, h.d_vals, x, y, p.d_lb, p.d_carry, p.d_win,
+    if (int rc = optin.ensure(reinterpret_cast<const void *>(&k_tiled16<BLOCK, BLOCKS, PAD>), h.device, (int)lds)) return rc;
+    hipLaunchKernelGGL((k_tiled16<BLOCK, BLOCKS, PAD>), dim3(p.n16), dim3(BLOCK), lds, s, h.rows, h.cols, p.n16, h.d_row_ptr,
+                       p.d_col16, h.d_vals, x, y, p.d_lb, p.d_carry, slots_of(p), p.d_win,
                        p.n16 == p.nchunks ? (const int32_t *)nullptr : p.d_list16, p.region, p.d_blk);
     return check_launch("k_tiled16");
 }
@@ -1410,36 +1556,38 @@
 static int launch_tiled16(const spmv_csr &h, const ChunkPlan &p, const float *x, float *y, hipStream_t s)
 {
     if (p.n16 <= 0) return SPMV_OK;
-    return p.nblk_chunks > 0 ? launch_tiled16_t<BLOCK, true>(h, p, x, y, s) : launch_tiled16_t<BLOCK, false>(h, p, x, y, s);
-}
-
-template <int BLOCK, bool BLOCKS>
+    if (p.nblk_chunks > 0) return launch_tiled16_t<BLOCK, true, true>(h, p, x, y, s);
+    return padded(p) ? launch_tiled16_t<BLOCK, false, true>(h, p, x, y, s) : launch_tiled16_t<BLOCK, false, false>(h, p, x, y, s);
+}
+
+template <int BLOCK, bool BLOCKS, bool PAD>
 static int launch_mixed_t(const spmv_csr &h, const ChunkPlan &p, const float *x, float *y, hipStream_t s)
 {
     const size_t lds = sizeof(float) * (size_t)p.region;
     static LdsOptIn optin;
-    if (int rc = optin.ensure(reinterpret_cast<const void *>(&k_tiled_mixed<BLOCK, BLOCKS>), h.device, (int)lds)) return rc;
+    if (int rc = optin.ensure(reinterpret_cast<const void *>(&k_tiled_mixed<BLOCK, BLOCKS, PAD>), h.device, (int)lds)) return rc;
     const int n32 = p.nchunks - p.n16 - p.nsorted;
-    hipLaunchKernelGGL((k_tiled_mixed<BLOCK, BLOCKS>), dim3(p.nchunks), dim3(BLOCK), lds, s, h.rows, h.nnz, h.cols, n32,
+    hipLaunchKernelGGL((k_tiled_mixed<BLOCK, BLOCKS, PAD>), dim3(p.nchunks), dim3(BLOCK), lds, s, h.rows, h.nnz, h.cols, n32,
                        p.nsorted, p.n16, h.d_row_ptr, h.d_col_idx, p.d_col16, p.d_perm, h.d_vals, x, y, p.d_lb, p.d_carry,
-                       p.d_win, p.d_list32, p.d_list_sorted, p.d_list16, p.region, p.d_blk);
+                       slots_of(p), p.d_win, p.d_list32, p.d_list_sorted, p.d_list16, p.region, p.d_blk);
     return check_launch("k_tiled_mixed");
 }
 
 template <int BLOCK>
 static int launch_mixed(const spmv_csr &h, const ChunkPlan &p, const float *x, float *y, hipStream_t s)
 {
-    return p.nblk_chunks > 0 ? launch_mixed_t<BLOCK, true>(h, p, x, y, s) : launch_mixed_t<BLOCK, false>(h, p, x, y, s);
-}
-
-template <int BLOCK>
+    if (p.nblk_chunks > 0) return launch_mixed_t<BLOCK, true, true>(h, p, x, y, s);
+    return padded(p) ? launch_mixed_t<BLOCK, false, true>(h, p, x, y, s) : launch_mixed_t<BLOCK, false, false>(h, p, x, y, s);
+}
+
+template <int BLOCK, bool PAD>
 static int launch_sorted(const spmv_csr &h, const ChunkPlan &p, const float *x, float *y, hipStream_t s)
 {
     const size_t lds = sizeof(float) * (size_t)p.region;
     static LdsOptIn optin;
-    if (int rc = optin.ensure(reinterpret_cast<const void *>(&k_sorted<BLOCK>), h.device, (int)lds)) return rc;
-    hipLaunchKernelGGL((k_sorted<BLOCK>), dim3(p.nsorted), dim3(BLOCK), lds, s, h.rows, p.nsorted, h.d_row_ptr, p.d_perm,
-                       h.d_vals, x, y, p.d_lb, p.d_carry, p.d_win, p.d_list_sorted);
+    if (int rc = optin.ensure(reinterpret_cast<const void *>(&k_sorted<BLOCK, PAD>), h.device, (int)lds)) return rc;
+    hipLaunchKernelGGL((k_sorted<BLOCK, PAD>), dim3(p.nsorted), dim3(BLOCK), lds, s, h.rows, p.nsorted, h.d_row_ptr, p.d_perm,
+                       h.d_vals, x, y, p.d_lb, p.d_carry, slots_of(p), p.d_win, p.d_list_sorted);
     return check_launch("k_sorted");
 }
 
@@ -1449,14 +1597,16 @@
     if constexpr (TILED) {
         if (!persist && (p.n16 > 0 || p.nsorted > 0)) {
             if (p.n16 == p.nchunks) return launch_tiled16<BLOCK>(h, p, x, y, s);
-            if (p.nsorted == p.nchunks) return launch_sorted<BLOCK>(h, p, x, y, s);
+            if (p.nsorted == p.nchunks) return padded(p) ? launch_sorted<BLOCK, true>(h, p, x, y, s) : launch_sorted<BLOCK, false>(h, p, x, y, s);
             return launch_mixed<BLOCK>(h, p, x, y, s);
         }
     }
-    if (!persist) return launch_range<BLOCK, TILED, false>(h, p, 0, p.nchunks, x, y, s);
+    if (!persist)
+        return padded(p) ? launch_range<BLOCK, TILED, false, true>(h, p, 0, p.nchunks, x, y, s)
+                         : launch_range<BLOCK, TILED, false, false>(h, p, 0, p.nchunks, x, y, s);
     const int nfull = (int)(h.nnz / chunk_of(BLOCK));
-    int rc = launch_range<BLOCK, TILED, true>(h, p, 0, nfull, x, y, s);
-    if (rc == SPMV_OK && p.nchunks > nfull) rc = launch_range<BLOCK, TILED, false>(h, p, nfull, p.nchunks - nfull, x, y, s);
+    int rc = launch_range<BLOCK, TILED, true, true>(h, p, 0, nfull, x, y, s);
+    if (rc == SPMV_OK && p.nchunks > nfull) rc = launch_range<BLOCK, TILED, false, true>(h, p, nfull, p.nchunks - nfull, x, y, s);
     return rc;
 }
 
@@ -1480,7 +1630,7 @@
     else if (p.block == 512) rc = launch_either<512, true>(persist, h, p, x, y, s);
     else rc = launch_either<1024, true>(persist, h, p, x, y, s);
     if (rc) return rc;
-    if (p.nchunks > 1 && p.spanning_rows > 0) {
+    if (!p.fused && p.nchunks > 1 && p.spanning_rows > 0) {
         hipLaunchKernelGGL(k_carry_fixup, dim3((p.nchunks - 1 + 255) / 256), dim3(256), 0, s, p.nchunks,
                            chunk_of(p.block), h.d_row_ptr, p.d_lb, p.d_carry, y);
         rc = check_launch("k_carry_fixup");
diff --git a/spmv-test_amd/csrc/spmv_internal.hpp b/spmv-test_amd/csrc/spmv_internal.hpp
--- a/spmv-test_amd/csrc/spmv_internal.hpp
+++ b/spmv-test_amd/csrc/spmv_internal.hpp
@@ -80,6 +80,10 @@
     int nchunks = 0;
     DevPtr<int32_t> d_lb;
     DevPtr<float> d_carry;
+    DevPtr<uint64_t> d_slots;
+    bool fused = false;
+    bool pad = true;
+    int long_spans = 0;
     DevPtr<int32_t> d_win;
     DevPtr<uint16_t> d_col16;
     DevPtr<int32_t> d_list16;
```

New measurement: 5090 GB/s. -12.7%, worse.
